# opensensor/thingino-accel

Hardware: AMD Instinct MI355X
Metric: images/sec yolov5s_int8 640x640 batch256 (higher is better)
Workload: dtype int8

## Files before the change

### thingino-accel_amd/csrc/hip/conv_i8.hip

```cpp
#include "conv_i8_common.hpp"

#ifndef I8M_ABL
#define I8M_ABL 0
#endif
template <int BPX, int BN, int STAGES, int KS = 1, int NW = 4>
__global__ __launch_bounds__(NW * 64) void conv_i8_mfma(const mhip_conv_i8_t p, const long total_pix, const int k64,
                                                         const int8_t *__restrict__ zeros, const unsigned noc,
                                                         const unsigned nblk, const int lg_inc, const unsigned kw_magic,
                                                         const fastdiv_t dhw, const fastdiv_t dow, const int bufmode,
                                                         const unsigned in_bytes) {
    ANAT_BEGIN();
    const bool POW2 = lg_inc >= 0;
    const bool masked = p.kh * p.kw <= 32;
    constexpr int SLICE = (BPX + BN) * BK;
    constexpr int STAGE = KS * SLICE;
    constexpr int NWN = BN == 128 ? 2 : 1;
    constexpr int NWM = NW / NWN;
    constexpr int WPX = BPX / NWM / 16;
    constexpr int WOC = BN / NWN / 16;
    constexpr int XROWS = BPX / NW;
    constexpr int XI = XROWS / 16;
    constexpr int LW = (BN / 16 + NW - 1) / NW;
    constexpr int L = XI + LW;
    static_assert(XI >= 1 && XROWS % 16 == 0, "every wave fetches whole 16-row pieces of the pixel tile");
// ... 158 lines not shown
        nstage = nstage + 1 == STAGES ? 0 : nstage + 1;
    }
    ANAT_NOW(2);
    __syncthreads();
    if (I8M_ABL & 1) {
        int fold = 0;
#pragma unroll
        for (int s = 0; s < WOC; s++)
#pragma unroll
            for (int t = 0; t < WPX; t++) fold ^= acc[s][t][0] ^ acc[s][t][1] ^ acc[s][t][2] ^ acc[s][t][3];
        if (fold == 0x12345678) p.out[0] = 1;
        return;
    }
    epilogue<BPX, BN, WPX, WOC, true>(p, acc, lds, slut, rowoff, oc0, pxw, ocw, hw);
    ANAT_END(p);
}

__device__ __forceinline__ int lds_off128(int row, int chunk8) { return row * 128 + ((chunk8 ^ ((row >> 1) & 7)) << 4); }
template <int BPX, int BN, int NW>
__global__ __launch_bounds__(NW * 64) void conv_i8_r128(const mhip_conv_i8_t p, const long total_pix, const int k128,
                                                         const unsigned noc, const unsigned nblk, const int lg_inc,
                                                         const unsigned kw_magic, const fastdiv_t dhw, const fastdiv_t dow,
                                                         const unsigned in_bytes) {
    constexpr int STAGE = (BPX + BN) * 128;
    constexpr int NWN = BN == 128 ? 2 : 1;
    constexpr int NWM = NW / NWN;
    constexpr int WPX = BPX / NWM / 16;
    constexpr int WOC = BN / NWN / 16;
    constexpr int XI = BPX / 8 / NW;
    constexpr int WI = BN / 8 / NW;
    static_assert(XI >= 1 && WI >= 1 && BPX % (8 * NW) == 0 && BN % (8 * NW) == 0, "whole 8-row pieces per wave");
    extern __shared__ __attribute__((aligned(16))) int8_t dynlds[];
    uint8_t *slut = (uint8_t *)dynlds;
    lds_base_must_be_zero(dynlds);
    long *rowoff = (long *)(dynlds + LUTB);
    int8_t *lds = dynlds + BPX * 8 + LUTB;

    const int tid = threadIdx.x, lane = tid & 63;
    const int wv = __builtin_amdgcn_readfirstlane(tid >> 6);
    const unsigned id = xcd_remap(blockIdx.x, nblk);
    const long pix0 = (long)(id / noc) * BPX;
    const int oc0 = (int)(id % noc) * BN;
    const int hw = p.out_h * p.out_w;
    const int wm = wv % NWM, wn = wv / NWM;
    const int pxw = wm * (WPX * 16), ocw = wn * (WOC * 16);
    v4i acc[WOC][WPX];
    init_acc<WPX, WOC>(p, acc, oc0 + ocw);
    if (p.lut2) { if (tid < 128) ((uint32_t *)slut)[tid] = ((const uint32_t *)p.lut2)[tid]; }
    else if (p.lut && tid < 64) ((uint32_t *)slut)[tid] = ((const uint32_t *)p.lut)[tid];
    fill_rowoff<BPX>(p, rowoff, [=](int row) { long q = pix0 + row; return q < total_pix ? q : -1L; }, (unsigned)hw, dhw);

    const int lrow = lane >> 3, lslot = lane & 7;
    int xvoff[XI];
    unsigned tapmask[XI];
#pragma unroll
    for (int j = 0; j < XI; j++) {
        const int trow = (wv * XI + j) * 8 + lrow;
        const long pix = pix0 + trow;
        const bool valid = pix < total_pix;
        const unsigned f = valid ? fdiv((unsigned)pix, dhw) : 0u;
        const unsigned rem = valid ? (unsigned)pix - f * (unsigned)hw : 0u;
        const int oy = (int)fdiv(rem, dow), ox = (int)(rem - (unsigned)oy * (unsigned)p.out_w);
        const int iy0 = oy * p.stride_h - p.pad_top, ix0 = ox * p.stride_w - p.pad_left;
        const int chunk = lslot ^ ((trow >> 1) & 7);
        xvoff[j] = (int)(f * (unsigned)p.in_stride) + (iy0 * p.in_w + ix0) * p.in_c + chunk * 16;
        const int kx_lo = ix0 < 0 ? -ix0 : 0, kx_hi = p.in_w - ix0 < p.kw ? p.in_w - ix0 : p.kw;
        const unsigned colbits = kx_hi > kx_lo ? ((kx_hi >= 32 ? ~0u : (1u << kx_hi) - 1u) & ~((1u << kx_lo) - 1u)) : 0u;
        unsigned m = 0;
        for (int r = 0; r < p.kh; r++) {
            const int iy = iy0 + r;
            if (iy >= 0 && iy < p.in_h) m |= colbits << (r * p.kw);
        }
        tapmask[j] = valid ? m : 0u;
    }
    int wvoff[WI];
#pragma unroll
    for (int j = 0; j < WI; j++) {
        const int trow = (wv * WI + j) * 8 + lrow;
        wvoff[j] = (oc0 + trow) * k128 + (lslot ^ ((trow >> 1) & 7)) * 16;
    }
    const __amdgpu_buffer_rsrc_t xrs = __builtin_amdgcn_make_buffer_rsrc((void *)p.in, 0, (int)in_bytes, 0x00020000);
    const __amdgpu_buffer_rsrc_t wrs = __builtin_amdgcn_make_buffer_rsrc((void *)p.w, 0, p.oc_pad * k128, 0x00020000);
    const int taps = p.kh * p.kw;
    const int nst = k128 / 128;
    auto issue = [&](int st, int buf) {
        int8_t *sb = lds + buf * STAGE;
        const int utap = (st * 128) >> lg_inc, urc = (st * 128) & ((1 << lg_inc) - 1);
        const int uky = (int)(((unsigned)utap * kw_magic) >> 16), ukx = utap - uky * p.kw;
        const int ukoff = (uky * p.in_w + ukx) * p.in_c + urc;
        const bool uvalid = utap < taps;
#pragma unroll
        for (int j = 0; j < XI; j++) {
            const bool ok = uvalid & (((tapmask[j] >> utap) & 1u) != 0u);
            blds16(xrs, ok ? xvoff[j] + ukoff : -1, 0, sb + (wv * XI + j) * 1024);
        }
#pragma unroll
        for (int j = 0; j < WI; j++) blds16(wrs, wvoff[j], st * 128, sb + BPX * 128 + (wv * WI + j) * 1024);
    };

    issue(0, 0);
    const int frow = lane & 15, fchunk = lane >> 4;
    for (int st = 0; st < nst; st++) {
        wait_vmcnt<0>();
        __builtin_amdgcn_s_barrier();
        asm volatile("" ::: "memory");
        const int8_t *xs = lds + (st & 1) * STAGE, *ws = xs + BPX * 128;
        v4i xb[2][WPX], wa[2][WOC];
#pragma unroll
        for (int h = 0; h < 2; h++) {
#pragma unroll
            for (int t = 0; t < WPX; t++) xb[h][t] = *(const v4i *)(xs + lds_off128(pxw + t * 16 + frow, h * 4 + fchunk));
#pragma unroll
            for (int q = 0; q < WOC; q++) wa[h][q] = *(const v4i *)(ws + lds_off128(ocw + q * 16 + frow, h * 4 + fchunk));
        }
        if (st + 1 < nst) issue(st + 1, (st + 1) & 1);
#pragma unroll
        for (int h = 0; h < 2; h++)
#pragma unroll
            for (int q = 0; q < WOC; q++)
#pragma unroll
                for (int t = 0; t < WPX; t++) acc[q][t] = __builtin_amdgcn_mfma_i32_16x16x64_i8(wa[h][q], xb[h][t], acc[q][t], 0, 0, 0);
    }
    __syncthreads();
    epilogue<BPX, BN, WPX, WOC, true>(p, acc, lds, slut, rowoff, oc0, pxw, ocw, hw);
}

template <int A, int B>
__device__ __forceinline__ void wait_vmcnt_at_most(int n) {
    constexpr int HI = A > B ? A : B, LO = A > B ? B : A;
    if (n >= A + B) wait_vmcnt<A + B>();
    else if (n >= HI) wait_vmcnt<HI>();
    else if (n >= LO) wait_vmcnt<LO>();
    else wait_vmcnt<0>();
}

struct conv_out_side_t {
    int8_t *out;
    size_t out_stride;
    const int8_t *w;
    const int32_t *bias;
    const uint8_t *lut, *lut2;
    int out_c, relu, out_pix_stride, out_ch_off;
    float cs;
    unsigned out_bytes;
};
template <int BPX, int BN, int STAGES, bool HAS_LUT, bool SEG = false, bool PAIR = false>
__global__ __launch_bounds__(NTHREADS) void conv_i8_persist(const mhip_conv_i8_t pin, const unsigned total_pix, const int k64,
                                                            const int8_t *__restrict__ zeros, const unsigned noc,
                                                            const unsigned npt, const unsigned ngrp, const int lg_inc,
                                                            const unsigned kw_magic, const fastdiv_t dhw, const fastdiv_t dow,
                                                            const unsigned out_bytes_first, const conv_out_side_t alt,
                                                            const unsigned noc0, const int bufmode, const unsigned in_bytes,
                                                            const int wres) {
    ANAT_BEGIN();
    const int STAGE = wres ? BPX * BK : (BPX + BN) * BK;
    constexpr int NWN = BN == 128 ? 2 : 1;
    constexpr int NWM = 4 / NWN;
    constexpr int WPX = BPX / NWM / 16;
    constexpr int WOC = BN / NWN / 16;
    constexpr int XI = BPX / 64;
    constexpr int LW = BN >= 128 ? 2 : 1;
    constexpr int L = XI + LW;
    constexpr int NST = WPX;
    extern __shared__ __attribute__((aligned(16))) int8_t dynlds[];
    uint8_t *slut = (uint8_t *)dynlds;
    int8_t *lds = dynlds + LUTB;
    lds_base_must_be_zero(dynlds);

    const int tid = threadIdx.x, lane = tid & 63;
    const int wv = __builtin_amdgcn_readfirstlane(tid >> 6);
    const unsigned id = xcd_remap(blockIdx.x, noc * ngrp);
    const unsigned grp = id / noc;
    unsigned ot = id - grp * noc;
    mhip_conv_i8_t p = pin;
    unsigned out_bytes = out_bytes_first;
    if (PAIR && ot >= noc0) {
        ot -= noc0;
        p.lut2 = alt.lut2;
        p.out = alt.out; p.out_stride = alt.out_stride; p.w = alt.w; p.bias = alt.bias; p.lut = alt.lut;
        p.out_c = alt.out_c; p.relu = alt.relu; p.out_pix_stride = alt.out_pix_stride; p.out_ch_off = alt.out_ch_off;
        p.cs = alt.cs;
        out_bytes = alt.out_bytes;
    }
    const int oc0 = (int)ot * BN;
    const unsigned t0 = (unsigned)(((unsigned long long)grp * npt) / ngrp);
    const unsigned t1 = (unsigned)(((unsigned long long)(grp + 1) * npt) / ngrp);
    if (t0 >= t1) return;
    const unsigned hw = (unsigned)(p.out_h * p.out_w);
    const int wm = wv % NWM, wn = wv / NWM;
    const int pxw = wm * (WPX * 16), ocw = wn * (WOC * 16);

    auto packed_row16 = [](int c) { return ((c >> 2) & 1) * 16 + (c >> 3) * 4 + (c & 3); };
    v4i bias[WOC];
#pragma unroll
    for (int s = 0; s < WOC; s++)
        bias[s] = p.bias ? *(const v4i *)(p.bias + (BN == 16 ? packed_row16((lane >> 4) * 4) : oc0 + ocw + s * 16 + (lane >> 4) * 4)) : (v4i){0, 0, 0, 0};
    if (HAS_LUT) {
        if (p.lut2) { if (tid < 128) ((uint32_t *)slut)[tid] = ((const uint32_t *)p.lut2)[tid]; }
        else if (tid < 64) ((uint32_t *)slut)[tid] = ((const uint32_t *)p.lut)[tid];
        __syncthreads();
    }
    const __amdgpu_buffer_rsrc_t orsrc = __builtin_amdgcn_make_buffer_rsrc(p.out, 0, (int)out_bytes, 0x00020000);

    const int schunk = (lane & 3) ^ (((lane >> 4) & 1) << 1);
    const int8_t *xwin[XI];
    unsigned tapmask[XI];
    unsigned rowf[SEG ? XI : 1], rowrem[SEG ? XI : 1];
    unsigned rowrem_up[SEG ? XI : 1];
    int xvoff[XI];
    auto setup_rows = [&](unsigned tile) {
#pragma unroll
        for (int j = 0; j < XI; j++) {
            const unsigned pix = tile * BPX + wv * (BPX / 4) + j * 16 + (lane >> 2);
            const bool valid = pix < total_pix;
            const unsigned f = valid ? fdiv(pix, dhw) : 0u;
            const unsigned rem = valid ? pix - f * hw : 0u;
            if (SEG) {
                rowf[j] = f;
                rowrem[j] = rem;
                const unsigned oy = fdiv(rem, dow), ox = rem - oy * (unsigned)p.out_w;
                rowrem_up[j] = (oy >> 1) * ((unsigned)p.out_w >> 1) + (ox >> 1);
                tapmask[j] = valid ? 1u : 0u;
                continue;
            }
            const int oy = (int)fdiv(rem, dow), ox = (int)(rem - (unsigned)oy * (unsigned)p.out_w);
            const int iy0 = oy * p.stride_h - p.pad_top, ix0 = ox * p.stride_w - p.pad_left;
            xwin[j] = p.in + (size_t)f * p.in_stride + ((long)iy0 * p.in_w + ix0) * p.in_c;
            xvoff[j] = (int)(f * (unsigned)p.in_stride) + (iy0 * p.in_w + ix0) * p.in_c + schunk * 16;
            const int kx_lo = ix0 < 0 ? -ix0 : 0, kx_hi = p.in_w - ix0 < p.kw ? p.in_w - ix0 : p.kw;
            const unsigned colbits = kx_hi > kx_lo ? ((kx_hi >= 32 ? ~0u : (1u << kx_hi) - 1u) & ~((1u << kx_lo) - 1u)) : 0u;
            unsigned m = 0;
            for (int r = 0; r < p.kh; r++) {
                const int iy = iy0 + r;
                if (iy >= 0 && iy < p.in_h) m |= colbits << (r * p.kw);
            }
            tapmask[j] = valid ? m : 0u;
        }
    };
    const int8_t *wsrc[LW];
    int wq[LW], wvoff[LW];
#pragma unroll
    for (int j = 0; j < LW; j++) {
        wq[j] = BN >= 64 ? wv * LW + j : (BN == 16 ? 0 : (wv & 1));
        const int wrow = BN == 16 ? packed_row16(lane >> 2) : oc0 + wq[j] * 16 + (lane >> 2);
        wsrc[j] = p.w + (size_t)wrow * k64 + schunk * 16;
        wvoff[j] = wrow * k64 + schunk * 16;
    }
    const __amdgpu_buffer_rsrc_t xrs = __builtin_amdgcn_make_buffer_rsrc((void *)p.in, 0, (int)in_bytes, 0x00020000);
    const __amdgpu_buffer_rsrc_t wrs = __builtin_amdgcn_make_buffer_rsrc((void *)p.w, 0, p.oc_pad * k64, 0x00020000);
    const int taps = p.kh * p.kw;
    const int nks = k64 / BK;

    auto issue = [&](int ks, int stage) {
        int8_t *sb = lds + stage * STAGE;
        const unsigned pos = (unsigned)(ks * BK + schunk * 16);
        if (SEG) {
            auto owner = [&](int c) { return (c >= p.seg_c0[1]) + (c >= p.seg_c0[2]) + (c >= p.seg_c0[3]); };
            const int sa = owner(ks * BK), sb2 = owner(ks * BK + 32);
            const bool hi = schunk >= 2;
            const int8_t *base = hi ? p.seg_in[sb2] : p.seg_in[sa];
            const unsigned fstride = (unsigned)(hi ? p.seg_stride[sb2] : p.seg_stride[sa]);
            const unsigned segc = (unsigned)(hi ? p.seg_c[sb2] : p.seg_c[sa]);
            const unsigned coff = pos - (unsigned)(hi ? p.seg_c0[sb2] : p.seg_c0[sa]);
            const bool up = ((p.seg_up >> (hi ? sb2 : sa)) & 1) != 0;
            const bool kvalid = (int)pos < p.in_c;
#pragma unroll
            for (int j = 0; j < XI; j++) {
                const bool ok = kvalid & (tapmask[j] != 0u);
                const int8_t *src = base + (size_t)rowf[j] * fstride + (size_t)(up ? rowrem_up[j] : rowrem[j]) * segc + coff;
                glds16(ok ? src : zeros, sb + (wv * (BPX / 4) + j * 16) * BK);
            }
        } else if (bufmode) {
            const int utap = (ks * BK) >> lg_inc, urc = (ks * BK) & ((1 << lg_inc) - 1);
            const int uky = (int)(((unsigned)utap * kw_magic) >> 16), ukx = utap - uky * p.kw;
            const int ukoff = (uky * p.in_w + ukx) * p.in_c + urc;
            const bool uvalid = utap < taps;
#pragma unroll
            for (int j = 0; j < XI; j++) {
                const bool ok = uvalid & (((tapmask[j] >> utap) & 1u) != 0u);
                blds16(xrs, ok ? xvoff[j] + ukoff : -1, 0, sb + (wv * (BPX / 4) + j * 16) * BK);
            }
            if (!wres)
#pragma unroll
                for (int j = 0; j < LW; j++) blds16(wrs, wvoff[j], ks * BK, sb + BPX * BK + wq[j] * 16 * BK);
            return;
        } else {
            const unsigned tap = pos >> lg_inc;
            const int rc = (int)(pos & ((1u << lg_inc) - 1u));
            const int ky = (int)((tap * kw_magic) >> 16);
            const int kx = (int)tap - ky * p.kw;
            const bool kvalid = (int)tap < taps;
            const long koff = ((long)ky * p.in_w + kx) * p.in_c + rc;
#pragma unroll
            for (int j = 0; j < XI; j++) {
                const bool ok = kvalid & ((tapmask[j] >> tap) & 1u);
                glds16(ok ? xwin[j] + koff : zeros, sb + (wv * (BPX / 4) + j * 16) * BK);
            }
        }
        if (!wres)
#pragma unroll
            for (int j = 0; j < LW; j++) glds16(wsrc[j] + ks * BK, sb + BPX * BK + wq[j] * 16 * BK);
    };

    int8_t *const wres_base = lds + STAGES * STAGE;
    if (wres)
        for (int ks = 0; ks < nks; ks++)
#pragma unroll
            for (int j = 0; j < LW; j++) glds16(wsrc[j] + ks * BK, wres_base + (ks * BN + wq[j] * 16) * BK);
    unsigned itile = t0;
    int iks = 0;
    int younger[STAGES - 1];
    setup_rows(t0);
    int nstage = 0;
#pragma unroll
    for (int s = 0; s < STAGES - 1; s++) {
        int n = 0;
        if (itile < t1) {
            issue(iks, nstage);
            n = wres ? XI : L;
            if (++iks == nks) {
                iks = 0;
                if (++itile < t1) setup_rows(itile);
            }
        }
#pragma unroll
        for (int i = 0; i < s; i++) younger[i] += n;
        younger[s] = 0;
        nstage++;
    }
    nstage = STAGES - 1;

    const int frow = lane & 15, fchunk = lane >> 4;
    const int chan = ocw + (lane >> 4) * (4 * WOC);
    const int pstride = p.out_pix_stride ? p.out_pix_stride : p.out_c;
    const int lo = p.relu ? 0 : -128;
    const uint8_t *lut128 = slut + 128;
    const bool ragged = (p.out_c % (WOC * 4)) != 0;
    int stage = 0;
    ANAT_NOW(1);
    for (unsigned tile = t0; tile < t1; tile++) {
        v4i acc[WOC][WPX];
        for (int ks = 0; ks < nks; ks++) {
            wait_vmcnt_at_most<(STAGES - 2) * L, NST>(younger[0]);
            __builtin_amdgcn_s_barrier();
            asm volatile("" ::: "memory");
            const int8_t *xs = lds + stage * STAGE, *ws = wres ? wres_base + ks * (BN * BK) : xs + BPX * BK;
            v4i xb[WPX], wa[WOC];
#pragma unroll
            for (int t = 0; t < WPX; t++) xb[t] = *(const v4i *)(xs + lds_off(pxw + t * 16 + frow, fchunk));
#pragma unroll
            for (int s = 0; s < WOC; s++) wa[s] = *(const v4i *)(ws + lds_off(ocw + s * 16 + frow, fchunk));
            int n = 0;
            if (itile < t1) {
                issue(iks, nstage);
                n = wres ? XI : L;
                if (++iks == nks) {
                    iks = 0;
                    if (++itile < t1) setup_rows(itile);
                }
            }
#pragma unroll
            for (int i = 0; i + 1 < STAGES - 1; i++) younger[i] = younger[i + 1] + n;
            younger[STAGES - 2] = 0;
            if (ks == 0) {
#pragma unroll
                for (int s = 0; s < WOC; s++)
#pragma unroll
                    for (int t = 0; t < WPX; t++) acc[s][t] = __builtin_amdgcn_mfma_i32_16x16x64_i8(wa[s], xb[t], bias[s], 0, 0, 0);
            } else {
#pragma unroll
                for (int s = 0; s < WOC; s++)
#pragma unroll
                    for (int t = 0; t < WPX; t++) acc[s][t] = __builtin_amdgcn_mfma_i32_16x16x64_i8(wa[s], xb[t], acc[s][t], 0, 0, 0);
            }
            stage = stage + 1 == STAGES ? 0 : stage + 1;
            nstage = nstage + 1 == STAGES ? 0 : nstage + 1;
        }
#ifdef ANATOMY
        if (tile + 1 == t1) ANAT_NOW(2);
#endif
#pragma unroll
        for (int t = 0; t < WPX; t++) {
            const unsigned pix = tile * BPX + pxw + t * 16 + (lane & 15);
            const unsigned f = fdiv(pix, dhw), rem = pix - f * hw;
            const unsigned off = f * (unsigned)p.out_stride + rem * (unsigned)pstride + (unsigned)(p.out_ch_off + oc0 + chan);
            const int nvalid = p.out_c - (oc0 + chan);
            const bool ok = pix < total_pix && nvalid >= WOC * 4;
            uint32_t pk[WOC];
            int a[WOC * 4];
#pragma unroll
            for (int s = 0; s < WOC; s++)
#pragma unroll
                for (int r = 0; r < 4; r++) a[s * 4 + r] = acc[s][t][r];
            if (HAS_LUT && p.lut2) requant_pack<WOC * 4, HAS_LUT, true, true, false, true>(a, p.cs, lo, lut128, pk);
            else requant_pack<WOC * 4, HAS_LUT, true, true>(a, p.cs, lo, lut128, pk);
            const int voff = ok ? (int)off : -1;
            if (WOC == 4)
                __builtin_amdgcn_raw_buffer_store_b128((v4i){(int)pk[0], (int)pk[1], (int)pk[2], (int)pk[3]}, orsrc, voff, 0, 0);
            else if (WOC == 2)
                __builtin_amdgcn_raw_buffer_store_b64((v2i){(int)pk[0], (int)pk[WOC > 1 ? 1 : 0]}, orsrc, voff, 0, 0);
            else
                __builtin_amdgcn_raw_buffer_store_b32((int)pk[0], orsrc, voff, 0, 0);
            if (ragged) {
                const bool part = pix < total_pix && nvalid > 0 && nvalid < WOC * 4;
                const int nv = part ? nvalid : 0;
                const int o4 = nv & 8, o2 = nv & 12, o1 = nv & 14;
                const uint32_t w4 = o4 ? pk[(WOC * 4 > 8) ? 2 : 0] : pk[0];
                const int i2 = o2 >> 2, i1 = o1 >> 2;
                uint32_t w2 = pk[0], w1 = pk[0];
#pragma unroll
                for (int q = 1; q < WOC; q++) {
                    w2 = i2 == q ? pk[q] : w2;
                    w1 = i1 == q ? pk[q] : w1;
                }
                w1 >>= (o1 & 2) * 8;
                if (WOC == 4)
                    __builtin_amdgcn_raw_buffer_store_b64((v2i){(int)pk[0], (int)pk[1]}, orsrc, (nv & 8) ? (int)off : -1, 0, 0);
                __builtin_amdgcn_raw_buffer_store_b32((int)w4, orsrc, (nv & 4) ? (int)off + o4 : -1, 0, 0);
                __builtin_amdgcn_raw_buffer_store_b16((short)w2, orsrc, (nv & 2) ? (int)off + o2 : -1, 0, 0);
                __builtin_amdgcn_raw_buffer_store_b8((char)w1, orsrc, (nv & 1) ? (int)off + o1 : -1, 0, 0);
            }
        }
#pragma unroll
        for (int i = 0; i < STAGES - 1; i++) younger[i] += ragged ? NST * (WOC == 4 ? 5 : 4) : NST;
    }
    ANAT_END(p);
}
ANAT_SETTER(mhip_anatomy_set_i8)
__device__ __forceinline__ bool mhip_small_c_dev(int in_c, int kw, int out_c) { return in_c <= 4 && kw <= 8 && out_c <= 64; }
template <int BN>
__global__ __launch_bounds__(NTHREADS) void conv_i8_generic(const mhip_conv_i8_t p, const long total_pix, const int k64,
                                                            const fastdiv_t dhw) {
    constexpr int STAGE = (BP + BN) * BK;
    constexpr int WPX = 2, WOC = BN / 16;
    constexpr int TILE_BYTES = BP * (BN + OPAD);
    constexpr int LDS_BYTES = (2 * STAGE > TILE_BYTES ? 2 * STAGE : TILE_BYTES) + 256;
    __shared__ __attribute__((aligned(16))) int8_t lds[LDS_BYTES];
    __shared__ long rowoff[BP];
    uint8_t *slut = (uint8_t *)lds + LDS_BYTES - 256;

    const int tid = threadIdx.x, lane = tid & 63, wv = tid >> 6;
    const long pix0 = (long)blockIdx.x * BP;
    const int oc0 = blockIdx.y * BN;
    const int hw = p.out_h * p.out_w;
    if (p.lut && tid < 64) ((uint32_t *)slut)[tid] = ((const uint32_t *)p.lut)[tid];
    fill_rowoff<BP>(p, rowoff, [=](int row) { long q = pix0 + row; return q < total_pix ? q : -1L; }, (unsigned)hw, dhw);

    const int cc = tid & 3;
    const int8_t *xbase[2];
    int iy0[2], ix0[2];
    bool rvalid[2];
#pragma unroll
    for (int j = 0; j < 2; j++) {
        long pix = pix0 + (tid >> 2) + j * 64;
        rvalid[j] = pix < total_pix;
        long f = rvalid[j] ? pix / hw : 0;
        int rem = rvalid[j] ? (int)(pix - f * hw) : 0;
        int oy = rem / p.out_w, ox = rem - oy * p.out_w;
        iy0[j] = oy * p.stride_h - p.pad_top;
        ix0[j] = ox * p.stride_w - p.pad_left;
        xbase[j] = p.in + (size_t)f * p.in_stride;
    }
    int ky = 0, rc = cc * 16;
    while (rc >= p.row_pad) { rc -= p.row_pad; ky++; }
    const int ceff = mhip_small_c_dev(p.in_c, p.kw, p.out_c) ? 4 : p.in_c;
    const int nks = k64 / BK;
    constexpr int WLOADS = (BN * 4 + NTHREADS - 1) / NTHREADS;
    v4i xreg[2], wreg[WLOADS];

    auto load_global = [&](int ks) {
#pragma unroll
        for (int j = 0; j < 2; j++) {
            v4i v = {0, 0, 0, 0};
            const int iy = iy0[j] + ky;
            if (rvalid[j] && ky < p.kh && iy >= 0 && iy < p.in_h) {
                const int8_t *rowp = xbase[j] + ((long)iy * p.in_w + ix0[j]) * p.in_c;
                int8_t b[16];
#pragma unroll
                for (int e = 0; e < 16; e++) {
                    const int rr = rc + e;
                    int8_t val = 0;
                    const int tap = rr / ceff, ch = rr - tap * ceff;
                    if (tap < p.kw && ch < p.in_c) {
                        const int ix = ix0[j] + tap;
                        if (ix >= 0 && ix < p.in_w) val = rowp[tap * p.in_c + ch];
                    }
                    b[e] = val;
                }
                v = *(v4i *)b;
            }
            xreg[j] = v;
        }
#pragma unroll
        for (int j = 0; j < WLOADS; j++) {
            const int idx = tid + j * NTHREADS;
            if (idx < BN * 4) wreg[j] = *(const v4i *)(p.w + (size_t)(oc0 + (idx >> 2)) * k64 + ks * BK + (idx & 3) * 16);
        }
        rc += BK;
        while (rc >= p.row_pad) { rc -= p.row_pad; ky++; }
    };
    auto store_lds = [&](int buf) {
#pragma unroll
        for (int j = 0; j < 2; j++) *(v4i *)(lds + buf * STAGE + lds_off((tid >> 2) + j * 64, cc)) = xreg[j];
#pragma unroll
        for (int j = 0; j < WLOADS; j++) {
            const int idx = tid + j * NTHREADS;
            if (idx < BN * 4) *(v4i *)(lds + buf * STAGE + BP * BK + lds_off(idx >> 2, idx & 3)) = wreg[j];
        }
    };

    v4i acc[WOC][WPX];
    init_acc<WPX, WOC>(p, acc, oc0);

    load_global(0);
    store_lds(0);
    __syncthreads();
    const int frow = lane & 15, fchunk = lane >> 4;
    const int pxw = wv * 32;
    for (int ks = 0; ks < nks; ks++) {
        const int buf = ks & 1;
        if (ks + 1 < nks) load_global(ks + 1);
        v4i xb[WPX];
#pragma unroll
        for (int t = 0; t < WPX; t++) xb[t] = *(const v4i *)(lds + buf * STAGE + lds_off(pxw + t * 16 + frow, fchunk));
#pragma unroll
        for (int s = 0; s < WOC; s++) {
            v4i wa = *(const v4i *)(lds + buf * STAGE + BP * BK + lds_off(s * 16 + frow, fchunk));
#pragma unroll
            for (int t = 0; t < WPX; t++) acc[s][t] = __builtin_amdgcn_mfma_i32_16x16x64_i8(wa, xb[t], acc[s][t], 0, 0, 0);
        }
        if (ks + 1 < nks) store_lds(buf ^ 1);
        __syncthreads();
    }
    epilogue<BP, BN, WPX, WOC>(p, acc, lds, slut, rowoff, oc0, pxw, 0, hw);
}

extern "C" int mhip_conv_i8_oc_row(int oc, int oc_pad) {
    const int G = (oc_pad % 64 == 0) ? 64 : 32, NS = G / 16;
    const int g = oc / G, local = oc - g * G;
    const int q = local / (4 * NS), rem = local - q * 4 * NS, s = rem >> 2, r = rem & 3;
    return g * G + s * 16 + q * 4 + r;
}

extern "C" int mhip_conv_i8_is_safe(float cs) {
    return cs == cs && cs < 0.99f && cs > -0.99f;
}

extern "C" int mhip_conv_i8_lut2_ok(float cs) {
    if (!mhip_conv_i8_is_safe(cs)) return 0;
    const float a = cs < 0 ? -cs : cs;
    if (!(a >= 1e-6f)) return 0;
    const float quirk = 0.49999997f;
    const double a0 = (double)quirk / (double)a;
    for (int d = -3; d <= 3; d++) {
        const double c = (double)(long long)(a0 + 0.5) + d;
        if (c < 1.0 || c > 2147483647.0) continue;
        volatile float prod = (float)(int)c * a;
        if (prod == quirk) return 0;
    }
    return 1;
}

extern "C" int mhip_conv_i8_small_c(int in_c, int kw, int out_c) { return in_c <= 4 && kw <= 8 && out_c <= 64; }

extern "C" void mhip_conv_i8_pack_geom(int in_c, int kw, int out_c, int *row_pad, int *oc_pad, int *c_eff) {
    const int small = mhip_conv_i8_small_c(in_c, kw, out_c);
    if (row_pad) *row_pad = small ? 32 : (kw * in_c + 15) & ~15;
    if (oc_pad) *oc_pad = (out_c + 31) & ~31;
    if (c_eff) *c_eff = small ? 4 : in_c;
}

static tune_t g_tune;
static int env_int(const char *name, int dflt) {
    const char *e = getenv(name);
    return e ? atoi(e) : dflt;
}
const tune_t &conv_i8_tune_state() {
    if (!g_tune.init) {
        g_tune.persist = env_int("MARS_HIP_PERSIST", 1);
// ... 208 lines not shown
    *bpx = px;
    return true;
}

static variant_t default_variant(const mhip_conv_i8_t *p, int nks) {
    variant_t v;
    v.patch = 0;
    v.ks2 = 0;
    v.w8 = 0;
    v.wres = 0;
    v.r128 = 0;
    v.rows = 0;
    int ring = 0;
    const long wg_large = ((long)p->frames * p->out_h * p->out_w + 255) / 256 * ((p->oc_pad + 127) / 128);
    const bool few = wg_large < tune().few_wgs && tune().persist && !tune().bpx && !tune().stages && tune().small_batch;
    if (few) {
        if (conv_i8_patch_ok(p, 4, &ring)) {
            v.persist = 0; v.bpx = 0; v.stages = 0; v.patch = 4;
            return v;
        }
        if (nks >= 8 && r128_ok(p)) {
            v.persist = 0; v.bpx = 0; v.stages = 0; v.r128 = 1;
            return v;
        }
        v.bpx = 128;
        v.persist = nks <= tune().persist_maxk && persist_eligible(p);
        if (((p->out_c | p->out_pix_stride | p->out_ch_off) & 15) != 0 && p->nseg <= 1) v.persist = 0;
        v.stages = v.persist ? 2 : 3;
        return v;
    }
    if (tune().persist && !tune().bpx && !tune().stages && tune().rows && p->out_w <= 20 && p->in_c >= 256 && conv_i8_rows_ok(p)) {
        v.persist = 0; v.bpx = 0; v.stages = 0; v.rows = 1;
        return v;
    }
    if (tune().persist && !tune().bpx && !tune().stages) {
        if (conv_i8_patch_ok(p, 16, &ring)) {
            v.persist = 0; v.bpx = 0; v.stages = 0; v.patch = 16;
            return v;
        }
        if (conv_i8_patch_ok(p, 8, &ring) && ring >= 2) {
            v.persist = 0; v.bpx = 0; v.stages = 0; v.patch = 8;
            return v;
        }
    }
    v.bpx = tune().bpx ? tune().bpx : ((p->oc_pad % 128 != 0 && nks <= 2) ? 256 : 128);
    v.persist = tune().persist && nks <= tune().persist_maxk && persist_eligible(p);
    if (((p->out_c | p->out_pix_stride | p->out_ch_off) & 15) != 0 && p->nseg <= 1) v.persist = 0;
    v.stages = v.persist ? 2 : (tune().stages ? tune().stages : (nks <= 4 ? 2 : 3));
    if (v.stages != 3) v.stages = 2;
    if (v.persist && v.stages == 2 && !tune().bpx && wres_default(p, nks, &v.bpx)) v.wres = 1;
    if ((!v.persist || (!v.wres && nks >= 8 && p->nseg <= 1)) && !tune().bpx && !tune().stages && p->oc_pad % 128 == 0 &&
        nks >= (tune().persist_maxk < 8 ? tune().persist_maxk + 1 : 8)) {
        v.persist = 0; v.w8 = 1; v.bpx = 256; v.stages = 3;
    }
    if (p->nseg > 1 && !v.wres && !tune().bpx && nks >= 8) v.bpx = 256;
    return v;
}

template <int BPX, int BN>
static int launch_variant_t(const mhip_conv_i8_t *p, long total_pix, int k64, const variant_t &v) {
    if (v.persist) {
        if (!persist_eligible(p)) return -1;
        int lg = 0;
        while ((1 << lg) < p->in_c) lg++;
        const unsigned magic = ((65536u + (unsigned)p->kw - 1u) / (unsigned)p->kw);
        if (v.wres && wres_lds<BPX, BN>(k64) > 80 * 1024) return -1;
        if (p->nseg > 1)
            return p->lut ? launch_persist_t<BPX, BN, 2, true, true>(p, total_pix, k64, lg, magic, nullptr, v.wres)
                          : launch_persist_t<BPX, BN, 2, false, true>(p, total_pix, k64, lg, magic, nullptr, v.wres);
        if (v.wres)
            return p->lut ? launch_persist_t<BPX, BN, 2, true>(p, total_pix, k64, lg, magic, nullptr, 1)
                          : launch_persist_t<BPX, BN, 2, false>(p, total_pix, k64, lg, magic, nullptr, 1);
        if (v.stages == 2)
            return p->lut ? launch_persist_t<BPX, BN, 2, true>(p, total_pix, k64, lg, magic)
                          : launch_persist_t<BPX, BN, 2, false>(p, total_pix, k64, lg, magic);
        return -1;
    }
    if constexpr (BN == 16) {
        return -1;
    } else {
        if (v.w8) return BN == 128 ? launch_mfma<256, 128, 3, 1, 8>(p, total_pix, k64) : -1;
        if (v.ks2) return BPX == 128 && BN >= 64 ? launch_mfma<128, (BN >= 64 ? BN : 64), 2, 2>(p, total_pix, k64) : -1;
        return v.stages == 2 ? launch_mfma<BPX, BN, 2>(p, total_pix, k64) : launch_mfma<BPX, BN, 3>(p, total_pix, k64);
    }
}
static bool bn16_ok(const mhip_conv_i8_t *p) {
    static const bool off = getenv("MARS_HIP_NO_BN16") != nullptr;
    return !off && p->out_c <= 16 && p->oc_pad == 32 && p->nseg <= 1;
}

static int launch_variant(const mhip_conv_i8_t *p, long total_pix, int k64, const variant_t &v) {
    if (v.persist < 0) return -1;
    if (v.rows) return conv_i8_launch_rows(p);
    if (v.r128) return launch_r128(p, total_pix, v.r128);
    if (v.patch) return conv_i8_launch_patch(p, k64, v.patch);
    const int bn = p->oc_pad % 128 == 0 ? 128 : (p->oc_pad % 64 == 0 ? 64 : 32);
    const bool b16 = v.persist && v.stages == 2 && bn16_ok(p);
    if (v.bpx == 256) {
        if (bn == 128) return launch_variant_t<256, 128>(p, total_pix, k64, v);
        if (bn == 64) return launch_variant_t<256, 64>(p, total_pix, k64, v);
        if (b16) return launch_variant_t<256, 16>(p, total_pix, k64, v);
        return launch_variant_t<256, 32>(p, total_pix, k64, v);
    }
    if (bn == 128) return launch_variant_t<128, 128>(p, total_pix, k64, v);
    if (bn == 64) return launch_variant_t<128, 64>(p, total_pix, k64, v);
    if (b16) return launch_variant_t<128, 16>(p, total_pix, k64, v);
    return launch_variant_t<128, 32>(p, total_pix, k64, v);
}

template <int BPX, int BN>
static int launch_pair_t(const mhip_conv_i8_t *a, const mhip_conv_i8_t *b, long total_pix, int k64, int lg, unsigned magic,
                         int wres) {
    if (a->nseg > 1) return -2;
    return launch_persist_t<BPX, BN, 2, true, false, true>(a, total_pix, k64, lg, magic, b, wres);
}
extern "C" int mhip_conv_i8_pair(const mhip_conv_i8_t *a, const mhip_conv_i8_t *b) {
    if (!a || !b || !tune().persist || tune().variant) return -2;
    if (a->in != b->in || a->in_stride != b->in_stride || a->frames != b->frames || a->in_h != b->in_h || a->in_w != b->in_w ||
        a->in_c != b->in_c || a->out_h != b->out_h || a->out_w != b->out_w || a->kh != b->kh || a->kw != b->kw ||
        a->stride_h != b->stride_h || a->stride_w != b->stride_w || a->pad_top != b->pad_top || a->pad_left != b->pad_left ||
        a->row_pad != b->row_pad || a->nseg != b->nseg || a->seg_up != b->seg_up || !a->lut || !b->lut || a->add || b->add ||
        a->out_nchw || b->out_nchw)
        return -2;
    for (int i = 0; i < a->nseg; i++)
        if (a->seg_in[i] != b->seg_in[i] || a->seg_c[i] != b->seg_c[i] || a->seg_stride[i] != b->seg_stride[i]) return -2;
    if ((a->in_c % 16) != 0 || mhip_conv_i8_small_c(a->in_c, a->kw, a->out_c) || mhip_conv_i8_small_c(b->in_c, b->kw, b->out_c))
        return -2;
    if (a->nseg > 1 && (!seg_valid(a) || !seg_valid(b))) return -2;
    if (!persist_eligible(a) || !persist_eligible(b)) return -2;
    const int bn = a->oc_pad % 128 == 0 ? 128 : (a->oc_pad % 64 == 0 ? 64 : 32);
    const int bnb = b->oc_pad % 128 == 0 ? 128 : (b->oc_pad % 64 == 0 ? 64 : 32);
    if (bn != bnb || !mhip_zero_page()) return -2;
    const long total_pix = (long)a->frames * a->out_h * a->out_w;
    const int k64 = (a->kh * a->row_pad + BK - 1) / BK * BK, nks = k64 / BK;
    if (total_pix <= 0 || total_pix > 0x7fffffffL) return -2;
    int lg = 0;
    while ((1 << lg) < a->in_c) lg++;
    const unsigned magic = ((65536u + (unsigned)a->kw - 1u) / (unsigned)a->kw);
    const variant_t dv = default_variant(a, nks);
    const int bpx = dv.bpx ? dv.bpx : 128, wres = dv.persist && dv.wres && (tune().wres & 2);
    const bool b16 = bn16_ok(a) && bn16_ok(b);
    if (bpx == 256) {
        if (bn == 128) return launch_pair_t<256, 128>(a, b, total_pix, k64, lg, magic, wres);
        if (bn == 64) return launch_pair_t<256, 64>(a, b, total_pix, k64, lg, magic, wres);
        if (b16) return launch_pair_t<256, 16>(a, b, total_pix, k64, lg, magic, wres);
        return launch_pair_t<256, 32>(a, b, total_pix, k64, lg, magic, wres);
    }
    if (bn == 128) return launch_pair_t<128, 128>(a, b, total_pix, k64, lg, magic, wres);
    if (bn == 64) return launch_pair_t<128, 64>(a, b, total_pix, k64, lg, magic, wres);
    if (b16) return launch_pair_t<128, 16>(a, b, total_pix, k64, lg, magic, wres);
    return launch_pair_t<128, 32>(a, b, total_pix, k64, lg, magic, wres);
}

extern "C" int mhip_conv_i8_seg_ok(const mhip_conv_i8_t *p) {
    return p && (p->in_c % 16) == 0 && !mhip_conv_i8_small_c(p->in_c, p->kw, p->out_c) && seg_valid(p) && persist_eligible(p);
}

extern "C" int mhip_conv_i8_variants(const mhip_conv_i8_t *p, int *codes, int max) {
    if (!p || (p->in_c % 16) != 0 || mhip_conv_i8_small_c(p->in_c, p->kw, p->out_c)) return 0;
    const int k64 = (p->kh * p->row_pad + BK - 1) / BK * BK, nks = k64 / BK;
    int n = 0;
    if (p->pre_w) {
        const int first = conv_i8_pre_tile_rows(p);
        for (int th : {first, 16, 8, 4})
            if (th && n < max && conv_i8_patch_ok(p, th, nullptr)) {
                const int code = th == 16 ? 10 : (th == 8 ? 9 : 11);
                bool seen = false;
                for (int i = 0; i < n; i++) seen |= codes[i] == code;
                if (!seen) codes[n++] = code;
            }
        return n;
    }
    if (p->nseg > 1) {
        const int bn = p->oc_pad % 128 == 0 ? 128 : (p->oc_pad % 64 == 0 ? 64 : 32);
        const variant_t dv = default_variant(p, nks);
        const int dflt = dv.persist && dv.wres ? (dv.bpx == 256 ? 15 : 14) : (dv.bpx == 256 ? 4 : 2);
        if (n < max) codes[n++] = dflt;
        if (n < max && dflt != 2) codes[n++] = 2;
        if (n < max && dflt != 4) codes[n++] = 4;
        if (n < max && dflt != 14 && LUTB + 2 * (size_t)128 * BK + (size_t)nks * bn * BK <= 80 * 1024) codes[n++] = 14;
        if (n < max && dflt != 15 && LUTB + 2 * (size_t)256 * BK + (size_t)nks * bn * BK <= 80 * 1024) codes[n++] = 15;
        return n;
    }
    const int dflt = variant_code(default_variant(p, nks));
    if (n < max) codes[n++] = dflt;
    for (int code = 1; code <= NVARIANTS; code++) {
        const variant_t v = variant_of(code);
        if (code == dflt) continue;
        if (v.patch && !conv_i8_patch_ok(p, v.patch, nullptr)) continue;
        if (v.persist && !persist_eligible(p)) continue;
        if (v.ks2 && ((nks & 1) || nks < 4 || p->oc_pad % 64 != 0)) continue;
        if (v.w8 && (p->oc_pad % 128 != 0 || nks < 3)) continue;
        if (v.persist < 0) continue;
        if (v.r128 && !r128_ok(p)) continue;
        if (v.rows && !conv_i8_rows_ok(p)) continue;
        if (v.wres) {
            const int bn = p->oc_pad % 128 == 0 ? 128 : (p->oc_pad % 64 == 0 ? 64 : 32);
            if (LUTB + 2 * (size_t)v.bpx * BK + (size_t)nks * bn * BK > 80 * 1024) continue;
        }
        if (!v.persist && v.stages == 3 && nks <= 2) continue;
        if (n < max) codes[n++] = code;
    }
    return n;
}

template <int BN>
static int launch_generic(const mhip_conv_i8_t *p, long total_pix, int k64) {
    dim3 grid((unsigned)((total_pix + BP - 1) / BP), (unsigned)(p->oc_pad / BN));
    hipLaunchKernelGGL((conv_i8_generic<BN>), grid, dim3(NTHREADS), 0, mhip_stream_native(), *p, total_pix, k64,
                       make_fastdiv((unsigned)(p->out_h * p->out_w)));
    return mhip_check(hipGetLastError(), "conv_i8_generic launch");
}

extern "C" int mhip_conv_i8(const mhip_conv_i8_t *p) {
    if (!p || !p->in || !p->out || !p->w) return -1;
    if (p->out_pix_stride < 0 || p->out_ch_off < 0 || (p->out_nchw && (p->out_pix_stride || p->out_ch_off)) ||
        (p->out_pix_stride && p->out_pix_stride < p->out_ch_off + p->out_c))
        return -1;
    if (p->frames <= 0 || p->in_h <= 0 || p->in_w <= 0 || p->in_c <= 0 || p->out_h <= 0 || p->out_w <= 0 ||
        p->out_c <= 0 || p->kh <= 0 || p->kw <= 0 || p->stride_h < 0 || p->stride_w < 0)
        return -1;
    int row_pad, oc_pad;
    mhip_conv_i8_pack_geom(p->in_c, p->kw, p->out_c, &row_pad, &oc_pad, nullptr);
    if (row_pad != p->row_pad || oc_pad != p->oc_pad) return -1;
    if (p->add && (!p->safe || p->out_nchw || ((p->out_c | p->out_pix_stride | p->out_ch_off) & 15) || (p->in_c % 16) != 0 ||
                   mhip_conv_i8_small_c(p->in_c, p->kw, p->out_c) || p->nseg > 1))
        return -1;
    const long total_pix = (long)p->frames * p->out_h * p->out_w;
    const int k64 = (p->kh * p->row_pad + BK - 1) / BK * BK;
    if (total_pix <= 0 || total_pix > 0x7fffffffL || (total_pix + BP - 1) / BP * (oc_pad / 32) > 0x7fffffffL) return -1;
    if (p->in_planar) {
        if (p->in_planar > 4 || p->in_c != 4 || p->in_w < 4 || p->stride_h < 1 || p->stride_w < 1 || p->add || p->nseg > 1 ||
            !mhip_conv_i8_small_c(p->in_c, p->kw, p->out_c))
            return -2;
        return conv_i8_try_smallc(p, k64);
    }
    if (mhip_conv_i8_small_c(p->in_c, p->kw, p->out_c)) {
        if (p->stride_h >= 1 && p->stride_w >= 1) {
            int rc = conv_i8_try_rgb(p, k64);
            if (rc == -2) rc = conv_i8_try_smallc(p, k64);
            if (rc != -2) return rc;
        }
        if (p->add || p->nseg > 1) return -1;
        if (oc_pad % 64 == 0) return launch_generic<64>(p, total_pix, k64);
        return launch_generic<32>(p, total_pix, k64);
    }
    if (p->pre_w) {
        if (!mhip_zero_page() || !mhip_conv_i8_pre_ok(p)) return -1;
        int th = conv_i8_pre_tile_rows(p);
        const int code = p->variant ? p->variant : tune().variant;
        if (code >= 9 && code <= 11) {
            const int want = code == 10 ? 16 : (code == 9 ? 8 : 4);
            if (conv_i8_patch_ok(p, want, nullptr)) th = want;
        } else if (tune().small_batch && conv_i8_patch_ok(p, 4, nullptr) &&
                   ((long)p->frames * p->out_h * p->out_w + 255) / 256 * ((p->oc_pad + 127) / 128) < 256) {
            th = 4;
        }
        return conv_i8_launch_patch(p, k64, th);
    }
    if ((p->in_c % 16) == 0) {
        if (!mhip_zero_page()) return -1;
        const int nks = k64 / BK;
        if (p->variant < 0 || p->variant > NVARIANTS) return -1;
        int code = p->variant;
        if (p->nseg > 1) {
            if (!seg_valid(p) || !persist_eligible(p)) return -1;
            if (!code && tune().variant) {
                int codes[NVARIANTS];
                const int n = mhip_conv_i8_variants(p, codes, NVARIANTS);
                for (int i = 0; i < n; i++)
                    if (codes[i] == tune().variant) code = codes[i];
            }
            variant_t v = variant_of(code == 4 || code == 14 || code == 15 ? code : 2);
            if (!code) {
                const variant_t dv = default_variant(p, nks);
                v.bpx = dv.bpx ? dv.bpx : 128;
                v.wres = dv.persist && dv.wres;
            }
            return launch_variant(p, total_pix, k64, v);
        }
        if (!code && tune().variant) {
            int codes[NVARIANTS];
            const int n = mhip_conv_i8_variants(p, codes, NVARIANTS);
            for (int i = 0; i < n; i++)
                if (codes[i] == tune().variant) code = codes[i];
        }
        return launch_variant(p, total_pix, k64, code ? variant_of(code) : default_variant(p, nks));
    }
    if (oc_pad % 64 == 0) return launch_generic<64>(p, total_pix, k64);
    return launch_generic<32>(p, total_pix, k64);
}
```

### thingino-accel_amd/csrc/host/mars_internal.h

```cpp
#ifndef MARS_INTERNAL_H
#define MARS_INTERNAL_H

#include <stddef.h>
#include <stdint.h>

#include "../mhip.h"
#include "mars_hip.h"
#include "mars_runtime.h"

enum {
    OP_CONV_I8 = 0,
    OP_CONV_F32,
    OP_RELU_BYTES,
    OP_LUT_I8,
    OP_BINARY_I8,
    OP_SIGMOID_F32,
    OP_BINARY_F32,
    OP_RELU_F32,
    OP_BN,
    OP_MAXPOOL,
    OP_CONCAT_SLICE,
    OP_UPSAMPLE,
    OP_UPSAMPLE_Q, OP_MAXPOOL_Q,
    OP_CONCAT_Q,
    OP_CONV_F32_VHEAD,
    OP_FAIL,
};

#define NO_OFF ((size_t)-1)
#define MARS_MAX_IO 4
#define MARS_MAX_MODEL_TUNE 16

typedef struct {
    size_t bytes;
    size_t extent;
    size_t stride;
    uint8_t *dev;
    int is_weight;
    int needed;
    int io_in, io_out;
    uint8_t *host;
    uint8_t *dense_dev;
    int pix_c, pix_stride;
    int rec_c, rec_hw;
    int nhwc_c, nhwc_hw;
    size_t zero_from;
    int partial;
    int nhwc_pitch;
    int tail_read;
} mtensor_t;

typedef struct {
    int kind, layer, err;
    int t_in[4], n_in, t_out;
    int in_h, in_w, in_c, out_h, out_w, out_c, kh, kw, sh, sw, pt, pl;
    int nchw, relu, is_mul, is_f32, leaky, safe;
    size_t in_byte_off, out_byte_off;
    int k_limit;
    int vc_n, vc_t[3], vc_run, vc_shift;
    int rows_only;
    int out_nchw;
    int silu_f32;
    int f32_exact;
    int variant;
    int add_t; float add_s_conv, add_s_other, add_inv;
    int nseg, seg_t[4], seg_c[4], seg_up;
    int chain_n, chain_out[3];
    int pair_next;
    int row_pad, oc_pad, c_pad;
    int ch_off, scale_h, scale_w, bn_n;
    int out_pix_stride, out_ch_off;
    int store_c;
    float cs, f0, f1, f2;
    size_t n;
    size_t w_off, b_off, lut_off, s_off;
    int pre;
    size_t pre_w_off, pre_b_off, pre_lut2_off;
    float pre_cs;
    size_t w2_off;
    int w2_rows;
    int w2_planes;
    size_t w3_off;
    int w3_stem;
    int in_rec, out_rec;
    size_t lut2_off;
    size_t w_blob_off[2];
    double macs, bytes;
    int prof_kind;
    float last_ms;
    void *ev0, *ev1;
    int prof_rec;
    void *ev_start;
} mars_op_t;

typedef struct {
    int fusion;
    unsigned no_fuse_lut : 1, no_nhwc_internal : 1, no_vconcat_q : 1, no_pair_f32 : 1, no_rec : 1, no_zero_tail : 1, no_vconcat_f32 : 1,
        no_rowpad : 1;
    size_t rec_limit;
    size_t vconcat_limit;
    size_t bottleneck_limit;
} plan_switches_t;

typedef struct mars_model_ext {
    mars_model_t pub;
    plan_switches_t sw;
    int batch, profiling, deferred;
    int plan_err;
    int no_vconcat;
    int no_download;
    int no_bottleneck;
    int rec_frames;
    int rec_skipped;
    size_t rec_max_frames;
    mtensor_t *mt;
    mars_op_t *ops;
    int n_ops, cap_ops;
    uint8_t *arena_host;
    size_t arena_size, arena_cap;
    uint8_t *arena_dev;
    size_t blob_mirror_bytes;
    uint8_t *act_dev;
    size_t act_bytes;
    uint8_t *scratch_dev;
    size_t scratch_per_frame;
    int scratch_t, scratch_cpad, scratch_f0, scratch_n;
    void *det_dev;
    int *det_counts_dev;
    float *det_lut_dev;
    int det_cap;
    float det_lut_scale[4];
    int det_lut_n;
    int det_lut_mono[4];
    float *heads_lut_dev;
    float heads_lut_scale[4];
    int heads_lut_n;
    float *dfl_lut_dev;
    float dfl_lut_scale[4][2];
    int dfl_lut_n;
    void *ev_graph_done, *ev_tail_done;
    int tail_pending;
    int frame0, run_frames;
    void *ev_fork, *ev_join[3];
    void *ev_chunk[2][8];
    void *graph_exec;
    unsigned graph_gen;
    int ran_plain;
    void *pipe;
    struct { char key[28]; int value, saved; } tune[MARS_MAX_MODEL_TUNE];
    int n_tune, tune_depth;
    int plan_f32_mode;
    unsigned char *layer_noop;
    void *roi_dev;
    int roi_cap_slots, roi_cap_frames;
    int roi_slots;
    struct mars_model_ext *roi_from;
    void *cls_dev;
    size_t cls_bytes, cls_sums_off, cls_top_off;
    int cls_frames, cls_c, cls_top_k;
    void *ev_label_done;
    int label_pending;
    void *label_dev;
    int label_cap, label_frames;
    void *match_dev;
    size_t match_bytes, match_top_off, match_row_off;
    int match_frames, match_top_k;
    void *ident_dev;
    int ident_cap, ident_frames;
    struct mars_model_ext *live_next;
} mars_model_ext_t;


#define MARS_INTERNAL __attribute__((visibility("hidden")))
#define ALIGN_UP(x, a) (((x) + (size_t)(a) - 1) & ~((size_t)(a) - 1))
#define NO_TENSOR 0xFFFFFFFFu
#define MAX_DIM_PRODUCT ((size_t)1 << 40)
#define ARENA_MAX ((size_t)1 << 40)
#define MAX_CHANNELS 65536
MARS_INTERNAL int mars_verbose(void);
#define VLOG(...) do { if (mars_verbose()) fprintf(stderr, "Mars: " __VA_ARGS__); } while (0)
MARS_INTERNAL void drop_graph(mars_model_ext_t *m);
MARS_INTERNAL mars_model_ext_t *mars_live_models(void);
MARS_INTERNAL void plan_switches_read(plan_switches_t *sw, int at_load);
MARS_INTERNAL mars_error_t build_plan(mars_model_ext_t *m);
MARS_INTERNAL mars_error_t upload_params(mars_model_ext_t *m);
MARS_INTERNAL mars_error_t alloc_batch(mars_model_ext_t *m, int n);
MARS_INTERNAL size_t elem_size(uint32_t dtype);
MARS_INTERNAL size_t shape_numel(const mars_tensor_t *d);
MARS_INTERNAL size_t reference_buffer_size(const mars_model_ext_t *m);
MARS_INTERNAL size_t arena_reserve(mars_model_ext_t *m, size_t bytes);
MARS_INTERNAL void blob_read(const mars_model_ext_t *m, size_t off, size_t n, void *dst);
MARS_INTERNAL int op_reads(const mars_op_t *o, int t);
MARS_INTERNAL int op_writes(const mars_op_t *o, int t);
MARS_INTERNAL size_t planned_stride(const mtensor_t *t);
MARS_INTERNAL void conv_i8_geometry(const mars_op_t *op, int frames, mhip_conv_i8_t *p);
MARS_INTERNAL int conv_i8_pre_fits(const mars_op_t *op, int frames, size_t in_stride, size_t out_stride);
MARS_INTERNAL void plan_layer(mars_model_ext_t *m, int li);
MARS_INTERNAL void fold_silu(mars_model_ext_t *m, int f32);
MARS_INTERNAL void fuse_lut(mars_model_ext_t *m);
MARS_INTERNAL void nhwc_internal(mars_model_ext_t *m);
MARS_INTERNAL void fold_add(mars_model_ext_t *m, int f32);
MARS_INTERNAL void virtual_concat(mars_model_ext_t *m);
MARS_INTERNAL void elide_concat(mars_model_ext_t *m);
MARS_INTERNAL void trim_concat(mars_model_ext_t *m);
MARS_INTERNAL void fuse_pool_chains(mars_model_ext_t *m);
MARS_INTERNAL void pair_convs(mars_model_ext_t *m);
MARS_INTERNAL void fuse_bottleneck(mars_model_ext_t *m);
MARS_INTERNAL void pad_output_rows(mars_model_ext_t *m);
MARS_INTERNAL void virtual_concat_q(mars_model_ext_t *m);
MARS_INTERNAL void f32_policy(mars_model_ext_t *m);
MARS_INTERNAL void zero_tail_f32(mars_model_ext_t *m);
MARS_INTERNAL void pair_convs_f32(mars_model_ext_t *m);
MARS_INTERNAL void rec_pairs(mars_model_ext_t *m);
MARS_INTERNAL void virtual_concat_f32(mars_model_ext_t *m);
MARS_INTERNAL void plan_check(mars_model_ext_t *m);
MARS_INTERNAL void conv_i8_params(const mars_model_ext_t *m, const mars_op_t *op, mhip_conv_i8_t *p);
MARS_INTERNAL int mars_preproc_prepare(int w, int h, int tw, int th);
MARS_INTERNAL int mars_preproc_prepare_nv12(int w, int h, int tw, int th, int frames);

MARS_INTERNAL void mars_roi_release(mars_model_ext_t *m);

MARS_INTERNAL void mars_cls_release(mars_model_ext_t *m);

MARS_INTERNAL void mars_match_release(mars_model_ext_t *m);

MARS_INTERNAL int mars_tensor_chw(const mars_tensor_t *d, int *c, int *h, int *w);
MARS_INTERNAL int mars_locate_i8(const mars_model_ext_t *m, int T, int ch, int hh, int ww, int any_writer, int *buf, int *off, int *pix_step, int *ch_step);
MARS_INTERNAL mars_error_t mars_tail_on_aux(mars_model_ext_t *m, int (*launch)(struct mars_model_ext *, const void *, void *, int *), const void *cfg);

mars_error_t mars_detect_prepare(mars_model_ext_t *m, const int *output_indices, int n_outputs);
int mars_detect_launch(mars_model_ext_t *m, const int *output_indices, int n_outputs, float nms_thresh, void *dets_dev,
                       int *counts_dev);

typedef struct {
    int n, ti[4], stride[4], nc[4], h[4], w[4], pix_step[4], ch_step[4];
    float anchors[4][3][2];
    float conf, nms;
    int map, px, py;
    float rx, ry;
    int internal;
} mars_heads_cfg_t;
MARS_INTERNAL int mars_find_heads(const mars_model_ext_t *m, int *tensor_ids, int *strides, int *num_classes, int cap);
MARS_INTERNAL mars_error_t mars_heads_resolve(mars_model_ext_t *m, const mars_yolo_heads_t *h, mars_heads_cfg_t *c);
MARS_INTERNAL mars_error_t mars_heads_prepare(mars_model_ext_t *m, const mars_heads_cfg_t *c);
MARS_INTERNAL int mars_heads_launch(mars_model_ext_t *m, const mars_heads_cfg_t *c, void *dets_dev, int *counts_dev);

typedef struct {
    int n, reg_max, stride[4], nc[4], h[4], w[4];
    int box_t[4], cls_t[4], box_buf[4], cls_buf[4], box_off[4], cls_off[4];
    int box_pix_step[4], box_ch_step[4], cls_pix_step[4], cls_ch_step[4];
    float box_scale[4], cls_scale[4];
    float conf, nms;
    int map, px, py;
    float rx, ry;
    int internal;
} mars_dfl_cfg_t;
MARS_INTERNAL int mars_find_dfl_heads(const mars_model_ext_t *m, int *box_ids, int *cls_ids, int *strides, int *num_classes, int *reg_max, int cap);
MARS_INTERNAL mars_error_t mars_dfl_resolve(mars_model_ext_t *m, const mars_yolo_dfl_heads_t *h, mars_dfl_cfg_t *c);
MARS_INTERNAL mars_error_t mars_dfl_prepare(mars_model_ext_t *m, const mars_dfl_cfg_t *c);
MARS_INTERNAL int mars_dfl_launch(mars_model_ext_t *m, const mars_dfl_cfg_t *c, void *dets_dev, int *counts_dev);

int32_t mars_trunc_x86(float x);
void mars_pack_conv_i8(const int8_t *w, size_t avail, int nchw, int out_c, int in_c, int kh, int kw,
                       int c_pad, int row_pad, int oc_pad, int8_t *dst);

#endif
```

### thingino-accel_amd/csrc/host/mars_model.c

```c
#include <math.h>
#include <stdio.h>
#include <stdlib.h>
#include <string.h>
#include <sys/types.h>
#include <time.h>

#include "mars_internal.h"
#include "nna.h"


int mars_verbose(void) {
    static int v = -1;
    if (v < 0) v = getenv("MARS_VERBOSE") ? 1 : 0;
    return v;
}

void plan_switches_read(plan_switches_t *sw, int at_load) {
    const char *e;
    if (at_load) sw->fusion = (e = getenv("MARS_HIP_FUSION")) ? atoi(e) : 1;
    sw->no_fuse_lut = getenv("MARS_HIP_NO_FUSE_LUT") != NULL;
    sw->no_nhwc_internal = getenv("MARS_HIP_NO_NHWC_INTERNAL") != NULL;
    sw->no_vconcat_q = getenv("MARS_HIP_NO_VCONCAT_Q") != NULL;
    sw->no_pair_f32 = getenv("MARS_HIP_NO_PAIR_F32") != NULL;
    sw->no_rec = getenv("MARS_HIP_NO_REC") != NULL;
    sw->no_zero_tail = getenv("MARS_HIP_NO_ZERO_TAIL") != NULL;
    sw->no_vconcat_f32 = getenv("MARS_HIP_NO_VCONCAT_F32") != NULL;
    sw->no_rowpad = getenv("MARS_HIP_NO_ROWPAD") != NULL;
    sw->rec_limit = (e = getenv("MARS_HIP_REC_LIMIT")) ? (size_t)strtoull(e, NULL, 0) : (size_t)0xfffffff0u;
    sw->vconcat_limit = (e = getenv("MARS_HIP_VCONCAT_LIMIT")) ? (size_t)strtoull(e, NULL, 0) : (size_t)0x7fffffffu;
    sw->bottleneck_limit = (e = getenv("MARS_HIP_BOTTLENECK_LIMIT")) ? (size_t)strtoull(e, NULL, 0) : 0;
}

void drop_graph(mars_model_ext_t *m) {
    if (m->graph_exec) {
        mhip_sync();
        mhip_graph_destroy(m->graph_exec);
    }
    m->graph_exec = NULL;
    m->ran_plain = 0;
}

static const char *const k_err[] = {
    "OK", "Invalid magic number", "Version mismatch", "Memory allocation failed",
    "Invalid file format", "NNA initialization failed", "Layer execution failed",
    "Invalid tensor", "Invalid layer",
};

const char *mars_get_error_string(mars_error_t err) {
    int i = -(int)err;
    if (i >= 0 && i < (int)(sizeof(k_err) / sizeof(k_err[0]))) return k_err[i];
    return "Unknown error";
}

static void free_device_state(mars_model_ext_t *m) {
    drop_graph(m);
    if (m->act_dev) mhip_free(m->act_dev);
    if (m->scratch_dev) mhip_free(m->scratch_dev);
    m->act_dev = m->scratch_dev = NULL;
    for (uint32_t i = 0; m->mt && i < m->pub.header.num_tensors; i++) {
        if (m->mt[i].host) mhip_host_free(m->mt[i].host);
        m->mt[i].host = NULL;
        if (m->mt[i].dense_dev) mhip_free(m->mt[i].dense_dev);
        m->mt[i].dense_dev = NULL;
        if (!m->mt[i].is_weight) m->mt[i].dev = NULL;
    }
    if (m->det_dev) mhip_free(m->det_dev);
    if (m->det_counts_dev) mhip_free(m->det_counts_dev);
    m->det_dev = NULL;
    m->det_counts_dev = NULL;
    m->det_cap = 0;
    m->tail_pending = 0;
    mars_roi_release(m);
    mars_cls_release(m);
}

static void free_ops(mars_model_ext_t *m) {
    drop_graph(m);
    for (int i = 0; i < m->n_ops; i++) {
        if (m->ops[i].ev0) mhip_event_destroy(m->ops[i].ev0);
        if (m->ops[i].ev1) mhip_event_destroy(m->ops[i].ev1);
    }
    free(m->ops);
    m->ops = NULL;
    m->n_ops = m->cap_ops = 0;
}

static mars_model_ext_t *g_live_models = NULL;
mars_model_ext_t *mars_live_models(void) { return g_live_models; }

void mars_free(mars_model_t *model) {
    if (!model) return;
    mars_model_ext_t *m = (mars_model_ext_t *)model;
    for (mars_model_ext_t **pp = &g_live_models; *pp; pp = &(*pp)->live_next)
        if (*pp == m) { *pp = m->live_next; break; }
    for (mars_model_ext_t *x = g_live_models; x; x = x->live_next)
        if (x->roi_from == m) x->roi_from = NULL;
    if (m->pipe) mars_hip_pipe_close(model);
    if (mhip_ready()) mhip_sync();
    free_device_state(m);
    free_ops(m);
    if (m->arena_dev) mhip_free(m->arena_dev);
    if (m->det_lut_dev) mhip_free(m->det_lut_dev);
    if (m->heads_lut_dev) mhip_free(m->heads_lut_dev);
    if (m->dfl_lut_dev) mhip_free(m->dfl_lut_dev);
    if (m->ev_graph_done) mhip_event_destroy(m->ev_graph_done);
    if (m->ev_tail_done) mhip_event_destroy(m->ev_tail_done);
    if (m->ev_label_done) mhip_event_destroy(m->ev_label_done);
    if (m->ev_fork) mhip_event_destroy(m->ev_fork);
    for (int k = 0; k < 3; k++)
        if (m->ev_join[k]) mhip_event_destroy(m->ev_join[k]);
    for (int k = 0; k < 2; k++)
        for (int c = 0; c < 8; c++)
            if (m->ev_chunk[k][c]) mhip_event_destroy(m->ev_chunk[k][c]);
    free(m->arena_host);
    free(m->layer_noop);
    free(m->mt);
    free(m->pub.weights);
    free(m->pub.layers);
    free(m->pub.tensors);
    free(m);
}

mars_error_t build_plan(mars_model_ext_t *m) {
    const uint32_t nt = m->pub.header.num_tensors, nl = m->pub.header.num_layers;
    plan_switches_read(&m->sw, 0);
    free_ops(m);
    m->arena_size = 0;
    if (m->arena_host) memset(m->arena_host, 0, m->arena_cap);
    m->scratch_per_frame = 0;
    m->plan_err = MARS_OK;
    m->plan_f32_mode = mhip_conv_f32_mode(-1);
    m->blob_mirror_bytes = m->pub.weights_size;
    for (uint32_t i = 0; i < nt; i++) {
        m->mt[i].extent = m->mt[i].bytes;
        m->mt[i].pix_c = m->mt[i].pix_stride = 0;
        m->mt[i].needed = (m->mt[i].io_in || m->mt[i].io_out) ? 1 : 0;
    }
    for (uint32_t i = 0; i < nl && m->plan_err == MARS_OK; i++) {
        const int n0 = m->n_ops;
        plan_layer(m, (int)i);
        m->layer_noop[i] = m->n_ops == n0;
    }
    if (m->plan_err != MARS_OK) return (mars_error_t)m->plan_err;
    if (m->sw.fusion >= 1) {
        fold_silu(m, 0);
        fuse_lut(m);
        fold_silu(m, 1);
        nhwc_internal(m);
        fold_add(m, 0);
        fold_add(m, 1);
        if (!m->no_vconcat) virtual_concat(m);
        elide_concat(m);
        trim_concat(m);
        fuse_pool_chains(m);
        pair_convs(m);
        if (m->sw.fusion >= 2 && !m->no_bottleneck) fuse_bottleneck(m);
        pad_output_rows(m);
        virtual_concat_q(m);
    } else {
        nhwc_internal(m);
    }
    f32_policy(m);
    zero_tail_f32(m);
    if (m->sw.fusion >= 1) pair_convs_f32(m);
    rec_pairs(m);
    virtual_concat_f32(m);
    if (m->plan_err == MARS_OK) plan_check(m);
    return (mars_error_t)m->plan_err;
}

mars_error_t upload_params(mars_model_ext_t *m) {
    size_t mirror_off = arena_reserve(m, m->blob_mirror_bytes + 64);
    if (mirror_off == NO_OFF) return MARS_ERR_ALLOC_FAILED;
    if (!m->deferred) blob_read(m, 0, m->blob_mirror_bytes, m->arena_host + mirror_off);
    if (m->arena_dev) mhip_free(m->arena_dev);
    m->arena_dev = (uint8_t *)mhip_malloc(m->arena_size);
    if (!m->arena_dev) return MARS_ERR_ALLOC_FAILED;
    if (mhip_h2d_async(m->arena_dev, m->arena_host, m->arena_size) || mhip_sync()) return MARS_ERR_NNA_INIT_FAILED;
    for (uint32_t i = 0; i < m->pub.header.num_tensors; i++) {
        if (!m->mt[i].is_weight) continue;
        m->mt[i].dev = m->arena_dev + mirror_off + (size_t)m->pub.tensors[i].desc.data_offset;
        m->mt[i].stride = 0;
        m->pub.tensors[i].paddr = m->mt[i].dev;
    }
    m->pub.ddr_paddr = m->arena_dev;
    m->pub.ddr_size = m->arena_size;
    return MARS_OK;
}

mars_error_t alloc_batch(mars_model_ext_t *m, int n) {
    const uint32_t nt = m->pub.header.num_tensors;
    if (m->pipe) mars_hip_pipe_close(&m->pub);
    if (mhip_sync()) return MARS_ERR_LAYER_FAILED;
    plan_switches_read(&m->sw, 0);
    const size_t vlim = m->sw.vconcat_limit, blim = m->sw.bottleneck_limit;
    const int rec_replan = (size_t)n > m->rec_max_frames || (m->rec_skipped && n < m->rec_frames);
    m->rec_frames = n;
    if (m->no_vconcat || m->no_bottleneck || rec_replan) {
        m->no_vconcat = m->no_bottleneck = 0;
        mars_error_t e = build_plan(m);
        if (e == MARS_OK) e = upload_params(m);
        if (e != MARS_OK) return e;
    }
    if (!m->no_vconcat)
        for (int i = 0; i < m->n_ops; i++) {
            const mars_op_t *op = &m->ops[i];
            if (op->kind != OP_CONV_I8 || op->nseg < 2 || op->t_out < 0) continue;
            if (planned_stride(&m->mt[op->t_out]) * (size_t)n > vlim) {
                m->no_vconcat = 1;
                mars_error_t e = build_plan(m);
                if (e == MARS_OK) e = upload_params(m);
                if (e != MARS_OK) return e;
                break;
            }
        }
    if (m->sw.fusion >= 2 && !m->no_bottleneck)
        for (int i = 0; i < m->n_ops; i++) {
            const mars_op_t *op = &m->ops[i];
            if (op->kind != OP_CONV_I8 || !op->pre || op->t_out < 0) continue;
            const size_t in_stride = op->t_in[0] >= 0 ? planned_stride(&m->mt[op->t_in[0]]) : 0;
            if (!conv_i8_pre_fits(op, n, in_stride, planned_stride(&m->mt[op->t_out])) || (blim && (size_t)n > blim)) {
                m->no_bottleneck = 1;
                mars_error_t e = build_plan(m);
                if (e == MARS_OK) e = upload_params(m);
                if (e != MARS_OK) return e;
                break;
            }
        }
    free_device_state(m);
    size_t per_frame = 0;
    for (uint32_t i = 0; i < nt; i++) {
        mtensor_t *t = &m->mt[i];
        if (t->is_weight || !t->needed) continue;
        t->stride = planned_stride(t);
        per_frame += t->stride;
    }
    m->act_bytes = per_frame * (size_t)n;
    m->act_dev = (uint8_t *)mhip_malloc(m->act_bytes + 512);
    if (!m->act_dev) return MARS_ERR_ALLOC_FAILED;
    if (mhip_memset_async(m->act_dev, 0, m->act_bytes + 256)) return MARS_ERR_ALLOC_FAILED;
    size_t off = 256;
    for (uint32_t i = 0; i < nt; i++) {
        mtensor_t *t = &m->mt[i];
        mars_runtime_tensor_t *rt = &m->pub.tensors[i];
        if (t->is_weight) continue;
        rt->vaddr = NULL; rt->paddr = NULL; rt->alloc_size = 0;
        if (!t->needed) continue;
        t->dev = m->act_dev + off;
        off += t->stride * (size_t)n;
        rt->paddr = t->dev;
        rt->alloc_size = t->stride * (size_t)n;
        if (t->io_in || t->io_out) {
            const size_t hb = t->bytes * (size_t)n, ref = reference_buffer_size(m);
            size_t cap = hb > ref ? hb : ref;
            if (ref > ((size_t)8 << 20)) cap = hb;
            t->host = (uint8_t *)mhip_host_alloc(cap ? cap : 64);
            if (!t->host) return MARS_ERR_ALLOC_FAILED;
            memset(t->host, 0, cap);
            rt->vaddr = t->host;
            rt->alloc_size = n == 1 && cap >= ref ? ref : hb;
        }
        if (t->pix_stride) {
            t->dense_dev = (uint8_t *)mhip_malloc(t->bytes * (size_t)n);
            if (!t->dense_dev) return MARS_ERR_ALLOC_FAILED;
        }
    }
    if (m->scratch_per_frame) {
        m->scratch_dev = (uint8_t *)mhip_malloc(ALIGN_UP(m->scratch_per_frame, 256) * (size_t)n + 256);
        if (!m->scratch_dev) return MARS_ERR_ALLOC_FAILED;
    }
    m->batch = n;
    m->frame0 = 0;
    m->run_frames = n;
    return mhip_sync() ? MARS_ERR_ALLOC_FAILED : MARS_OK;
}

static mars_error_t load_host(const void *data, size_t size, unsigned flags, mars_model_ext_t **out_m) {
    if (!data || !out_m || size < sizeof(mars_header_t)) return MARS_ERR_INVALID_FILE;
    const uint8_t *p = (const uint8_t *)data;
    mars_header_t h;
    memcpy(&h, p, sizeof(h));
    if (h.magic != MARS_MAGIC) {
        VLOG("Invalid magic 0x%08x (expected 0x%08x)\n", h.magic, MARS_MAGIC);
        return MARS_ERR_INVALID_MAGIC;
    }
    if (h.version_major != MARS_VERSION_MAJOR) return MARS_ERR_VERSION_MISMATCH;
    if (h.num_tensors > 65536 || h.num_layers > 65536 || h.num_inputs > 4 || h.num_outputs > 4) return MARS_ERR_INVALID_FILE;
    const size_t tables = sizeof(h) + (size_t)h.num_tensors * sizeof(mars_tensor_t) + (size_t)h.num_layers * sizeof(mars_layer_t);
    if (tables > size) return MARS_ERR_INVALID_FILE;
    const int deferred = (flags & MARS_HIP_LOAD_DEFER_WEIGHTS) != 0;
    if (!deferred && h.weights_size > 0 && (h.weights_offset > size || h.weights_size > size - h.weights_offset))
        return MARS_ERR_INVALID_FILE;
    if (h.weights_size > ((uint64_t)1 << 36)) return MARS_ERR_INVALID_FILE;

    mars_model_ext_t *m = (mars_model_ext_t *)calloc(1, sizeof(*m));
    if (!m) return MARS_ERR_ALLOC_FAILED;
    m->pub.header = h;
    plan_switches_read(&m->sw, 1);
    m->deferred = deferred;
    m->pub.tensors = (mars_runtime_tensor_t *)calloc(h.num_tensors ? h.num_tensors : 1, sizeof(mars_runtime_tensor_t));
    m->pub.layers = (mars_runtime_layer_t *)calloc(h.num_layers ? h.num_layers : 1, sizeof(mars_runtime_layer_t));
    m->mt = (mtensor_t *)calloc(h.num_tensors ? h.num_tensors : 1, sizeof(mtensor_t));
    m->layer_noop = (unsigned char *)calloc(h.num_layers ? h.num_layers : 1, 1);
    if (!m->pub.tensors || !m->pub.layers || !m->mt || !m->layer_noop) { mars_free(&m->pub); return MARS_ERR_ALLOC_FAILED; }
    const uint8_t *q = p + sizeof(h);
    for (uint32_t i = 0; i < h.num_tensors; i++, q += sizeof(mars_tensor_t)) memcpy(&m->pub.tensors[i].desc, q, sizeof(mars_tensor_t));
    for (uint32_t i = 0; i < h.num_layers; i++, q += sizeof(mars_layer_t)) memcpy(&m->pub.layers[i].desc, q, sizeof(mars_layer_t));

    m->pub.weights_size = (size_t)h.weights_size;
    if (h.weights_size) {
        m->pub.weights = calloc(1, (size_t)h.weights_size);
        if (!m->pub.weights) { mars_free(&m->pub); return MARS_ERR_ALLOC_FAILED; }
        if (!deferred) memcpy(m->pub.weights, p + h.weights_offset, (size_t)h.weights_size);
    }
    m->pub.ddr_base = m->pub.weights;
    for (uint32_t i = 0; i < h.num_tensors; i++) {
        mars_runtime_tensor_t *rt = &m->pub.tensors[i];
        if (rt->desc.ndims > MARS_MAX_DIMS) { mars_free(&m->pub); return MARS_ERR_INVALID_FILE; }
        m->mt[i].bytes = shape_numel(&rt->desc) * elem_size(rt->desc.dtype);
        if (rt->desc.data_size > 0) {
            if (rt->desc.data_offset > h.weights_size) { mars_free(&m->pub); return MARS_ERR_INVALID_FILE; }
            m->mt[i].is_weight = 1;
            rt->vaddr = (uint8_t *)m->pub.weights + rt->desc.data_offset;
            rt->alloc_size = (size_t)rt->desc.data_size;
        }
    }
    for (uint32_t i = 0; i < h.num_inputs; i++) {
        uint32_t id = h.input_tensor_ids[i];
        if (id < h.num_tensors && !m->mt[id].is_weight) m->mt[id].io_in = (int)i + 1;
    }
    for (uint32_t i = 0; i < h.num_outputs; i++) {
        uint32_t id = h.output_tensor_ids[i];
        if (id < h.num_tensors && !m->mt[id].is_weight) m->mt[id].io_out = (int)i + 1;
    }

    mars_error_t err = build_plan(m);
    if (err != MARS_OK) { mars_free(&m->pub); return err; }
    VLOG("%u layers -> %d launches, parameter arena %zu bytes\n", h.num_layers, m->n_ops, m->arena_size);
    *out_m = m;
    return MARS_OK;
}

mars_error_t mars_hip_load_memory_ex(const void *data, size_t size, unsigned flags, mars_model_t **out_model) {
    if (!out_model) return MARS_ERR_INVALID_FILE;
    mars_model_ext_t *m = NULL;
    mars_error_t err = load_host(data, size, flags, &m);
    if (err != MARS_OK) return err;
    if (!nna_is_ready() || !mhip_ready()) {
        fprintf(stderr, "Mars: no initialised MI355X device (call nna_init first); refusing to load\n");
        mars_free(&m->pub);
        return MARS_ERR_NNA_INIT_FAILED;
    }
    err = upload_params(m);
    if (err == MARS_OK) err = alloc_batch(m, 1);
    if (err != MARS_OK) { mars_free(&m->pub); return err; }
    m->live_next = g_live_models;
    g_live_models = m;
    *out_model = &m->pub;
    return MARS_OK;
}

static int describe_op_full(const mars_op_t *o, char *line, size_t cap, int k) {
#define ADD(...) k += snprintf(line + k, cap - (size_t)k, __VA_ARGS__)
    ADD(" | err %d in %dx%dx%d out %dx%dx%d k %dx%d s %dx%d p %d,%d", o->err, o->in_h, o->in_w, o->in_c, o->out_h, o->out_w, o->out_c, o->kh, o->kw, o->sh, o->sw, o->pt, o->pl);
    ADD(" nchw %d out_nchw %d relu %d is_mul %d is_f32 %d leaky %d safe %d silu %d f32_exact %d variant %d", o->nchw, o->out_nchw, o->relu, o->is_mul, o->is_f32, o->leaky,
        o->safe, o->silu_f32, o->f32_exact, o->variant);
    ADD(" row_pad %d oc_pad %d c_pad %d store_c %d ch_off %d out_ch_off %d out_pix_stride %d in_byte_off %zu out_byte_off %zu scale %dx%d bn_n %d n %zu", o->row_pad,
        o->oc_pad, o->c_pad, o->store_c, o->ch_off, o->out_ch_off, o->out_pix_stride, o->in_byte_off, o->out_byte_off, o->scale_h, o->scale_w, o->bn_n, o->n);
    ADD(" k_limit %d rows_only %d pair_next %d in_rec %d out_rec %d vc %d,%d,%d:", o->k_limit, o->rows_only, o->pair_next, o->in_rec, o->out_rec, o->vc_n, o->vc_run, o->vc_shift);
    for (int q = 0; q < o->vc_n && q < 3; q++) ADD(" %d", o->vc_t[q]);
    ADD(" add %d %a %a %a seg %d up %d:", o->add_t, (double)o->add_s_conv, (double)o->add_s_other, (double)o->add_inv, o->nseg, o->seg_up);
    for (int q = 0; q < o->nseg && q < 4; q++) ADD(" %d/%d", o->seg_t[q], o->seg_c[q]);
    ADD(" chain %d:", o->chain_n);
    for (int q = 0; q < o->chain_n && q < 3; q++) ADD(" %d", o->chain_out[q]);
    ADD(" cs %a f %a %a %a", (double)o->cs, (double)o->f0, (double)o->f1, (double)o->f2);
    ADD(" w_off %zd b_off %zd lut_off %zd lut2_off %zd s_off %zd w2_off %zd rows %d planes %d w3_off %zd stem %d blob %zd %zd", (ssize_t)o->w_off, (ssize_t)o->b_off,
        (ssize_t)o->lut_off, (ssize_t)o->lut2_off, (ssize_t)o->s_off, (ssize_t)o->w2_off, o->w2_rows, o->w2_planes, (ssize_t)o->w3_off, o->w3_stem, (ssize_t)o->w_blob_off[0],
        (ssize_t)o->w_blob_off[1]);
    ADD(" pre %d", o->pre);
    if (o->pre) ADD(" %zd %zd %zd %a", (ssize_t)o->pre_w_off, (ssize_t)o->pre_b_off, (ssize_t)o->pre_lut2_off, (double)o->pre_cs);
    ADD(" macs %a bytes %a prof_kind %d", o->macs, o->bytes, o->prof_kind);
#undef ADD
    return k;
}

size_t mars_hip_describe_plan(const void *data, size_t size, unsigned flags, char *out, size_t cap) {
    static const char *const kinds[] = {"conv_i8", "conv_f32", "relu_bytes", "lut_i8", "binary_i8", "sigmoid_f32", "binary_f32", "relu_f32", "bn",
                                        "maxpool", "concat_slice", "upsample", "upsample_q", "maxpool_q", "concat_q", "conv_f32_vhead", "fail"};
    mars_model_ext_t *m = NULL;
    const int full = (flags & MARS_HIP_DESCRIBE_FULL) != 0;
    if (load_host(data, size, flags & ~MARS_HIP_DESCRIBE_FULL, &m) != MARS_OK) return 0;
    size_t n = 0;
    char line[4096];
#define EMIT() do { const size_t l = strlen(line); if (out && n < cap) memcpy(out + n, line, n + l <= cap ? l : cap - n); n += l; } while (0)
    for (int i = 0; i < m->n_ops; i++) {
        const mars_op_t *o = &m->ops[i];
        int k = snprintf(line, sizeof line, "op %d layer %d %s in", i, o->layer, o->kind >= 0 && o->kind <= OP_FAIL ? kinds[o->kind] : "?");
        for (int q = 0; q < o->n_in && q < 4; q++) k += snprintf(line + k, sizeof line - (size_t)k, " %d", o->t_in[q]);
        k += snprintf(line + k, sizeof line - (size_t)k, " out %d", o->t_out);
#define FLAG(cond, ...) if (cond) k += snprintf(line + k, sizeof line - (size_t)k, __VA_ARGS__)
        FLAG(o->kind == OP_CONV_I8 || o->kind == OP_CONV_F32 || o->kind == OP_CONV_F32_VHEAD, " k%dx%d s%d c%d->%d", o->kh, o->kw, o->sw, o->in_c, o->out_c);
        FLAG(o->nchw, " relayout"); FLAG(o->out_nchw, " planar_store"); FLAG(o->lut_off != NO_OFF, " lut"); FLAG(o->add_t, " add=%d", o->add_t - 1);
        FLAG(o->nseg, " seg=%d", o->nseg); FLAG(o->pair_next, " pair_next"); FLAG(o->pre, " pre"); FLAG(o->silu_f32, " silu");
        FLAG(o->k_limit, " k_limit=%d", o->k_limit); FLAG(o->in_rec, " in_rec=%d", o->in_rec); FLAG(o->out_rec, " out_rec");
        FLAG(o->vc_shift, " view=-%d", o->vc_shift); FLAG(o->vc_n, " vcat=%dx%d", o->vc_n, o->vc_run);
        FLAG(o->rows_only, " rows_only=%d", o->rows_only); FLAG(o->out_byte_off, " out_off=%zu", o->out_byte_off); FLAG(o->chain_n, " chain=%d", o->chain_n);
        FLAG(o->out_pix_stride, " pix_stride=%d", o->out_pix_stride); FLAG(o->kind == OP_FAIL, " err=%d", o->err);
#undef FLAG
        if (full) k = describe_op_full(o, line, sizeof line, k);
        snprintf(line + k, sizeof line - (size_t)k, "\n");
        EMIT();
    }
    for (uint32_t t = 0; t < m->pub.header.num_tensors; t++) {
        const mtensor_t *mt = &m->mt[t];
        const int listed = mt->nhwc_c || mt->partial || mt->zero_from || mt->rec_c || mt->pix_stride;
        if (!listed && !(full && mt->needed)) continue;
        int k = listed ? snprintf(line, sizeof line, "tensor %u nhwc_c %d pitch %d partial %d zero_from %zu rec_c %d pix_stride %d", t, mt->nhwc_c, mt->nhwc_pitch,
                                  mt->partial, mt->zero_from, mt->rec_c, mt->pix_stride)
                       : snprintf(line, sizeof line, "+tensor %u", t);
        if (full)
            k += snprintf(line + k, sizeof line - (size_t)k, " | bytes %zu extent %zu needed %d tail_read %d weight %d io %d,%d pix_c %d rec_hw %d nhwc_hw %d", mt->bytes,
                          mt->extent, mt->needed, mt->tail_read, mt->is_weight, mt->io_in, mt->io_out, mt->pix_c, mt->rec_hw, mt->nhwc_hw);
        snprintf(line + k, sizeof line - (size_t)k, "\n");
        EMIT();
    }
    if (full) {
        const plan_switches_t *w = &m->sw;
        snprintf(line, sizeof line, "+plan n_ops %d arena_size %zu scratch_per_frame %zu blob_mirror_bytes %zu rec_max_frames %zu rec_skipped %d f32_mode %d | fusion %d"
                 " no_fuse_lut %d no_nhwc_internal %d no_vconcat_q %d no_pair_f32 %d no_rec %d no_zero_tail %d no_vconcat_f32 %d no_rowpad %d rec_limit %zu"
                 " vconcat_limit %zu bottleneck_limit %zu\n", m->n_ops, m->arena_size, m->scratch_per_frame, m->blob_mirror_bytes, m->rec_max_frames, m->rec_skipped,
                 m->plan_f32_mode, w->fusion, w->no_fuse_lut, w->no_nhwc_internal, w->no_vconcat_q, w->no_pair_f32, w->no_rec, w->no_zero_tail, w->no_vconcat_f32,
                 w->no_rowpad, w->rec_limit, w->vconcat_limit, w->bottleneck_limit);
        EMIT();
    }
#undef EMIT
    if (out && cap) out[n < cap ? n : cap - 1] = 0;
    mars_free(&m->pub);
    return n;
}

int mars_yolo_find_heads(const void *data, size_t size, int *tensor_ids, int *strides, int *num_classes, int cap) {
    mars_model_ext_t *m = NULL;
    if (load_host(data, size, 0, &m) != MARS_OK) return -1;
    const int n = mars_find_heads(m, tensor_ids, strides, num_classes, cap);
    mars_free(&m->pub);
    return n;
}

int mars_yolo_find_dfl_heads(const void *data, size_t size, int *box_ids, int *cls_ids, int *strides, int *num_classes, int *reg_max, int cap) {
    mars_model_ext_t *m = NULL;
    if (load_host(data, size, 0, &m) != MARS_OK) return -1;
    const int n = mars_find_dfl_heads(m, box_ids, cls_ids, strides, num_classes, reg_max, cap);
    mars_free(&m->pub);
    return n;
}

mars_error_t mars_load_memory(const void *data, size_t size, mars_model_t **model) {
    return mars_hip_load_memory_ex(data, size, 0, model);
}

mars_error_t mars_load_file(const char *path, mars_model_t **model) {
    if (!path || !model) return MARS_ERR_INVALID_FILE;
    FILE *fp = fopen(path, "rb");
    if (!fp) {
        fprintf(stderr, "Mars: Cannot open %s\n", path);
        return MARS_ERR_INVALID_FILE;
    }
    fseek(fp, 0, SEEK_END);
    long size = ftell(fp);
    fseek(fp, 0, SEEK_SET);
    if (size <= 0) { fclose(fp); return MARS_ERR_INVALID_FILE; }
    void *buf = malloc((size_t)size);
    if (!buf) { fclose(fp); return MARS_ERR_ALLOC_FAILED; }
    if (fread(buf, 1, (size_t)size, fp) != (size_t)size) { free(buf); fclose(fp); return MARS_ERR_INVALID_FILE; }
    fclose(fp);
    mars_error_t err = mars_load_memory(buf, (size_t)size, model);
    free(buf);
    return err;
}

mars_runtime_tensor_t *mars_get_input(mars_model_t *model, int index) {
    if (!model || index < 0 || (uint32_t)index >= model->header.num_inputs) return NULL;
    uint32_t tid = model->header.input_tensor_ids[index];
    if (tid >= model->header.num_tensors) return NULL;
    return &model->tensors[tid];
}

mars_runtime_tensor_t *mars_get_output(mars_model_t *model, int index) {
    if (!model || index < 0 || (uint32_t)index >= model->header.num_outputs) return NULL;
    uint32_t tid = model->header.output_tensor_ids[index];
    if (tid >= model->header.num_tensors) return NULL;
    return &model->tensors[tid];
}

int mars_get_num_inputs(mars_model_t *model) { return model ? (int)model->header.num_inputs : 0; }
int mars_get_num_outputs(mars_model_t *model) { return model ? (int)model->header.num_outputs : 0; }

void mars_print_summary(mars_model_t *model) {
    if (!model) return;
    mars_model_ext_t *m = (mars_model_ext_t *)model;
    printf("\nMars model summary (MI355X)\n");
    printf("Layers: %u\n", model->header.num_layers);
    printf("Tensors: %u\n", model->header.num_tensors);
    printf("Inputs: %u\n", model->header.num_inputs);
    printf("Outputs: %u\n", model->header.num_outputs);
    printf("Weights: %zu bytes\n", model->weights_size);
    printf("Launches per run: %d, batch %d, activations %zu bytes, parameters %zu bytes\n\n", m->n_ops, m->batch,
           m->act_bytes, m->arena_size);
}
```

### thingino-accel_amd/csrc/host/mars_plan.c

```c
#include <math.h>
#include <stdio.h>
#include <stdlib.h>
#include <string.h>
#include <time.h>

#include "mars_internal.h"
#include "nna.h"

int32_t mars_trunc_x86(float x) {
    if (x >= -2147483648.0f && x < 2147483648.0f) return (int32_t)x;
    return INT32_MIN;
}
static int sat8(int32_t v) { return v > 127 ? 127 : (v < -128 ? -128 : v); }
static int q_half_up(float v) { return sat8(mars_trunc_x86(v + 0.5f)); }

size_t elem_size(uint32_t dtype) {
    switch (dtype) {
        case MARS_DTYPE_FLOAT32: case MARS_DTYPE_INT32: return 4;
        case MARS_DTYPE_INT16: return 2;
        default: return 1;
    }
}

size_t shape_numel(const mars_tensor_t *d) {
// ... 1023 lines not shown
    drop_dead_ops(m);
    free(readers);
}

void pad_output_rows(mars_model_ext_t *m) {
    for (uint32_t i = 0; i < m->pub.header.num_tensors; i++) m->mt[i].pix_c = m->mt[i].pix_stride = 0;
    if (m->sw.no_rowpad) return;
    for (int i = 0; i < m->n_ops; i++) {
        mars_op_t *o = &m->ops[i];
        if (o->kind != OP_CONV_I8 || o->out_nchw || o->out_pix_stride || o->out_ch_off || o->add_t || o->t_out < 0 ||
            (o->out_c & 15) == 0 || (o->in_c & 15) != 0)
            continue;
        mtensor_t *t = &m->mt[o->t_out];
        const int P = (o->out_c + 15) & ~15;
        const size_t px = (size_t)o->out_h * o->out_w;
        if (!t->io_out || t->io_in || P > o->oc_pad || t->bytes != px * (size_t)o->out_c || (px * P) % 256 != 0) continue;
        if (touched_by_other(m, o->t_out, i, i)) continue;
        o->out_pix_stride = P;
        o->store_c = P;
        t->pix_c = o->out_c;
        t->pix_stride = P;
        if (px * P > t->extent) t->extent = px * P;
    }
}

void virtual_concat(mars_model_ext_t *m) {
    const int nt = (int)m->pub.header.num_tensors;
    for (int T = 0; T < nt; T++) {
        const mtensor_t *mt = &m->mt[T];
        if (mt->is_weight || mt->io_in || mt->io_out) continue;
        int sl[4], ns = 0, bad = 0, first_reader = -1, last_reader = -1, last_slice = -1;
        for (int i = 0; i < m->n_ops && !bad; i++) {
            const mars_op_t *o = &m->ops[i];
            if (o->t_out == T) {
                if (o->kind != OP_CONCAT_SLICE || ns >= 4) bad = 1;
                else { sl[ns++] = i; last_slice = i; }
            }
            for (int k = 0; k < o->n_in; k++)
                if (o->t_in[k] == T) {
                    if (o->kind != OP_CONV_I8 || k != 0 || o->n_in != 1 || o->nchw || o->kh != 1 || o->kw != 1 || o->sh != 1 ||
                        o->sw != 1 || o->pt || o->pl || !o->safe || o->nseg || (o->out_c & 15) || o->in_h != o->out_h ||
                        o->in_w != o->out_w || (o->in_c & (o->in_c - 1)) != 0 || o->add_t)
                        bad = 1;
                    if (first_reader < 0) first_reader = i;
                    last_reader = i;
                }
        }
        if (bad || ns < 2 || first_reader < 0 || last_slice > first_reader) continue;
        for (int a = 0; a < ns; a++)
            for (int b = a + 1; b < ns; b++)
                if (m->ops[sl[b]].ch_off < m->ops[sl[a]].ch_off) { int t = sl[a]; sl[a] = sl[b]; sl[b] = t; }
        int c = 0;
        const mars_op_t *s0 = &m->ops[sl[0]];
        for (int a = 0; a < ns && !bad; a++) {
            const mars_op_t *o = &m->ops[sl[a]];
            if (o->ch_off != c || (o->in_c & 31) || o->out_h != s0->out_h || o->out_w != s0->out_w || o->out_c != s0->out_c ||
                o->t_in[0] == T || o->t_in[0] < 0)
                bad = 1;
            c += o->in_c;
            if (!bad && touched_between(m, sl[a] + 1, last_reader + 1, o->t_in[0], USE_WRITE)) bad = 1;
        }
        if (bad || c != s0->out_c) continue;
        for (int i = 0; i < m->n_ops && !bad; i++) {
            const mars_op_t *o = &m->ops[i];
            if (o->kind == OP_CONV_I8 && o->n_in == 1 && o->t_in[0] == T &&
                (o->in_c != c || (size_t)o->in_h * o->in_w != (size_t)s0->out_h * s0->out_w))
                bad = 1;
        }
        if (bad) continue;
        for (int i = 0; i < m->n_ops; i++) {
            mars_op_t *o = &m->ops[i];
            if (o->kind != OP_CONV_I8 || o->n_in != 1 || o->t_in[0] != T) continue;
            o->nseg = ns;
            o->n_in = ns;
            for (int a = 0; a < ns; a++) {
                o->seg_t[a] = o->t_in[a] = m->ops[sl[a]].t_in[0];
                o->seg_c[a] = m->ops[sl[a]].in_c;
            }
        }
        for (int a = 0; a < ns; a++) m->ops[sl[a]].kind = -1;
        m->mt[T].needed = 0;
        for (int a = 0; a < ns; a++) {
            const int S = m->ops[sl[a]].t_in[0];
            int up = -1, nread = 0, nwrite = 0, ok = 1;
            for (int i = 0; i < m->n_ops; i++) {
                const mars_op_t *o = &m->ops[i];
                if (o->kind == -1) continue;
                if (o->t_out == S) { nwrite++; up = i; }
                for (int k = 0; k < o->n_in; k++)
                    if (o->t_in[k] == S && !(o->kind == OP_CONV_I8 && o->nseg == ns && o->seg_t[a] == S)) nread++;
            }
            if (nwrite != 1 || nread != 0 || up < 0 || m->mt[S].io_out || m->mt[S].io_in || m->mt[S].is_weight) continue;
            const mars_op_t *u = &m->ops[up];
            if (u->kind != OP_UPSAMPLE || u->out_pix_stride || u->scale_h != 2 || u->scale_w != 2 || u->out_h != 2 * u->in_h ||
                u->out_w != 2 * u->in_w || u->in_c != m->ops[sl[a]].in_c || u->out_h != s0->out_h || u->out_w != s0->out_w)
                continue;
            const int U = u->t_in[0];
            if (U < 0 || U == S) continue;
            int last = -1;
            for (int i = 0; i < m->n_ops; i++)
                if (m->ops[i].kind == OP_CONV_I8 && m->ops[i].nseg == ns && m->ops[i].seg_t[a] == S) last = i;
            for (int i = up; i <= last && ok; i++)
                if (m->ops[i].kind != -1 && m->ops[i].t_out == U) ok = 0;
            if (!ok) continue;
            for (int i = 0; i < m->n_ops; i++) {
                mars_op_t *o = &m->ops[i];
                if (o->kind == OP_CONV_I8 && o->nseg == ns && o->seg_t[a] == S) {
                    o->seg_t[a] = o->t_in[a] = U;
                    o->seg_up |= 1 << a;
                }
            }
            m->ops[up].kind = -1;
            m->mt[S].needed = 0;
        }
    }
    drop_dead_ops(m);
}

static int same_conv_input(const mars_op_t *a, const mars_op_t *b) {
    if (a->n_in != b->n_in || a->nseg != b->nseg || a->seg_up != b->seg_up) return 0;
    for (int k = 0; k < a->n_in; k++)
        if (a->t_in[k] != b->t_in[k]) return 0;
    for (int k = 0; k < a->nseg; k++)
        if (a->seg_t[k] != b->seg_t[k] || a->seg_c[k] != b->seg_c[k]) return 0;
    return a->in_h == b->in_h && a->in_w == b->in_w && a->in_c == b->in_c && a->out_h == b->out_h && a->out_w == b->out_w &&
           a->kh == b->kh && a->kw == b->kw && a->sh == b->sh && a->sw == b->sw && a->pt == b->pt && a->pl == b->pl &&
           a->row_pad == b->row_pad && a->oc_pad == b->oc_pad;
}
static int pairable(const mars_op_t *o) {
    return o->kind == OP_CONV_I8 && !o->nchw && !o->out_nchw && !o->add_t && !o->nseg && o->safe && o->lut_off != NO_OFF && !o->pair_next &&
           (o->in_c & 15) == 0 && o->in_c > 4 && (o->out_c & 15) == 0 && !o->out_pix_stride;
}
static int pair_up(mars_model_ext_t *m, int i, int j) {
    const mars_op_t *b = &m->ops[j];
    if (touched_between(m, i + 1, j, b->t_out, USE_READ | USE_WRITE)) return 0;
    for (int k = 0; k < b->n_in; k++)
        if (touched_between(m, i + 1, j, b->t_in[k], USE_WRITE)) return 0;
    const mars_op_t moved = *b;
    memmove(&m->ops[i + 2], &m->ops[i + 1], sizeof(mars_op_t) * (size_t)(j - i - 1));
    m->ops[i + 1] = moved;
    m->ops[i].pair_next = 1;
    return 1;
}
void pair_convs(mars_model_ext_t *m) {
    for (int i = 0; i + 1 < m->n_ops; i++) {
        mars_op_t *a = &m->ops[i];
        if (!pairable(a) || (i > 0 && m->ops[i - 1].pair_next)) continue;
        for (int j = i + 1; j < m->n_ops && j <= i + 48; j++) {
            mars_op_t *b = &m->ops[j];
            if (!pairable(b) || !same_conv_input(a, b) || b->t_out == a->t_out) continue;
            if (op_reads(b, b->t_out) || op_reads(b, a->t_out)) continue;
            if (pair_up(m, i, j)) break;
        }
    }
}

static int pairable_f32(const mars_op_t *o) {
    return o->kind == OP_CONV_F32 && !o->add_t && o->n_in == 1 && o->w2_off != NO_OFF && o->w3_off == NO_OFF && !o->pair_next && !o->in_rec && !o->out_rec &&
           o->kh == 1 && o->kw == 1;
}
void pair_convs_f32(mars_model_ext_t *m) {
    if (m->sw.no_pair_f32) return;
    for (int i = 0; i + 1 < m->n_ops; i++) {
        mars_op_t *a = &m->ops[i];
        if (!pairable_f32(a) || (i > 0 && m->ops[i - 1].pair_next)) continue;
        for (int j = i + 1; j < m->n_ops && j <= i + 48; j++) {
            mars_op_t *b = &m->ops[j];
            if (!pairable_f32(b) || b->t_in[0] != a->t_in[0] || b->t_out == a->t_out || b->t_out < 0 || a->t_out < 0) continue;
            if (a->in_h != b->in_h || a->in_w != b->in_w || a->in_c != b->in_c || a->out_h != b->out_h || a->out_w != b->out_w || a->out_c != b->out_c ||
                a->sh != b->sh || a->sw != b->sw || a->pt != b->pt || a->pl != b->pl || a->silu_f32 != b->silu_f32 || a->f32_exact != b->f32_exact)
                continue;
            if (planned_stride(&m->mt[a->t_out]) != planned_stride(&m->mt[b->t_out])) continue;
            if (a->w2_planes != b->w2_planes) continue;
            int ok = b->t_in[0] != b->t_out && b->t_in[0] != a->t_out;
            for (int q = i + 1; q < j && ok; q++)
                if (m->ops[q].pair_next) ok = 0;
            if (ok && pair_up(m, i, j)) break;
        }
    }
}

void fuse_pool_chains(mars_model_ext_t *m) {
    for (int i = 0; i + 1 < m->n_ops; i++) {
        mars_op_t *a = &m->ops[i];
        if (a->kind != OP_MAXPOOL || a->chain_n || a->sh != 1 || a->sw != 1 || a->out_pix_stride || (a->in_c & 15) ||
            a->out_h != a->in_h || a->out_w != a->in_w || a->kh <= 0 || a->kw <= 0 || (size_t)a->in_h * a->in_w * 64 > 60 * 1024 ||
            a->t_out < 0 || m->mt[a->t_out].io_out)
            continue;
        int n = 1;
        a->chain_out[0] = a->t_out;
        while (n < 3 && i + n < m->n_ops) {
            const mars_op_t *b = &m->ops[i + n];
            if (b->kind != OP_MAXPOOL || b->t_in[0] != a->chain_out[n - 1] || b->sh != 1 || b->sw != 1 || b->out_pix_stride ||
                b->in_c != a->in_c || b->in_h != a->in_h || b->in_w != a->in_w || b->out_h != a->in_h || b->out_w != a->in_w ||
                b->kh != a->kh || b->kw != a->kw || b->t_out < 0 || m->mt[b->t_out].io_out || b->t_out == a->t_in[0])
                break;
            a->chain_out[n] = b->t_out;
            n++;
        }
        if (n < 2) continue;
        a->chain_n = n;
        for (int k = 1; k < n; k++) {
            a->bytes += m->ops[i + k].bytes - (double)a->in_h * a->in_w * a->in_c;
            m->ops[i + k].kind = -1;
        }
        a->t_out = a->chain_out[n - 1];
    }
    drop_dead_ops(m);
}

void rec_pairs(mars_model_ext_t *m) {
    const int nt = (int)m->pub.header.num_tensors;
    for (int i = 0; i < nt; i++) m->mt[i].rec_c = m->mt[i].rec_hw = 0;
    m->rec_skipped = 0;
    m->rec_max_frames = (size_t)-1;
    if (m->sw.fusion < 1 || m->sw.no_rec || m->plan_f32_mode != 3) return;
    const size_t frames = m->rec_frames > 0 ? (size_t)m->rec_frames : 1, lim = m->sw.rec_limit;
    int *readers, *writers;
    if (!use_counts(m, &readers, &writers)) return;
    for (int j = 0; j < m->n_ops; j++) {
        mars_op_t *x = &m->ops[j];
        if (x->kind != OP_CONV_F32 || x->w3_off == NO_OFF || x->w3_stem || x->n_in != (x->add_t ? 2 : 1) || x->in_rec) continue;
        const int T = x->t_in[0];
        if (T < 0 || readers[T] != 1 || writers[T] != 1 || m->mt[T].io_in || m->mt[T].io_out || m->mt[T].is_weight) continue;
        if (x->add_t && x->add_t - 1 == T) continue;
        const int i = writer_before(m, T, j);
        if (i < 0) continue;
        mars_op_t *pr = &m->ops[i];
        if (pr->kind != OP_CONV_F32 || pr->add_t || pr->out_rec || (pr->out_c & 7) || pr->kh > 32 || pr->kw > 32) continue;
        if (pr->pair_next || (i > 0 && m->ops[i - 1].pair_next)) continue;
        if (pr->out_c != x->in_c || pr->out_h != x->in_h || pr->out_w != x->in_w) continue;
        if (!(pr->w2_off != NO_OFF || (pr->w3_off != NO_OFF && pr->w3_stem))) continue;
        if (pr->w2_off != NO_OFF && mhip_conv_f32_split_takes(pr->out_c, pr->in_c, pr->kh, pr->kw, pr->sh, pr->sw, pr->pl, pr->in_w, pr->out_w) < 0) continue;
        if (x->add_t && planned_stride(&m->mt[x->add_t - 1]) != planned_stride(&m->mt[x->t_out])) continue;
        if (m->mt[T].bytes != (size_t)x->in_c * x->in_h * x->in_w * 4) continue;
        const int form = mhip_conv_f32_patch_rec_form(x->out_c, x->in_c, x->kh, x->kw, x->sw, x->pl, x->in_h, x->in_w, x->out_h, x->out_w);
        if (!form) continue;
        if (form == 1) {
            const size_t n0 = mhip_conv_f32_patch_pack2(x->out_c, x->in_c, x->kh, x->kw, x->sw, x->pl, x->in_h, x->in_w, x->out_h, x->out_w, 0, NULL, NULL);
            const size_t n1 = mhip_conv_f32_patch_pack2(x->out_c, x->in_c, x->kh, x->kw, x->sw, x->pl, x->in_h, x->in_w, x->out_h, x->out_w, 1, NULL, NULL);
            if (!n1 || n1 != n0) continue;
        }
        {
            const int tt[3] = {pr->t_in[0], T, x->t_out};
            size_t worst = 0;
            for (int q = 0; q < 3; q++)
                if (tt[q] >= 0 && planned_stride(&m->mt[tt[q]]) > worst) worst = planned_stride(&m->mt[tt[q]]);
            if (worst && worst * frames > lim) {
                m->rec_skipped = 1;
                continue;
            }
            if (worst && lim / worst < m->rec_max_frames) m->rec_max_frames = lim / worst;
        }
        if (form == 1 && !m->deferred)
            mhip_conv_f32_patch_pack2(x->out_c, x->in_c, x->kh, x->kw, x->sw, x->pl, x->in_h, x->in_w, x->out_h, x->out_w, 1,
                                      (const float *)(m->arena_host + x->w_off), m->arena_host + x->w3_off);
        x->in_rec = form;
        pr->out_rec = 1;
        m->mt[T].rec_c = x->in_c;
        m->mt[T].rec_hw = x->in_h * x->in_w;
    }
    free(readers);
}

void zero_tail_f32(mars_model_ext_t *m) {
    const int nt = (int)m->pub.header.num_tensors;
    for (int i = 0; i < nt; i++) m->mt[i].zero_from = 0;
    for (int i = 0; i < m->n_ops; i++) m->ops[i].k_limit = 0;
    if (m->sw.fusion < 1 || m->sw.no_zero_tail) return;
    for (int j = 0; j < m->n_ops; j++) {
        mars_op_t *x = &m->ops[j];
        if (x->kind != OP_CONV_F32 || x->kh != 1 || x->kw != 1 || x->sh != 1 || x->sw != 1 || x->pt || x->pl || x->in_rec || x->w2_off == NO_OFF) continue;
        const int T = x->t_in[0];
        if (T < 0 || m->mt[T].is_weight || m->mt[T].io_in || m->pub.tensors[T].desc.dtype != MARS_DTYPE_FLOAT32) continue;
        if (m->mt[T].bytes != (size_t)x->in_c * x->in_h * x->in_w * 4) continue;
        size_t written = 0;
        int ok = 1, nw = 0;
        for (int q = 0; q < m->n_ops && ok; q++) {
            const mars_op_t *o = &m->ops[q];
            if (!op_writes(o, T)) continue;
            if (o->kind != OP_CONCAT_SLICE || o->out_pix_stride) { ok = 0; break; }
            nw++;
            const size_t npix = (size_t)o->out_h * o->out_w;
            if (npix && o->in_c > 0) {
                const size_t end = (npix - 1) * (size_t)o->out_c + (size_t)o->ch_off + (size_t)o->in_c;
                if (end > written) written = end;
            }
        }
        if (!ok || !nw || !written) continue;
        const size_t plane = (size_t)x->in_h * x->in_w * 4;
        const size_t kl = (written + plane - 1) / plane;
        if (kl >= (size_t)x->in_c) continue;
        if (!m->deferred) {
            const float *w = (const float *)(m->arena_host + x->w_off);
            int finite = 1;
            for (int oc = 0; oc < x->out_c && finite; oc++)
                for (int ic = (int)kl; ic < x->in_c; ic++) {
                    const float v = w[(size_t)oc * x->in_c + ic];
                    if (!(v - v == 0.0f)) { finite = 0; break; }
                }
            if (!finite) continue;
        }
        x->k_limit = (int)kl;
        if (!m->mt[T].zero_from || written > m->mt[T].zero_from) m->mt[T].zero_from = written;
        x->macs = (double)x->out_h * x->out_w * x->out_c * (double)kl;
        x->bytes = ((double)x->in_h * x->in_w * (double)kl + (double)x->out_h * x->out_w * x->out_c) * 4.0;
// ... 13 lines not shown
        if (N < 2 || N > 4 || T < 0 || m->mt[T].io_in || m->mt[T].io_out || m->mt[T].is_weight || m->pub.tensors[T].desc.dtype != MARS_DTYPE_FLOAT32) continue;
        const mars_op_t *last = &m->ops[e];
        const int Wb = last->in_c;
        if (Wb <= 0 || (Wb & 3) || last->out_c != Wb || last->ch_off != (N - 1) * Wb || last->out_pix_stride || last->out_h <= 0 || last->out_w <= 0) continue;
        const int TL = last->t_in[0];
        const size_t Lb = (size_t)last->out_h * last->out_w * (size_t)Wb, sB = (size_t)(N - 1) * (size_t)Wb;
        if (TL < 0 || TL == T || m->mt[TL].is_weight || m->mt[TL].io_in || m->mt[TL].io_out  || m->mt[TL].rec_c || m->mt[TL].nhwc_c || m->mt[TL].pix_stride || m->mt[TL].bytes < Lb ||
            m->pub.tensors[TL].desc.dtype != MARS_DTYPE_FLOAT32 || sB > 256)
            continue;
        int ok = 1, firsts[3] = {-1, -1, -1};
        for (int k = 0; k < N - 1 && ok; k++) {
            const mars_op_t *sl = &m->ops[first_op + k];
            const int ti = sl->t_in[0];
            if (sl->in_c != Wb || sl->out_c != Wb || sl->ch_off != k * Wb || sl->out_h != 1 || sl->out_w != 1 || sl->out_pix_stride || ti < 0 || ti == T ||
                m->mt[ti].is_weight || m->mt[ti].rec_c || m->mt[ti].nhwc_c || m->mt[ti].bytes < (size_t)Wb)
                ok = 0;
            firsts[k] = ti;
        }
        if (!ok) continue;
        int r1 = -1, nr = 0;
        for (int j = 0; j < m->n_ops && ok; j++) {
            const mars_op_t *o = &m->ops[j];
            if (j >= first_op && j <= e) continue;
            if (op_writes(o, T)) ok = 0;
            for (int k = 0; k < o->n_in; k++)
                if (o->t_in[k] == T) {
                    if (k != 0 || j <= e) ok = 0;
                    if (r1 < 0) r1 = j;
                    nr++;
                }
        }
        if (!ok || r1 < 0 || nr > 2) continue;
        const int paired = m->ops[r1].pair_next ? 1 : 0;
        if (nr != 1 + paired || (r1 > 0 && m->ops[r1 - 1].pair_next) || (paired && (r1 + 1 >= m->n_ops || m->ops[r1 + 1].t_in[0] != T))) continue;
        const int rl = r1 + paired;
        size_t km = 0, worst = 0;
        for (int j = r1; j <= rl && ok; j++) {
            const mars_op_t *x = &m->ops[j];
            if (x->kind != OP_CONV_F32 || x->k_limit <= 0 || x->n_in != 1 || x->add_t || x->in_rec || x->vc_shift || x->kh != 1 || x->kw != 1 || x->sh != 1 || x->sw != 1 ||
                x->pt || x->pl || x->w2_off == NO_OFF || x->in_h != x->out_h || x->in_w != x->out_w || x->t_out == TL || x->t_out == T || x->t_out < 0) { ok = 0; break; }
            const size_t hw = (size_t)x->in_h * x->in_w, Pb = hw * 4;
            if (m->mt[T].bytes != (size_t)x->in_c * Pb || Lb % Pb || sB / 4 >= hw) { ok = 0; break; }
            km = Lb / Pb;
            if (km < 1 || (size_t)x->k_limit != km + 1 || km + 1 > (size_t)x->in_c) { ok = 0; break; }
            if (x->out_rec && (x->out_c & 7)) { ok = 0; break; }
            for (int k = 0; k < N - 1; k++)
                if (x->t_out == firsts[k]) ok = 0;
            const size_t st = planned_stride(&m->mt[x->t_out]);
            if (st > worst) worst = st;
        }
        if (!ok) continue;
        ok = !touched_between(m, e + 1, rl + 1, TL, USE_WRITE);
        for (int k = 0; k < N - 1 && ok; k++) ok = !touched_between(m, e + 1, rl + 1, firsts[k], USE_WRITE);
        if (!ok) continue;
        if (planned_stride(&m->mt[TL]) > worst) worst = planned_stride(&m->mt[TL]);
        if (worst * (frames + 3) > lim) {
            m->rec_skipped = 1;
            continue;
        }
        if (lim / worst - 3 < m->rec_max_frames) m->rec_max_frames = lim / worst - 3;
        if (!m->deferred) {
            for (int j = r1; j <= rl && ok; j++) {
                const mars_op_t *x = &m->ops[j];
                const float *w = (const float *)(m->arena_host + x->w_off);
                for (int oc = 0; oc < x->out_c; oc++) {
                    const float v = w[(size_t)oc * x->in_c + km];
                    if (!(v - v == 0.0f)) { ok = 0; break; }
                }
            }
            if (!ok) continue;
        }
        const int heads = 1 + paired;
        size_t wt_off[2] = {NO_OFF, NO_OFF};
        for (int q = 0; q < heads; q++) {
            const mars_op_t *x = &m->ops[r1 + q];
            wt_off[q] = arena_reserve(m, mhip_conv_f32_vcat_pack(x->out_c, x->in_c, (int)km + 1, NULL, NULL));
            if (wt_off[q] == NO_OFF) return;
            if (!m->deferred)
                mhip_conv_f32_vcat_pack(x->out_c, x->in_c, (int)km + 1, (const float *)(m->arena_host + x->w_off), (float *)(m->arena_host + wt_off[q]));
        }
        while (m->n_ops + heads > m->cap_ops) {
            const int cap = m->cap_ops * 2;
            mars_op_t *np = (mars_op_t *)realloc(m->ops, (size_t)cap * sizeof(mars_op_t));
            if (!np) { m->plan_err = MARS_ERR_ALLOC_FAILED; return; }
            m->ops = np; m->cap_ops = cap;
        }
        memmove(&m->ops[rl + 1 + heads], &m->ops[rl + 1], sizeof(mars_op_t) * (size_t)(m->n_ops - rl - 1));
        m->n_ops += heads;
        for (int q = 0; q < heads; q++) {
            mars_op_t *x = &m->ops[r1 + q], *h = &m->ops[rl + 1 + q];
            const double hw = (double)x->in_h * x->in_w;
            x->t_in[0] = TL;
            x->vc_shift = (int)sB;
            x->k_limit = (int)km;
            x->macs = hw * x->out_c * (double)km;
            x->bytes = (hw * (double)km + hw * x->out_c) * 4.0;
            *h = *x;
            h->kind = OP_CONV_F32_VHEAD;
            h->pair_next = 0; h->vc_shift = 0;
            h->k_limit = (int)km + 1;
            h->vc_n = N - 1; h->vc_run = Wb / 4;
            h->n_in = N;
            for (int k = 0; k < N - 1; k++) { h->vc_t[k] = firsts[k]; h->t_in[1 + k] = firsts[k]; }
            h->macs = (double)(sB / 4) * x->out_c * (double)(km + 1);
            h->bytes = ((double)(sB / 4) * (double)(km + 1) + (double)(sB / 4) * x->out_c) * 4.0;
            h->variant = 0;
            h->w3_off = wt_off[q]; h->w3_stem = 0;
            h->w2_off = NO_OFF; h->w2_planes = 0;
        }
        memmove(&m->ops[first_op], &m->ops[e + 1], sizeof(mars_op_t) * (size_t)(m->n_ops - e - 1));
        m->n_ops -= N;
        m->mt[T].needed = 0;
        m->mt[T].partial = 1;
        m->mt[T].zero_from = 0;
        i = first_op - 1;
    }
}

void f32_policy(mars_model_ext_t *m) {
    const int nt = (int)m->pub.header.num_tensors;
    unsigned char *hot = (unsigned char *)calloc((size_t)nt + 1, 1);
    if (!hot) {
        for (int i = 0; i < m->n_ops; i++) m->ops[i].f32_exact = 1;
        return;
    }
    for (int i = m->n_ops - 1; i >= 0; i--) {
        mars_op_t *o = &m->ops[i];
        int reach = 0;
        if (o->kind == OP_MAXPOOL && o->t_in[0] >= 0 && m->pub.tensors[o->t_in[0]].desc.dtype == MARS_DTYPE_FLOAT32) reach = 1;
        if (o->kind == OP_RELU_BYTES && o->t_out >= 0) {
            hot[o->t_out] = 1;
            continue;
        }
        if (o->t_out >= 0 && hot[o->t_out]) reach = 1;
        for (int k = 0; k < o->chain_n; k++)
            if (o->chain_out[k] >= 0 && hot[o->chain_out[k]]) reach = 1;
        if (!reach) continue;
        for (int k = 0; k < o->n_in; k++)
            if (o->t_in[k] >= 0) hot[o->t_in[k]] = 1;
        if (o->kind == OP_CONV_F32) o->f32_exact = 1;
    }
    free(hot);
}

void plan_check(mars_model_ext_t *m) {
    for (int i = 0; i < m->n_ops; i++) {
        const mars_op_t *o = &m->ops[i];
        const char *why = NULL;
        if (o->kind == -1) why = "a dead op is left";
        else if (o->n_in < 0 || o->n_in > 4 || o->nseg < 0 || o->nseg > 4 || o->chain_n < 0 || o->chain_n > 3 || o->vc_n < 0 || o->vc_n > 3) why = "an operand count is out of range";
        else if (o->add_t && !op_reads(o, o->add_t - 1)) why = "add_t is not among t_in";
        else if (o->chain_n && o->t_out != o->chain_out[o->chain_n - 1]) why = "t_out is not the chain's last stage";
        else if (o->pair_next && (i + 1 >= m->n_ops || m->ops[i + 1].kind != o->kind)) why = "pair_next without a mate of its kind";
        for (int k = 0; !why && k < o->nseg; k++)
            if (!op_reads(o, o->seg_t[k])) why = "a seg_t is not among t_in";
        for (int k = 0; !why && k < o->vc_n; k++)
            if (!op_reads(o, o->vc_t[k])) why = "a vc_t is not among t_in";
        if (!why) continue;
        VLOG("plan_check: op %d (layer %d, kind %d): %s\n", i, o->layer, o->kind, why);
        m->plan_err = MARS_ERR_LAYER_FAILED;
        return;
    }
}
```

### thingino-accel_amd/csrc/host/mars_run.c

```c
#include <math.h>
#include <stdio.h>
#include <stdlib.h>
#include <string.h>
#include <time.h>

#include "mars_internal.h"
#include "nna.h"

static int g_graph_max_batch = 8;
static unsigned g_tune_gen = 1;
static int g_dual_min_batch = 64;
static int g_dual_ways = 2;
static uint8_t *tdev(const mars_model_ext_t *m, int ti) {
    if (ti < 0 || !m->mt[ti].dev) return NULL;
    return m->mt[ti].dev + (m->mt[ti].is_weight ? 0 : (size_t)m->frame0 * m->mt[ti].stride);
}
static size_t tstride(const mars_model_ext_t *m, int ti) { return ti >= 0 ? m->mt[ti].stride : 0; }

void conv_i8_params(const mars_model_ext_t *m, const mars_op_t *op, mhip_conv_i8_t *p) {
    uint8_t *A = m->arena_dev;
    conv_i8_geometry(op, m->run_frames, p);
    p->in = (const int8_t *)tdev(m, op->t_in[0]); p->in_stride = tstride(m, op->t_in[0]);
    p->out = (int8_t *)tdev(m, op->t_out); p->out_stride = tstride(m, op->t_out);
    if (p->in) p->in += op->in_byte_off;
// ... 127 lines not shown
            return mhip_binary_i8(op->is_mul, (const int8_t *)tdev(m, op->t_in[0]), tstride(m, op->t_in[0]),
                                  (const int8_t *)tdev(m, op->t_in[1]), tstride(m, op->t_in[1]),
                                  (int8_t *)tdev(m, op->t_out), tstride(m, op->t_out), B, op->n, op->f0, op->f1, op->f2,
                                  op->out_pix_stride ? op->in_c : 0, op->out_pix_stride, op->out_ch_off);
        case OP_SIGMOID_F32:
            return mhip_sigmoid_f32((const float *)tdev(m, op->t_in[0]), tstride(m, op->t_in[0]),
                                    (float *)tdev(m, op->t_out), tstride(m, op->t_out), B, op->n);
        case OP_RELU_F32:
            return mhip_relu_f32((const float *)tdev(m, op->t_in[0]), tstride(m, op->t_in[0]), (float *)tdev(m, op->t_out),
                                 tstride(m, op->t_out), B, op->n, op->f0);
        case OP_BINARY_F32:
            return mhip_binary_f32(op->is_mul ? 1 : 0, (const float *)tdev(m, op->t_in[0]), tstride(m, op->t_in[0]),
                                   (const float *)tdev(m, op->t_in[1]), tstride(m, op->t_in[1]),
                                   (float *)tdev(m, op->t_out), tstride(m, op->t_out), B, op->n);
        case OP_BN: {
            const float *s = op->s_off != NO_OFF ? (const float *)(A + op->s_off) : NULL;
            const float *b = op->b_off != NO_OFF ? (const float *)(A + op->b_off) : NULL;
            if (op->is_f32)
                return mhip_batchnorm_f32((const float *)tdev(m, op->t_in[0]), tstride(m, op->t_in[0]),
                                          (float *)tdev(m, op->t_out), tstride(m, op->t_out), B, op->bn_n, op->in_c,
                                          op->in_h * op->in_w, s, b);
            return mhip_batchnorm_i8((const int8_t *)tdev(m, op->t_in[0]), tstride(m, op->t_in[0]),
                                     (int8_t *)tdev(m, op->t_out), tstride(m, op->t_out), B, op->bn_n, op->in_c,
                                     op->in_h * op->in_w, s, b, op->f0, op->f1);
        }
        case OP_MAXPOOL:
            if (op->chain_n) {
                int8_t *outs[3] = {NULL, NULL, NULL};
                size_t strides[3] = {0, 0, 0};
                for (int k = 0; k < op->chain_n; k++) {
                    outs[k] = (int8_t *)tdev(m, op->chain_out[k]);
                    strides[k] = tstride(m, op->chain_out[k]);
                }
                return mhip_pool_chain_i8((const int8_t *)tdev(m, op->t_in[0]), tstride(m, op->t_in[0]), outs, strides,
                                          op->chain_n, B, op->in_h, op->in_w, op->in_c, op->kh, op->kw);
            }
            return mhip_maxpool_i8((const int8_t *)tdev(m, op->t_in[0]), tstride(m, op->t_in[0]), (int8_t *)tdev(m, op->t_out),
                                   tstride(m, op->t_out), B, op->in_h, op->in_w, op->in_c, op->out_h, op->out_w, op->kh,
                                   op->kw, op->sh, op->sw, op->out_pix_stride, op->out_ch_off);
        case OP_CONCAT_SLICE:
            return mhip_concat_slice((const int8_t *)tdev(m, op->t_in[0]), tstride(m, op->t_in[0]),
                                     (int8_t *)tdev(m, op->t_out), tstride(m, op->t_out), B, op->out_h, op->out_w,
                                     op->in_c, op->out_c, op->ch_off);
        case OP_UPSAMPLE_Q: {
            const mars_tensor_t *id = &m->pub.tensors[op->t_in[0]].desc, *od = &m->pub.tensors[op->t_out].desc;
            return mhip_upsample_nchwq((const int8_t *)tdev(m, op->t_in[0]), tstride(m, op->t_in[0]), id->shape[1], id->shape[2], id->shape[3],
                                       (int8_t *)tdev(m, op->t_out), tstride(m, op->t_out), od->shape[1], od->shape[2], od->shape[3], B, op->in_h, op->in_w,
                                       op->in_c, op->out_h, op->out_w, op->scale_h, op->scale_w);
        }
        case OP_MAXPOOL_Q: {
            const mars_tensor_t *id = &m->pub.tensors[op->t_in[0]].desc;
            return mhip_maxpool_nchwq((const int8_t *)tdev(m, op->t_in[0]), tstride(m, op->t_in[0]), (int8_t *)tdev(m, op->t_out), tstride(m, op->t_out), B,
                                      id->shape[1], id->shape[2], id->shape[3], op->kh, op->kw);
        }
        case OP_CONCAT_Q: {
            const int8_t *ins[4];
            size_t strides[4];
            int cs[4];
            for (int k = 0; k < op->n_in && k < 4; k++) {
                ins[k] = (const int8_t *)tdev(m, op->t_in[k]);
                strides[k] = tstride(m, op->t_in[k]);
                cs[k] = m->mt[op->t_in[k]].nhwc_c;
            }
            return mhip_concat_nchwq(ins, strides, cs, op->n_in, (int8_t *)tdev(m, op->t_out), tstride(m, op->t_out), B, op->out_c, op->in_h, op->in_w,
                                     op->rows_only);
        }
        case OP_UPSAMPLE:
            return mhip_upsample_i8((const int8_t *)tdev(m, op->t_in[0]), tstride(m, op->t_in[0]),
                                    (int8_t *)tdev(m, op->t_out), tstride(m, op->t_out), B, op->in_h, op->in_w, op->in_c,
                                    op->out_h, op->out_w, op->scale_h, op->scale_w, op->out_pix_stride, op->out_ch_off);
        default: return -1;
    }
}

static mars_error_t enqueue_plan(mars_model_t *model);
static double now_us(void);
static int tune_raw(const char *key, int value, int *get);

static void tune_push(mars_model_ext_t *m) {
    if (m->tune_depth++ || !m->n_tune) return;
    for (int i = 0; i < m->n_tune; i++) {
        tune_raw(m->tune[i].key, 0, &m->tune[i].saved);
        tune_raw(m->tune[i].key, m->tune[i].value, NULL);
    }
}
static void tune_pop(mars_model_ext_t *m) {
    if (--m->tune_depth || !m->n_tune) return;
    for (int i = m->n_tune - 1; i >= 0; i--) tune_raw(m->tune[i].key, m->tune[i].saved, NULL);
}
static mars_error_t run_device_async(mars_model_t *model);
mars_error_t mars_hip_run_device_async(mars_model_t *model) {
    if (!model) return MARS_ERR_INVALID_FILE;
    tune_push((mars_model_ext_t *)model);
    mars_error_t e = run_device_async(model);
    tune_pop((mars_model_ext_t *)model);
    return e;
}

static mars_error_t run_device_async(mars_model_t *model) {
    mars_model_ext_t *m = (mars_model_ext_t *)model;
    if (!m->act_dev || !m->arena_dev) return MARS_ERR_NNA_INIT_FAILED;
    int graphable = g_graph_max_batch > 0 && m->batch <= g_graph_max_batch && !m->profiling && !m->pipe;
    for (int i = 0; i < m->n_ops && graphable; i++)
        if (m->ops[i].kind == OP_FAIL) graphable = 0;
    if (!graphable) return enqueue_plan(model);
    if (m->graph_exec && m->graph_gen != g_tune_gen) {
        drop_graph(m);
        m->ran_plain = 0;
    }
    if (!m->graph_exec) {
        if (!m->ran_plain) {
            mars_error_t e = enqueue_plan(model);
            if (e == MARS_OK) m->ran_plain = 1;
            return e;
        }
        if (m->tail_pending) {
            mhip_select_stream(0);
            if (mhip_stream_wait(0, m->ev_tail_done)) return MARS_ERR_LAYER_FAILED;
            m->tail_pending = 0;
        }
        if (mhip_graph_begin() == 0) {
            mars_error_t e = enqueue_plan(model);
            m->graph_exec = mhip_graph_end(e == MARS_OK);
            m->graph_gen = g_tune_gen;
            if (e != MARS_OK) { m->graph_exec = NULL; return e; }
        }
        VLOG("plan of %d launches at batch %d %s\n", m->n_ops, m->batch, m->graph_exec ? "captured into a HIP graph" : "could not be captured");
        if (!m->graph_exec) {
            g_graph_max_batch = 0;
            return enqueue_plan(model);
        }
    }
    if (m->tail_pending) {
        mhip_select_stream(0);
        if (mhip_stream_wait(0, m->ev_tail_done)) return MARS_ERR_LAYER_FAILED;
        m->tail_pending = 0;
    }
    if (mhip_graph_launch(m->graph_exec)) return MARS_ERR_LAYER_FAILED;
    for (uint32_t i = 0; i < model->header.num_layers; i++) model->layers[i].is_executed = true;
    return MARS_OK;
}

static mars_error_t enqueue_range(mars_model_ext_t *m, int sid, int wait_tail) {
    void *prof_last = NULL;
    mhip_select_stream(sid);
    m->scratch_t = -1;
    for (int i = 0; i < m->n_ops; i++) {
        mars_op_t *op = &m->ops[i];
        if (op->kind == OP_FAIL) {
            fprintf(stderr, "Mars: Layer %d execution failed\n", op->layer);
            return (mars_error_t)op->err;
        }
        mars_op_t *mate = op->pair_next && i + 1 < m->n_ops ? &m->ops[i + 1] : NULL;
        if (wait_tail && ((op->t_out >= 0 && (m->mt[op->t_out].io_out || m->mt[op->t_out].tail_read)) ||
                          (mate && mate->t_out >= 0 && (m->mt[mate->t_out].io_out || m->mt[mate->t_out].tail_read)))) {
            mhip_stream_wait(sid, m->ev_tail_done);
            wait_tail = 0;
        }
        if (m->profiling) {
            if (!op->ev1) op->ev1 = mhip_event_create();
            if (!prof_last) {
                if (!op->ev0) op->ev0 = mhip_event_create();
                mhip_event_record(op->ev0);
                prof_last = op->ev0;
            }
            op->ev_start = prof_last;
        }
        int rc;
        if (mate && op->kind == OP_CONV_F32) {
            mhip_conv_f32_t pa, pb;
            conv_f32_params(m, op, &pa);
            conv_f32_params(m, mate, &pb);
            rc = mhip_conv_f32_pair(&pa, &pb);
            if (rc == -2) {
                rc = launch_op(m, op);
                if (!rc) rc = launch_op(m, mate);
            }
            i++;
        } else if (mate) {
            mhip_conv_i8_t pa, pb;
            conv_i8_params(m, op, &pa);
            conv_i8_params(m, mate, &pb);
            rc = mhip_conv_i8_pair(&pa, &pb);
            if (rc == -2) {
                rc = launch_op(m, op);
                if (!rc) rc = launch_op(m, mate);
            }
            i++;
        } else {
            rc = launch_op(m, op);
        }
        {
            const mars_op_t *w2[2] = {op, mate};
            for (int q = 0; q < 2; q++)
                if (w2[q] && op_writes(w2[q], m->scratch_t)) m->scratch_t = -1;
        }
        if (m->profiling) {
            const int nx = i + 1;
            const int end = m->profiling != 2 || nx >= m->n_ops || m->ops[nx].prof_kind != op->prof_kind;
            op->prof_rec = end;
            if (end) {
                mhip_event_record(op->ev1);
                prof_last = op->ev1;
            }
        }
        if (rc != 0) {
            fprintf(stderr, "Mars: Layer %d launch failed: %s\n", op->layer, mhip_last_error());
            return MARS_ERR_LAYER_FAILED;
        }
    }
    return MARS_OK;
}

static mars_error_t enqueue_plan(mars_model_t *model) {
    mars_model_ext_t *m = (mars_model_ext_t *)model;
    for (uint32_t i = 0; i < model->header.num_layers; i++) model->layers[i].is_executed = false;
    const int B = m->batch;
    int dual = g_dual_min_batch > 0 && B >= g_dual_min_batch && B >= 2 && !m->profiling &&
               !(g_graph_max_batch > 0 && B <= g_graph_max_batch);
    if (dual) {
        if (!m->ev_fork) m->ev_fork = mhip_event_create_sync();
        for (int k = 0; k < 3; k++) {
            if (!m->ev_join[k]) m->ev_join[k] = mhip_event_create_sync();
            if (!m->ev_join[k]) dual = 0;
        }
        if (!m->ev_fork) dual = 0;
    }
    mars_error_t e;
    if (!dual) {
        m->frame0 = 0; m->run_frames = B;
        e = enqueue_range(m, 0, m->tail_pending);
    } else {
        const int ways = g_dual_ways < B ? g_dual_ways : B;
        mhip_select_stream(0);
        int rc = mhip_event_record(m->ev_fork);
        for (int k = 1; k < ways && !rc; k++) rc = mhip_stream_wait(3 + k, m->ev_fork);
        if (rc) return MARS_ERR_LAYER_FAILED;
        e = MARS_OK;
        int f0 = 0;
        for (int k = 0; k < ways && e == MARS_OK; k++) {
            const int n = (B - f0 + (ways - k) - 1) / (ways - k);
            m->frame0 = f0; m->run_frames = n;
            e = enqueue_range(m, k ? 3 + k : 0, m->tail_pending);
            f0 += n;
        }
        for (int k = 1; k < ways; k++) {
            mhip_select_stream(3 + k);
            rc = mhip_event_record(m->ev_join[k - 1]);
            if (!rc) rc = mhip_stream_wait(0, m->ev_join[k - 1]);
            if (rc && e == MARS_OK) e = MARS_ERR_LAYER_FAILED;
        }
    }
    mhip_select_stream(0);
    m->frame0 = 0; m->run_frames = B;
    if (e != MARS_OK) return e;
    m->tail_pending = 0;
    for (uint32_t i = 0; i < model->header.num_layers; i++) model->layers[i].is_executed = true;
    return MARS_OK;
}

static double now_us(void) {
    struct timespec ts;
    clock_gettime(CLOCK_MONOTONIC, &ts);
    return ts.tv_sec * 1e6 + ts.tv_nsec * 1e-3;
}

mars_error_t mars_hip_run_device(mars_model_t *model) {
    double t0 = now_us();
    mars_error_t e = mars_hip_run_device_async(model);
    if (e != MARS_OK) { mhip_sync(); return e; }
    if (mhip_sync()) return MARS_ERR_LAYER_FAILED;
    mars_model_ext_t *m = (mars_model_ext_t *)model;
    if (m->profiling)
        for (int i = 0; i < m->n_ops; i++)
            m->ops[i].last_ms = (m->ops[i].prof_rec && m->ops[i].ev_start && m->ops[i].ev1) ? mhip_event_elapsed_ms(m->ops[i].ev_start, m->ops[i].ev1) : 0.f;
    model->total_inference_us += (uint64_t)(now_us() - t0);
    model->inference_count++;
    return MARS_OK;
}

static mars_error_t enqueue_upload_frames(mars_model_ext_t *m, int f0, int n) {
    for (uint32_t i = 0; i < m->pub.header.num_tensors; i++) {
        mtensor_t *t = &m->mt[i];
        if (!t->io_in || !t->host || !t->dev || t->bytes == 0) continue;
        if (mhip_h2d_2d_async(t->dev + (size_t)f0 * t->stride, t->stride, (const uint8_t *)t->host + (size_t)f0 * t->bytes, t->bytes,
                              t->bytes, (size_t)n))
            return MARS_ERR_LAYER_FAILED;
    }
    return MARS_OK;
}
static mars_error_t enqueue_upload(mars_model_ext_t *m) { return enqueue_upload_frames(m, 0, m->batch); }

static mars_error_t enqueue_download_frames(mars_model_ext_t *m, int f0, int n) {
    for (uint32_t i = 0; i < m->pub.header.num_tensors; i++) {
        mtensor_t *t = &m->mt[i];
        if (!t->io_out || !t->host || !t->dev || t->bytes == 0) continue;
        uint8_t *host = (uint8_t *)t->host + (size_t)f0 * t->bytes;
        if (t->pix_stride) {
            const size_t rows = (t->bytes / (size_t)t->pix_c) * (size_t)n;
            if (!t->dense_dev || t->stride != (t->bytes / (size_t)t->pix_c) * (size_t)t->pix_stride) return MARS_ERR_LAYER_FAILED;
            uint8_t *dense = (uint8_t *)t->dense_dev + (size_t)f0 * t->bytes;
            if (mhip_unpad_rows(t->dev + (size_t)f0 * t->stride, dense, rows, t->pix_c, t->pix_stride) ||
                mhip_d2h_async(host, dense, t->bytes * (size_t)n))
                return MARS_ERR_LAYER_FAILED;
            continue;
        }
        if (mhip_d2h_2d_async(host, t->bytes, t->dev + (size_t)f0 * t->stride, t->stride, t->bytes, (size_t)n)) return MARS_ERR_LAYER_FAILED;
    }
    return MARS_OK;
}
static mars_error_t enqueue_download(mars_model_ext_t *m) { return enqueue_download_frames(m, 0, m->batch); }

mars_error_t mars_hip_upload_inputs(mars_model_t *model) {
    if (!model) return MARS_ERR_INVALID_FILE;
    mars_error_t e = enqueue_upload((mars_model_ext_t *)model);
    if (mhip_sync() && e == MARS_OK) e = MARS_ERR_LAYER_FAILED;
    return e;
}

mars_error_t mars_hip_download_outputs(mars_model_t *model) {
    if (!model) return MARS_ERR_INVALID_FILE;
    mars_error_t e = enqueue_download((mars_model_ext_t *)model);
    if (mhip_sync() && e == MARS_OK) e = MARS_ERR_LAYER_FAILED;
    return e;
}

static int g_run_chunk = 128;
static mars_error_t run_chunked(mars_model_ext_t *m) {
    mars_model_t *model = &m->pub;
    const int B = m->batch;
    int nch = (B + g_run_chunk - 1) / g_run_chunk;
    if (nch > 8) nch = 8;
    for (int k = 0; k < 2; k++)
        for (int c = 0; c < nch; c++)
            if (!m->ev_chunk[k][c] && !(m->ev_chunk[k][c] = mhip_event_create_sync())) return MARS_ERR_ALLOC_FAILED;
    for (uint32_t i = 0; i < model->header.num_layers; i++) model->layers[i].is_executed = false;
    mars_error_t e = MARS_OK;
    mhip_select_stream(0);
    if (mhip_event_record(m->ev_chunk[1][nch - 1]) || mhip_stream_wait(2, m->ev_chunk[1][nch - 1])) e = MARS_ERR_LAYER_FAILED;
    int f0 = 0;
    mhip_select_stream(2);
    for (int c = 0; c < nch && e == MARS_OK; c++) {
        const int n = (B - f0 + (nch - c) - 1) / (nch - c);
        e = enqueue_upload_frames(m, f0, n);
        if (e == MARS_OK && mhip_event_record(m->ev_chunk[0][c])) e = MARS_ERR_LAYER_FAILED;
        f0 += n;
    }
    f0 = 0;
// ... 32 lines not shown
static mars_error_t run_whole(mars_model_t *model) {
    mars_model_ext_t *m = (mars_model_ext_t *)model;
    if (!m->act_dev || !m->arena_dev) return MARS_ERR_NNA_INIT_FAILED;
    const double t0 = now_us();
    mars_error_t e;
    int chunked = g_run_chunk > 0 && m->batch >= 2 * g_run_chunk && !m->profiling && !m->pipe;
    for (int i = 0; i < m->n_ops && chunked; i++)
        if (m->ops[i].kind == OP_FAIL) chunked = 0;
    if (chunked) {
        e = run_chunked(m);
    } else {
        e = enqueue_upload(m);
        if (e == MARS_OK) e = mars_hip_run_device_async(model);
        if (e == MARS_OK && !m->no_download) e = enqueue_download(m);
    }
    if (mhip_sync() && e == MARS_OK) e = MARS_ERR_LAYER_FAILED;
    if (e != MARS_OK) return e;
    if (m->profiling)
        for (int i = 0; i < m->n_ops; i++)
            m->ops[i].last_ms = (m->ops[i].prof_rec && m->ops[i].ev_start && m->ops[i].ev1) ? mhip_event_elapsed_ms(m->ops[i].ev_start, m->ops[i].ev1) : 0.f;
    model->total_inference_us += (uint64_t)(now_us() - t0);
    model->inference_count++;
    return MARS_OK;
}

mars_error_t mars_hip_sync(void) { return mhip_sync() ? MARS_ERR_LAYER_FAILED : MARS_OK; }


mars_error_t mars_hip_set_batch(mars_model_t *model, int n) {
    if (!model || n <= 0 || n > 65535) return MARS_ERR_INVALID_FILE;
    return alloc_batch((mars_model_ext_t *)model, n);
}

int mars_hip_get_batch(const mars_model_t *model) { return model ? ((const mars_model_ext_t *)model)->batch : 0; }

mars_error_t mars_hip_set_output_mode(mars_model_t *model, int mode) {
    if (!model || (mode != MARS_HIP_OUTPUT_HEADS && mode != MARS_HIP_OUTPUT_ON_DEVICE)) return MARS_ERR_INVALID_FILE;
    ((mars_model_ext_t *)model)->no_download = mode == MARS_HIP_OUTPUT_ON_DEVICE;
    return MARS_OK;
}

mars_error_t mars_hip_set_fusion(mars_model_t *model, int level) {
    if (!model) return MARS_ERR_INVALID_FILE;
    mars_model_ext_t *m = (mars_model_ext_t *)model;
    if (m->deferred) return MARS_ERR_INVALID_FILE;
    mhip_sync();
    m->sw.fusion = level;
    mars_error_t e = build_plan(m);
    if (e == MARS_OK) e = upload_params(m);
    if (e == MARS_OK) e = alloc_batch(m, m->batch > 0 ? m->batch : 1);
    return e;
}

static int tune_raw(const char *key, int value, int *get) {
    if (!key) return -1;
    struct { const char *k; int *v; int lo, hi; } tab[] = {
        {"graph_max_batch", &g_graph_max_batch, 0, 1 << 30},
        {"dual_stream_min_batch", &g_dual_min_batch, 0, 1 << 30},
        {"run_chunk", &g_run_chunk, 0, 1 << 30},
        {"dual_stream_ways", &g_dual_ways, 2, 4},
    };
    for (size_t i = 0; i < sizeof tab / sizeof tab[0]; i++)
        if (!strcmp(key, tab[i].k)) {
            if (get) { *get = *tab[i].v; return 0; }
            if (value < tab[i].lo || value > tab[i].hi) return -1;
            *tab[i].v = value;
            return 0;
        }
    if (!strcmp(key, "f32_mfma")) {
        if (get) { *get = mhip_conv_f32_mode(-1); return 0; }
        if (value < 0 || value > 4) return -1;
        mhip_conv_f32_mode(value);
        return 0;
    }
    return get ? mhip_conv_i8_tune_get(key, get) : mhip_conv_i8_tune(key, value);
}

static mars_error_t replan_for_f32_mode(mars_model_ext_t *m) {
    if (m->deferred || !m->arena_dev) return MARS_OK;
    int has_f32 = 0;
    for (int i = 0; i < m->n_ops && !has_f32; i++) has_f32 = m->ops[i].kind == OP_CONV_F32;
    if (!has_f32) return MARS_OK;
    tune_push(m);
    const int mode = mhip_conv_f32_mode(-1);
    mars_error_t e = MARS_OK;
    if (mode != m->plan_f32_mode && (mode >= 3 || m->plan_f32_mode >= 3)) {
        mhip_sync();
        e = build_plan(m);
        if (e == MARS_OK) e = upload_params(m);
        if (e == MARS_OK) e = alloc_batch(m, m->batch > 0 ? m->batch : 1);
    }
    tune_pop(m);
    return e;
}

int mars_hip_set_tuning(const char *key, int value) {
    g_tune_gen++;
    int rc = tune_raw(key, value, NULL);
    if (rc == 0 && key && !strcmp(key, "f32_mfma"))
        for (mars_model_ext_t *m = mars_live_models(); m; m = m->live_next)
            if (replan_for_f32_mode(m) != MARS_OK) rc = -1;
    return rc;
}

int mars_hip_get_tuning(const char *key, int *value) { return value ? tune_raw(key, 0, value) : -1; }

int mars_hip_model_set_tuning(mars_model_t *model, const char *key, int value) {
    mars_model_ext_t *m = (mars_model_ext_t *)model;
    int cur;
    if (!m || !key || strlen(key) >= sizeof m->tune[0].key || tune_raw(key, 0, &cur)) return -1;
    if (tune_raw(key, value, NULL)) return -1;
    tune_raw(key, cur, NULL);
    int i = 0;
    while (i < m->n_tune && strcmp(m->tune[i].key, key)) i++;
    if (i == m->n_tune) {
        if (m->n_tune == MARS_MAX_MODEL_TUNE) return -1;
        strcpy(m->tune[m->n_tune++].key, key);
    }
    m->tune[i].value = value;
    drop_graph(m);
    if (!strcmp(key, "f32_mfma") && replan_for_f32_mode(m) != MARS_OK) return -1;
    return 0;
}

int mars_hip_model_get_tuning(mars_model_t *model, const char *key, int *value) {
    mars_model_ext_t *m = (mars_model_ext_t *)model;
    if (!m || !key || !value) return -1;
    for (int i = 0; i < m->n_tune; i++)
        if (!strcmp(m->tune[i].key, key)) { *value = m->tune[i].value; return 0; }
    return tune_raw(key, 0, value);
}

static mars_error_t autotune_model(mars_model_t *model, int reps);
mars_error_t mars_hip_autotune(mars_model_t *model, int reps) {
    if (!model) return MARS_ERR_INVALID_FILE;
    tune_push((mars_model_ext_t *)model);
    mars_error_t e = autotune_model(model, reps);
    tune_pop((mars_model_ext_t *)model);
    return e;
}
static mars_error_t autotune_model(mars_model_t *model, int reps) {
    mars_model_ext_t *m = (mars_model_ext_t *)model;
    if (!m->act_dev || !m->arena_dev) return MARS_ERR_NNA_INIT_FAILED;
    drop_graph(m);
    if (reps <= 0) reps = 3;
    void *e0 = mhip_event_create(), *e1 = mhip_event_create();
    if (!e0 || !e1) return MARS_ERR_ALLOC_FAILED;
    mars_error_t err = MARS_OK;
    if (mhip_sync()) err = MARS_ERR_LAYER_FAILED;
    for (int i = 0; i < m->n_ops && err == MARS_OK; i++) {
        mars_op_t *op = &m->ops[i];
        if (op->kind != OP_CONV_I8 || op->nchw) continue;
        if (op->pair_next || (i > 0 && m->ops[i - 1].pair_next)) continue;
        mhip_conv_i8_t p;
        conv_i8_params(m, op, &p);
        int codes[32];
        const int n = mhip_conv_i8_variants(&p, codes, 32);
        if (getenv("MARS_VERBOSE") && atoi(getenv("MARS_VERBOSE")) > 1)
            fprintf(stderr, "Mars: autotune layer %d: %dx%dx%d -> %dx%dx%d k%dx%d s%d pixstride %d choff %d lut %d safe %d\n", op->layer,
                    p.in_h, p.in_w, p.in_c, p.out_h, p.out_w, p.out_c, p.kh, p.kw, p.stride_w, p.out_pix_stride, p.out_ch_off,
                    p.lut != NULL, p.safe);
        float best = 0.0f;
        int best_code = 0;
        for (int k = 0; k < n && err == MARS_OK; k++) {
            p.variant = codes[k];
            int rc = mhip_conv_i8(&p);
            if (!rc) rc = mhip_event_record(e0);
            for (int r = 0; r < reps && !rc; r++) rc = mhip_conv_i8(&p);
            if (!rc) rc = mhip_event_record(e1);
            if (rc || mhip_sync()) { err = MARS_ERR_LAYER_FAILED; break; }
            const float ms = mhip_event_elapsed_ms(e0, e1);
            if (getenv("MARS_VERBOSE") && atoi(getenv("MARS_VERBOSE")) > 1)
                fprintf(stderr, "Mars: autotune layer %d: candidate %d: %.1f us\n", op->layer, codes[k], ms * 1000.0f / reps);
            if (best_code == 0 || ms < best) { best = ms; best_code = codes[k]; }
        }
        if (err == MARS_OK && best_code) {
            if (getenv("MARS_VERBOSE"))
                fprintf(stderr, "Mars: autotune layer %d: variant %d (%.1f us) of %d candidates, default %d\n", op->layer,
                        best_code, best * 1000.0f / reps, n, n ? codes[0] : 0);
            op->variant = best_code;
        }
    }
    mhip_event_destroy(e0);
    mhip_event_destroy(e1);
    return err;
}

void *mars_hip_tensor_device(mars_model_t *model, int ti, size_t *frame_stride) {
    if (!model || ti < 0 || (uint32_t)ti >= model->header.num_tensors) return NULL;
    mars_model_ext_t *m = (mars_model_ext_t *)model;
    if (frame_stride) *frame_stride = m->mt[ti].stride;
    return m->mt[ti].dev;
}

size_t mars_hip_tensor_frame_bytes(const mars_model_t *model, int ti) {
    if (!model || ti < 0 || (uint32_t)ti >= model->header.num_tensors) return 0;
    return ((const mars_model_ext_t *)model)->mt[ti].bytes;
}

int mars_hip_tensor_row_pitch(mars_model_t *model, int ti, int *row_bytes) {
    if (!model || ti < 0 || (uint32_t)ti >= model->header.num_tensors) return 0;
    const mtensor_t *t = &((mars_model_ext_t *)model)->mt[ti];
    if (row_bytes) *row_bytes = t->pix_stride ? t->pix_c : 0;
    return t->pix_stride;
}

mars_error_t mars_hip_read_tensor(mars_model_t *model, int ti, int frame, void *dst, size_t bytes) {
    if (!model || !dst || ti < 0 || (uint32_t)ti >= model->header.num_tensors) return MARS_ERR_INVALID_TENSOR;
    mars_model_ext_t *m = (mars_model_ext_t *)model;
    mtensor_t *t = &m->mt[ti];
    if (!t->dev || frame < 0 || (!t->is_weight && frame >= m->batch)) return MARS_ERR_INVALID_TENSOR;
    if (!t->is_weight && bytes > t->stride) return MARS_ERR_INVALID_TENSOR;
    if (t->partial) return MARS_ERR_INVALID_TENSOR;
    if (t->is_weight) {
        const size_t off = (size_t)m->pub.tensors[ti].desc.data_offset;
        if (off > m->blob_mirror_bytes || bytes > m->blob_mirror_bytes - off) return MARS_ERR_INVALID_TENSOR;
        frame = 0;
    }
    if (mhip_sync()) return MARS_ERR_LAYER_FAILED;
    if (t->rec_c) {
        const size_t full = (size_t)t->rec_c * t->rec_hw * 4;
        uint8_t *raw = (uint8_t *)malloc(full);
        float *f = (float *)malloc(full);
        if (!raw || !f || bytes > full || mhip_d2h_async(raw, t->dev + (size_t)frame * t->stride, full) || mhip_sync()) {
            free(raw); free(f);
            return MARS_ERR_LAYER_FAILED;
        }
        for (int c = 0; c < t->rec_c; c++)
            for (int px = 0; px < t->rec_hw; px++) {
                const uint8_t *r = raw + ((size_t)(c >> 3) * t->rec_hw + px) * 32 + (size_t)(c & 7) * 2;
                uint16_t h, md;
                memcpy(&h, r, 2); memcpy(&md, r + 16, 2);
                const uint32_t hb = (uint32_t)h << 16, mb = (uint32_t)md << 16;
                float hf, mf;
                memcpy(&hf, &hb, 4); memcpy(&mf, &mb, 4);
                f[(size_t)c * t->rec_hw + px] = hf + mf;
            }
        memcpy(dst, f, bytes);
        free(raw); free(f);
        return MARS_OK;
    }
    if (t->nhwc_c) {
        const size_t full = (size_t)t->nhwc_c * t->nhwc_hw, pitch = t->nhwc_pitch ? (size_t)t->nhwc_pitch : (size_t)t->nhwc_c, dev_b = pitch * t->nhwc_hw;
        uint8_t *raw = (uint8_t *)malloc(dev_b), *pl = (uint8_t *)malloc(full);
        if (!raw || !pl || bytes > full || dev_b > t->stride || mhip_d2h_async(raw, t->dev + (size_t)frame * t->stride, dev_b) || mhip_sync()) {
            free(raw); free(pl);
            return MARS_ERR_LAYER_FAILED;
        }
        for (int px = 0; px < t->nhwc_hw; px++)
            for (int c = 0; c < t->nhwc_c; c++) pl[(size_t)c * t->nhwc_hw + px] = raw[(size_t)px * pitch + c];
        memcpy(dst, pl, bytes);
        free(raw); free(pl);
        return MARS_OK;
    }
    if (t->pix_stride) {
        uint8_t *dense = t->dense_dev + (size_t)frame * t->bytes;
        if (bytes > t->bytes || !t->dense_dev) return MARS_ERR_INVALID_TENSOR;
        if (mhip_unpad_rows(t->dev + (size_t)frame * t->stride, dense, t->bytes / (size_t)t->pix_c, t->pix_c, t->pix_stride) ||
            mhip_d2h_async(dst, dense, bytes) || mhip_sync())
            return MARS_ERR_LAYER_FAILED;
        return MARS_OK;
    }
    if (mhip_d2h_async(dst, t->dev + (size_t)frame * t->stride, bytes) || mhip_sync()) return MARS_ERR_LAYER_FAILED;
    return MARS_OK;
}

mars_error_t mars_hip_write_tensor(mars_model_t *model, int ti, int frame, const void *src, size_t bytes) {
    if (!model || !src || ti < 0 || (uint32_t)ti >= model->header.num_tensors) return MARS_ERR_INVALID_TENSOR;
    mars_model_ext_t *m = (mars_model_ext_t *)model;
    mtensor_t *t = &m->mt[ti];
    if (!t->dev || t->is_weight || frame < 0 || frame >= m->batch || bytes > t->stride) return MARS_ERR_INVALID_TENSOR;
    if (t->rec_c) {
        const size_t full = (size_t)t->rec_c * t->rec_hw * 4;
        if (bytes != full) return MARS_ERR_INVALID_TENSOR;
        uint8_t *raw = (uint8_t *)calloc(1, full);
        if (!raw) return MARS_ERR_ALLOC_FAILED;
        const float *f = (const float *)src;
        for (int c = 0; c < t->rec_c; c++)
            for (int px = 0; px < t->rec_hw; px++) {
                float x, hv, r;
                memcpy(&x, &f[(size_t)c * t->rec_hw + px], 4);
                uint32_t b;
                memcpy(&b, &x, 4);
                const uint16_t h = (b & 0x7fffffffu) > 0x7f800000u ? (uint16_t)((b >> 16) | 0x40u) : (uint16_t)((b + 0x7fffu + ((b >> 16) & 1u)) >> 16);
                const uint32_t hb = (uint32_t)h << 16;
                memcpy(&hv, &hb, 4);
                r = hv - hv == 0.0f ? x - hv : 0.0f;
                memcpy(&b, &r, 4);
                const uint16_t md = (b & 0x7fffffffu) > 0x7f800000u ? (uint16_t)((b >> 16) | 0x40u) : (uint16_t)((b + 0x7fffu + ((b >> 16) & 1u)) >> 16);
                uint8_t *q = raw + ((size_t)(c >> 3) * t->rec_hw + px) * 32 + (size_t)(c & 7) * 2;
                memcpy(q, &h, 2); memcpy(q + 16, &md, 2);
            }
        const int rc = mhip_h2d_async(t->dev + (size_t)frame * t->stride, raw, full) || mhip_sync();
        free(raw);
        return rc ? MARS_ERR_LAYER_FAILED : MARS_OK;
    }
    if (t->zero_from && bytes > t->zero_from) {
        const uint8_t *b = (const uint8_t *)src;
        for (size_t i = t->zero_from; i < bytes; i++)
            if (b[i]) return MARS_ERR_INVALID_TENSOR;
    }
    if (t->nhwc_c) {
        const size_t full = (size_t)t->nhwc_c * t->nhwc_hw, pitch = t->nhwc_pitch ? (size_t)t->nhwc_pitch : (size_t)t->nhwc_c, dev_b = pitch * t->nhwc_hw;
        if (bytes != full || dev_b > t->stride) return MARS_ERR_INVALID_TENSOR;
        uint8_t *raw = (uint8_t *)calloc(1, dev_b);
        if (!raw) return MARS_ERR_ALLOC_FAILED;
// ... 50 lines not shown
```

### thingino-accel_amd/csrc/mhip.h

```cpp
#ifndef MHIP_H
#define MHIP_H

#include <stddef.h>
#include <stdint.h>

#ifdef __cplusplus
extern "C" {
#endif

int mhip_init(int device_hint);
void mhip_shutdown(void);
int mhip_ready(void);
int mhip_device_info(int *cu_count, int *lds_bytes, int *gfx_version, size_t *hbm_bytes);
void *mhip_stream(void);
int mhip_sync(void);
void mhip_select_aux(int on);
void mhip_select_stream(int which);
int mhip_stream_wait(int which, void *ev);
int mhip_event_sync(void *ev);
void *mhip_malloc(size_t bytes);
void mhip_free(void *p);
void *mhip_host_alloc(size_t bytes);
void mhip_host_free(void *p);
int mhip_memset_async(void *dst, int value, size_t bytes);
int mhip_h2d_async(void *dst, const void *src, size_t bytes);
int mhip_d2h_async(void *dst, const void *src, size_t bytes);
int mhip_d2d_async(void *dst, const void *src, size_t bytes);
int mhip_h2d_2d_async(void *dst, size_t dpitch, const void *src, size_t spitch, size_t row_bytes, size_t rows);
int mhip_d2h_2d_async(void *dst, size_t dpitch, const void *src, size_t spitch, size_t row_bytes, size_t rows);
void *mhip_event_create(void);
void *mhip_event_create_sync(void);
void mhip_event_destroy(void *ev);
int mhip_event_record(void *ev);
float mhip_event_elapsed_ms(void *start, void *stop);
const char *mhip_last_error(void);
int mhip_graph_begin(void);
void *mhip_graph_end(int ok);
int mhip_graph_launch(void *exec);
void mhip_graph_destroy(void *exec);

typedef struct {
    const int8_t *in;  size_t in_stride;
    int8_t *out;       size_t out_stride;
    const int8_t *w;
    const int32_t *bias;
    const uint8_t *lut;
    const uint8_t *lut2;
    const int8_t *pre_w;
    const int32_t *pre_bias;
    const uint8_t *pre_lut2;
    float pre_cs;
    const int8_t *w_rgb;
    const int8_t *w_rows;
    int frames;
    int in_h, in_w, in_c;
    int out_h, out_w, out_c;
    int kh, kw, stride_h, stride_w, pad_top, pad_left;
    int row_pad;
    int oc_pad;
    float cs;
    int relu;
    int out_nchw;
    int in_planar;
    int safe;
    int out_pix_stride;
    int out_ch_off;
    int variant;
    const int8_t *add;
    float add_s_conv, add_s_other, add_inv;
    int nseg;
    const int8_t *seg_in[4];
    size_t seg_stride[4];
    int seg_c[4], seg_c0[4];
    int seg_up;
} mhip_conv_i8_t;
int mhip_conv_i8_oc_row(int oc, int oc_pad);
int mhip_conv_i8_pre_ok(const mhip_conv_i8_t *p);
size_t mhip_conv_i8_rgb_pack(int in_c, int kh, int kw, int stride_h, int stride_w, int pad_left, int oc_pad, int k64,
                             const int8_t *packed, int8_t *out);
size_t mhip_conv_i8_rows_pack(int in_c, int kh, int kw, int stride_h, int stride_w, int oc_pad, int k64, int out_w,
                              const int8_t *packed, int8_t *out);
unsigned long mhip_conv_i8_rows_launches(void);
int mhip_conv_i8_is_safe(float cs);
int mhip_conv_i8_lut2_ok(float cs);
int mhip_conv_i8_tune(const char *key, int value);
int mhip_conv_i8_tune_get(const char *key, int *value);
int mhip_conv_i8_variants(const mhip_conv_i8_t *p, int *codes, int max);
int mhip_conv_i8_seg_ok(const mhip_conv_i8_t *p);
int mhip_conv_i8_pair(const mhip_conv_i8_t *a, const mhip_conv_i8_t *b);
int mhip_conv_i8_small_c(int in_c, int kw, int out_c);
void mhip_conv_i8_pack_geom(int in_c, int kw, int out_c, int *row_pad, int *oc_pad, int *c_eff);
int mhip_conv_i8(const mhip_conv_i8_t *p);

typedef struct {
    const float *in;  size_t in_stride;
    float *out;       size_t out_stride;
    const float *w;   const float *bias;
    const void *w_split;
    const void *w_patch;
    int frames;
    int in_h, in_w, in_c, out_h, out_w, out_c;
    int kh, kw, stride_h, stride_w, pad_top, pad_left;
    int silu;
    const float *add; size_t add_stride;
    int use_mfma;
    int k_limit;
    int k_limit_required;
    int in_rec, out_rec;
} mhip_conv_f32_t;
int mhip_conv_f32(const mhip_conv_f32_t *p);
size_t mhip_conv_f32_vcat_pack(int out_c, int in_c, int planes, const float *w, float *out);
int mhip_conv_f32_vcat_head(const mhip_conv_f32_t *p, const float *w_t, const float *const *first, const size_t *first_strides, int n_first, int run_floats);
int mhip_conv_f32_pair(const mhip_conv_f32_t *a, const mhip_conv_f32_t *b);
unsigned long mhip_conv_f32_pair_launches(void);
size_t mhip_conv_f32_split_pack(int out_c, int in_c, int kh, int kw, int stride_w, int planes, const float *w, void *out);
unsigned long mhip_conv_f32_split_launches(void);
int mhip_conv_f32_split_takes(int out_c, int in_c, int kh, int kw, int stride_h, int stride_w, int pad_left, int in_w, int out_w);
size_t mhip_conv_f32_patch_pack(int out_c, int in_c, int kh, int kw, int stride, int pad, int in_h, int in_w, int out_h, int out_w,
                                const float *w, void *out);
size_t mhip_conv_f32_patch_pack2(int out_c, int in_c, int kh, int kw, int stride, int pad, int in_h, int in_w, int out_h, int out_w,
                                 int rec, const float *w, void *out);
int mhip_conv_f32_patch_geom2(int out_c, int in_c, int kh, int kw, int stride, int pad, int in_h, int in_w, int out_h, int out_w,
                              int rec, int *outv, int cap);
unsigned long mhip_conv_f32_prec_launches(void);
unsigned long mhip_conv_f32_recin_launches(void);
int mhip_conv_f32_patch_rec_form(int out_c, int in_c, int kh, int kw, int stride, int pad, int in_h, int in_w, int out_h, int out_w);
int mhip_conv_f32_patch_geom(int out_c, int in_c, int kh, int kw, int stride, int pad, int in_h, int in_w, int out_h, int out_w,
                             int *outv, int cap);
unsigned long mhip_conv_f32_patch_launches(void);
size_t mhip_conv_f32_stem_pack(int out_c, int in_c, int kh, int kw, int stride, int pad, int in_h, int in_w, int out_h, int out_w,
                               const float *w, void *out);
unsigned long mhip_conv_f32_stem_launches(void);
int mhip_conv_f32_mode(int set);

int mhip_lut_i8(const int8_t *in, size_t in_stride, int8_t *out, size_t out_stride, int frames,
                size_t n, const uint8_t *lut_dev);
int mhip_relu_bytes(int8_t *buf, size_t stride, int frames, size_t n);
int mhip_binary_i8(int is_mul, const int8_t *a, size_t a_stride, const int8_t *b, size_t b_stride,
                   int8_t *out, size_t out_stride, int frames, size_t n, float sa, float sb, float inv_so,
                   int out_run, int out_pix_stride, int out_ch_off);
int mhip_sigmoid_f32(const float *in, size_t in_stride, float *out, size_t out_stride, int frames, size_t n);
int mhip_binary_f32(int op , const float *a, size_t a_stride, const float *b,
                    size_t b_stride, float *out, size_t out_stride, int frames, size_t n);
int mhip_relu_f32(const float *in, size_t in_stride, float *out, size_t out_stride, int frames,
                  size_t n, float alpha);
int mhip_batchnorm_i8(const int8_t *in, size_t in_stride, int8_t *out, size_t out_stride, int frames,
                      int n, int c, int hw, const float *s, const float *b, float in_scale, float out_scale);
int mhip_batchnorm_f32(const float *in, size_t in_stride, float *out, size_t out_stride, int frames,
                       int n, int c, int hw, const float *s, const float *b);

int mhip_maxpool_i8(const int8_t *in, size_t in_stride, int8_t *out, size_t out_stride, int frames,
                    int in_h, int in_w, int ch, int out_h, int out_w, int kh, int kw, int sh, int sw,
                    int out_pix_stride, int out_ch_off);
int mhip_pool_chain_i8(const int8_t *in, size_t in_stride, int8_t *const *outs, const size_t *out_strides, int n,
                       int frames, int h, int w, int ch, int kh, int kw);
int mhip_unpad_rows(const void *src, void *dst, size_t rows, int width, int pitch);
int mhip_concat_slice(const int8_t *in, size_t in_stride, int8_t *out, size_t out_stride, int frames,
                      int out_h, int out_w, int in_c, int out_c, int ch_off);
int mhip_concat_nchwq(const int8_t *const *ins, const size_t *in_strides, const int *in_c, int n, int8_t *out, size_t out_stride,
                      int frames, int out_c, int H, int W, int rows_only );
int mhip_upsample_nchwq(const int8_t *in, size_t in_stride, int Ci, int Hi, int Wi, int8_t *out, size_t out_stride, int Co, int Ho, int Wo,
                        int frames, int qih, int qiw, int qch, int qoh, int qow, int sh, int sw);
int mhip_maxpool_nchwq(const int8_t *in, size_t in_stride, int8_t *out, size_t out_stride, int frames, int C, int H, int W, int kh, int kw);
int mhip_upsample_i8(const int8_t *in, size_t in_stride, int8_t *out, size_t out_stride, int frames,
                     int in_h, int in_w, int ch, int out_h, int out_w, int scale_h, int scale_w,
                     int out_pix_stride, int out_ch_off);
int mhip_nchw_to_nhwc_pad(const int8_t *in, size_t in_stride, int8_t *out, size_t out_stride,
                          int frames, int c, int hw, int c_pad);

typedef struct {
    const int8_t *pred[4]; size_t stride[4]; int npred[4];
    int pix_c[4], pix_stride[4];
    const float *lut[4];
    int mono[4];
    int nseg;
    int frames;
    float nms_thresh;
    void *dets;
    int *counts;
    int *raw_counts;
    int do_nms;
} mhip_detect_t;
int mhip_detect(const mhip_detect_t *p);
int mhip_nms_only(void *dets_dev, int *count_dev, int n, float thresh);
typedef struct {
    const int8_t *base[4]; size_t frame_stride[4];
    int h[4], w[4], nc[4];
    int pix_step[4], ch_step[4];
    int stride[4];
    float anchors[4][3][2];
    const float *sig;
    int nheads, frames;
    float conf, nms_thresh;
    void *dets;
    int *counts;
    int *raw_counts;
    int map, px, py;
    float rx, ry;
} mhip_heads_t;
int mhip_detect_heads(const mhip_heads_t *p);
typedef struct {
    const int8_t *box[4], *cls[4]; size_t box_frame_stride[4], cls_frame_stride[4];
    int h[4], w[4], nc[4];
    int box_pix_step[4], box_ch_step[4], cls_pix_step[4], cls_ch_step[4];
    int stride[4];
    int reg_max;
    const float *tab;
    int nheads, frames;
    float conf, nms_thresh;
    void *dets;
    int *counts;
    int *raw_counts;
    int map, px, py;
    float rx, ry;
} mhip_dfl_heads_t;
int mhip_detect_dfl(const mhip_dfl_heads_t *p);

typedef struct {
    const uint8_t *rgb; size_t rgb_stride;
    int8_t *out;        size_t out_stride;
    int frames, w, h, tw, th, nhwc;
    int nw, nh, px, py;
    const int *xstart, *xsrc; const float *xw;
    const int *ystart, *ysrc; const float *yw;
    int max_cols, max_rows;
    int n_xtaps;
    int max_ytaps;
    int form;
} mhip_letterbox_t;
int mhip_letterbox(const mhip_letterbox_t *p);
int mhip_nv12_to_rgb(const uint8_t *nv12, size_t nv12_stride, uint8_t *rgb, size_t rgb_stride, int frames, int w, int h, unsigned flags);
int mhip_letterbox_nv12_fused(const mhip_letterbox_t *p);
int mhip_letterbox_nv12(const mhip_letterbox_t *p, unsigned flags, uint8_t *scratch);

typedef struct {
    const uint8_t *frames; size_t frame_stride;
    int n_frames, w, h, fmt;
    unsigned nv12_flags;
    const void *dets; const int *counts; int det_cap;
    const void *boxes; const int *frame_of_box; int n_boxes;
    float expand, min_conf;
    int min_size, cls_first, cls_count, max_per_frame;
// ... 52 lines not shown
```

Measured before the change: 55610.

## Co-launch up to three independent 1x1 int8 convs in one persistent grid

Adds a grouped persistent conv kernel that takes up to three independent 1x1 int8 convolutions as one launch. Blocks are split among members in proportion to their work, and the shared kernel body moves into an included header. A planner pass finds groups of independent convs that share a tile size, and the runtime launches them together, falling back to separate launches if the group call declines. The aim is to fill the GPU better on small layers and cut launch count and tail idle time, at the cost of fixed STAGES=2, no per-layer autotuned variant, and a larger argument block.

```diff
diff --git a/thingino-accel_amd/csrc/hip/conv_i8.hip b/thingino-accel_amd/csrc/hip/conv_i8.hip
--- a/thingino-accel_amd/csrc/hip/conv_i8.hip
+++ b/thingino-accel_amd/csrc/hip/conv_i8.hip
@@ -334,279 +334,40 @@
                                                             const unsigned out_bytes_first, const conv_out_side_t alt,
                                                             const unsigned noc0, const int bufmode, const unsigned in_bytes,
                                                             const int wres) {
-    ANAT_BEGIN();
-    const int STAGE = wres ? BPX * BK : (BPX + BN) * BK;
-    constexpr int NWN = BN == 128 ? 2 : 1;
-    constexpr int NWM = 4 / NWN;
-    constexpr int WPX = BPX / NWM / 16;
-    constexpr int WOC = BN / NWN / 16;
-    constexpr int XI = BPX / 64;
-    constexpr int LW = BN >= 128 ? 2 : 1;
-    constexpr int L = XI + LW;
-    constexpr int NST = WPX;
-    extern __shared__ __attribute__((aligned(16))) int8_t dynlds[];
-    uint8_t *slut = (uint8_t *)dynlds;
-    int8_t *lds = dynlds + LUTB;
-    lds_base_must_be_zero(dynlds);
-
-    const int tid = threadIdx.x, lane = tid & 63;
-    const int wv = __builtin_amdgcn_readfirstlane(tid >> 6);
-    const unsigned id = xcd_remap(blockIdx.x, noc * ngrp);
-    const unsigned grp = id / noc;
-    unsigned ot = id - grp * noc;
-    mhip_conv_i8_t p = pin;
-    unsigned out_bytes = out_bytes_first;
-    if (PAIR && ot >= noc0) {
-        ot -= noc0;
-        p.lut2 = alt.lut2;
-        p.out = alt.out; p.out_stride = alt.out_stride; p.w = alt.w; p.bias = alt.bias; p.lut = alt.lut;
-        p.out_c = alt.out_c; p.relu = alt.relu; p.out_pix_stride = alt.out_pix_stride; p.out_ch_off = alt.out_ch_off;
-        p.cs = alt.cs;
-        out_bytes = alt.out_bytes;
-    }
-    const int oc0 = (int)ot * BN;
-    const unsigned t0 = (unsigned)(((unsigned long long)grp * npt) / ngrp);
-    const unsigned t1 = (unsigned)(((unsigned long long)(grp + 1) * npt) / ngrp);
-    if (t0 >= t1) return;
-    const unsigned hw = (unsigned)(p.out_h * p.out_w);
-    const int wm = wv % NWM, wn = wv / NWM;
-    const int pxw = wm * (WPX * 16), ocw = wn * (WOC * 16);
-
-    auto packed_row16 = [](int c) { return ((c >> 2) & 1) * 16 + (c >> 3) * 4 + (c & 3); };
-    v4i bias[WOC];
-#pragma unroll
-    for (int s = 0; s < WOC; s++)
-        bias[s] = p.bias ? *(const v4i *)(p.bias + (BN == 16 ? packed_row16((lane >> 4) * 4) : oc0 + ocw + s * 16 + (lane >> 4) * 4)) : (v4i){0, 0, 0, 0};
-    if (HAS_LUT) {
-        if (p.lut2) { if (tid < 128) ((uint32_t *)slut)[tid] = ((const uint32_t *)p.lut2)[tid]; }
-        else if (tid < 64) ((uint32_t *)slut)[tid] = ((const uint32_t *)p.lut)[tid];
-        __syncthreads();
-    }
-    const __amdgpu_buffer_rsrc_t orsrc = __builtin_amdgcn_make_buffer_rsrc(p.out, 0, (int)out_bytes, 0x00020000);
-
-    const int schunk = (lane & 3) ^ (((lane >> 4) & 1) << 1);
-    const int8_t *xwin[XI];
-    unsigned tapmask[XI];
-    unsigned rowf[SEG ? XI : 1], rowrem[SEG ? XI : 1];
-    unsigned rowrem_up[SEG ? XI : 1];
-    int xvoff[XI];
-    auto setup_rows = [&](unsigned tile) {
-#pragma unroll
-        for (int j = 0; j < XI; j++) {
-            const unsigned pix = tile * BPX + wv * (BPX / 4) + j * 16 + (lane >> 2);
-            const bool valid = pix < total_pix;
-            const unsigned f = valid ? fdiv(pix, dhw) : 0u;
-            const unsigned rem = valid ? pix - f * hw : 0u;
-            if (SEG) {
-                rowf[j] = f;
-                rowrem[j] = rem;
-                const unsigned oy = fdiv(rem, dow), ox = rem - oy * (unsigned)p.out_w;
-                rowrem_up[j] = (oy >> 1) * ((unsigned)p.out_w >> 1) + (ox >> 1);
-                tapmask[j] = valid ? 1u : 0u;
-                continue;
-            }
-            const int oy = (int)fdiv(rem, dow), ox = (int)(rem - (unsigned)oy * (unsigned)p.out_w);
-            const int iy0 = oy * p.stride_h - p.pad_top, ix0 = ox * p.stride_w - p.pad_left;
-            xwin[j] = p.in + (size_t)f * p.in_stride + ((long)iy0 * p.in_w + ix0) * p.in_c;
-            xvoff[j] = (int)(f * (unsigned)p.in_stride) + (iy0 * p.in_w + ix0) * p.in_c + schunk * 16;
-            const int kx_lo = ix0 < 0 ? -ix0 : 0, kx_hi = p.in_w - ix0 < p.kw ? p.in_w - ix0 : p.kw;
-            const unsigned colbits = kx_hi > kx_lo ? ((kx_hi >= 32 ? ~0u : (1u << kx_hi) - 1u) & ~((1u << kx_lo) - 1u)) : 0u;
-            unsigned m = 0;
-            for (int r = 0; r < p.kh; r++) {
-                const int iy = iy0 + r;
-                if (iy >= 0 && iy < p.in_h) m |= colbits << (r * p.kw);
-            }
-            tapmask[j] = valid ? m : 0u;
-        }
-    };
-    const int8_t *wsrc[LW];
-    int wq[LW], wvoff[LW];
-#pragma unroll
-    for (int j = 0; j < LW; j++) {
-        wq[j] = BN >= 64 ? wv * LW + j : (BN == 16 ? 0 : (wv & 1));
-        const int wrow = BN == 16 ? packed_row16(lane >> 2) : oc0 + wq[j] * 16 + (lane >> 2);
-        wsrc[j] = p.w + (size_t)wrow * k64 + schunk * 16;
-        wvoff[j] = wrow * k64 + schunk * 16;
-    }
-    const __amdgpu_buffer_rsrc_t xrs = __builtin_amdgcn_make_buffer_rsrc((void *)p.in, 0, (int)in_bytes, 0x00020000);
-    const __amdgpu_buffer_rsrc_t wrs = __builtin_amdgcn_make_buffer_rsrc((void *)p.w, 0, p.oc_pad * k64, 0x00020000);
-    const int taps = p.kh * p.kw;
-    const int nks = k64 / BK;
-
-    auto issue = [&](int ks, int stage) {
-        int8_t *sb = lds + stage * STAGE;
-        const unsigned pos = (unsigned)(ks * BK + schunk * 16);
-        if (SEG) {
-            auto owner = [&](int c) { return (c >= p.seg_c0[1]) + (c >= p.seg_c0[2]) + (c >= p.seg_c0[3]); };
-            const int sa = owner(ks * BK), sb2 = owner(ks * BK + 32);
-            const bool hi = schunk >= 2;
-            const int8_t *base = hi ? p.seg_in[sb2] : p.seg_in[sa];
-            const unsigned fstride = (unsigned)(hi ? p.seg_stride[sb2] : p.seg_stride[sa]);
-            const unsigned segc = (unsigned)(hi ? p.seg_c[sb2] : p.seg_c[sa]);
-            const unsigned coff = pos - (unsigned)(hi ? p.seg_c0[sb2] : p.seg_c0[sa]);
-            const bool up = ((p.seg_up >> (hi ? sb2 : sa)) & 1) != 0;
-            const bool kvalid = (int)pos < p.in_c;
-#pragma unroll
-            for (int j = 0; j < XI; j++) {
-                const bool ok = kvalid & (tapmask[j] != 0u);
-                const int8_t *src = base + (size_t)rowf[j] * fstride + (size_t)(up ? rowrem_up[j] : rowrem[j]) * segc + coff;
-                glds16(ok ? src : zeros, sb + (wv * (BPX / 4) + j * 16) * BK);
-            }
-        } else if (bufmode) {
-            const int utap = (ks * BK) >> lg_inc, urc = (ks * BK) & ((1 << lg_inc) - 1);
-            const int uky = (int)(((unsigned)utap * kw_magic) >> 16), ukx = utap - uky * p.kw;
-            const int ukoff = (uky * p.in_w + ukx) * p.in_c + urc;
-            const bool uvalid = utap < taps;
-#pragma unroll
-            for (int j = 0; j < XI; j++) {
-                const bool ok = uvalid & (((tapmask[j] >> utap) & 1u) != 0u);
-                blds16(xrs, ok ? xvoff[j] + ukoff : -1, 0, sb + (wv * (BPX / 4) + j * 16) * BK);
-            }
-            if (!wres)
-#pragma unroll
-                for (int j = 0; j < LW; j++) blds16(wrs, wvoff[j], ks * BK, sb + BPX * BK + wq[j] * 16 * BK);
-            return;
-        } else {
-            const unsigned tap = pos >> lg_inc;
-            const int rc = (int)(pos & ((1u << lg_inc) - 1u));
-            const int ky = (int)((tap * kw_magic) >> 16);
-            const int kx = (int)tap - ky * p.kw;
-            const bool kvalid = (int)tap < taps;
-            const long koff = ((long)ky * p.in_w + kx) * p.in_c + rc;
-#pragma unroll
-            for (int j = 0; j < XI; j++) {
-                const bool ok = kvalid & ((tapmask[j] >> tap) & 1u);
-                glds16(ok ? xwin[j] + koff : zeros, sb + (wv * (BPX / 4) + j * 16) * BK);
-            }
-        }
-        if (!wres)
-#pragma unroll
-            for (int j = 0; j < LW; j++) glds16(wsrc[j] + ks * BK, sb + BPX * BK + wq[j] * 16 * BK);
-    };
-
-    int8_t *const wres_base = lds + STAGES * STAGE;
-    if (wres)
-        for (int ks = 0; ks < nks; ks++)
-#pragma unroll
-            for (int j = 0; j < LW; j++) glds16(wsrc[j] + ks * BK, wres_base + (ks * BN + wq[j] * 16) * BK);
-    unsigned itile = t0;
-    int iks = 0;
-    int younger[STAGES - 1];
-    setup_rows(t0);
-    int nstage = 0;
-#pragma unroll
-    for (int s = 0; s < STAGES - 1; s++) {
-        int n = 0;
-        if (itile < t1) {
-            issue(iks, nstage);
-            n = wres ? XI : L;
-            if (++iks == nks) {
-                iks = 0;
-                if (++itile < t1) setup_rows(itile);
-            }
-        }
-#pragma unroll
-        for (int i = 0; i < s; i++) younger[i] += n;
-        younger[s] = 0;
-        nstage++;
-    }
-    nstage = STAGES - 1;
-
-    const int frow = lane & 15, fchunk = lane >> 4;
-    const int chan = ocw + (lane >> 4) * (4 * WOC);
-    const int pstride = p.out_pix_stride ? p.out_pix_stride : p.out_c;
-    const int lo = p.relu ? 0 : -128;
-    const uint8_t *lut128 = slut + 128;
-    const bool ragged = (p.out_c % (WOC * 4)) != 0;
-    int stage = 0;
-    ANAT_NOW(1);
-    for (unsigned tile = t0; tile < t1; tile++) {
-        v4i acc[WOC][WPX];
-        for (int ks = 0; ks < nks; ks++) {
-            wait_vmcnt_at_most<(STAGES - 2) * L, NST>(younger[0]);
-            __builtin_amdgcn_s_barrier();
-            asm volatile("" ::: "memory");
-            const int8_t *xs = lds + stage * STAGE, *ws = wres ? wres_base + ks * (BN * BK) : xs + BPX * BK;
-            v4i xb[WPX], wa[WOC];
-#pragma unroll
-            for (int t = 0; t < WPX; t++) xb[t] = *(const v4i *)(xs + lds_off(pxw + t * 16 + frow, fchunk));
-#pragma unroll
-            for (int s = 0; s < WOC; s++) wa[s] = *(const v4i *)(ws + lds_off(ocw + s * 16 + frow, fchunk));
-            int n = 0;
-            if (itile < t1) {
-                issue(iks, nstage);
-                n = wres ? XI : L;
-                if (++iks == nks) {
-                    iks = 0;
-                    if (++itile < t1) setup_rows(itile);
-                }
-            }
-#pragma unroll
-            for (int i = 0; i + 1 < STAGES - 1; i++) younger[i] = younger[i + 1] + n;
-            younger[STAGES - 2] = 0;
-            if (ks == 0) {
-#pragma unroll
-                for (int s = 0; s < WOC; s++)
-#pragma unroll
-                    for (int t = 0; t < WPX; t++) acc[s][t] = __builtin_amdgcn_mfma_i32_16x16x64_i8(wa[s], xb[t], bias[s], 0, 0, 0);
-            } else {
-#pragma unroll
-                for (int s = 0; s < WOC; s++)
-#pragma unroll
-                    for (int t = 0; t < WPX; t++) acc[s][t] = __builtin_amdgcn_mfma_i32_16x16x64_i8(wa[s], xb[t], acc[s][t], 0, 0, 0);
-            }
-            stage = stage + 1 == STAGES ? 0 : stage + 1;
-            nstage = nstage + 1 == STAGES ? 0 : nstage + 1;
-        }
-#ifdef ANATOMY
-        if (tile + 1 == t1) ANAT_NOW(2);
-#endif
-#pragma unroll
-        for (int t = 0; t < WPX; t++) {
-            const unsigned pix = tile * BPX + pxw + t * 16 + (lane & 15);
-            const unsigned f = fdiv(pix, dhw), rem = pix - f * hw;
-            const unsigned off = f * (unsigned)p.out_stride + rem * (unsigned)pstride + (unsigned)(p.out_ch_off + oc0 + chan);
-            const int nvalid = p.out_c - (oc0 + chan);
-            const bool ok = pix < total_pix && nvalid >= WOC * 4;
-            uint32_t pk[WOC];
-            int a[WOC * 4];
-#pragma unroll
-            for (int s = 0; s < WOC; s++)
-#pragma unroll
-                for (int r = 0; r < 4; r++) a[s * 4 + r] = acc[s][t][r];
-            if (HAS_LUT && p.lut2) requant_pack<WOC * 4, HAS_LUT, true, true, false, true>(a, p.cs, lo, lut128, pk);
-            else requant_pack<WOC * 4, HAS_LUT, true, true>(a, p.cs, lo, lut128, pk);
-            const int voff = ok ? (int)off : -1;
-            if (WOC == 4)
-                __builtin_amdgcn_raw_buffer_store_b128((v4i){(int)pk[0], (int)pk[1], (int)pk[2], (int)pk[3]}, orsrc, voff, 0, 0);
-            else if (WOC == 2)
-                __builtin_amdgcn_raw_buffer_store_b64((v2i){(int)pk[0], (int)pk[WOC > 1 ? 1 : 0]}, orsrc, voff, 0, 0);
-            else
-                __builtin_amdgcn_raw_buffer_store_b32((int)pk[0], orsrc, voff, 0, 0);
-            if (ragged) {
-                const bool part = pix < total_pix && nvalid > 0 && nvalid < WOC * 4;
-                const int nv = part ? nvalid : 0;
-                const int o4 = nv & 8, o2 = nv & 12, o1 = nv & 14;
-                const uint32_t w4 = o4 ? pk[(WOC * 4 > 8) ? 2 : 0] : pk[0];
-                const int i2 = o2 >> 2, i1 = o1 >> 2;
-                uint32_t w2 = pk[0], w1 = pk[0];
-#pragma unroll
-                for (int q = 1; q < WOC; q++) {
-                    w2 = i2 == q ? pk[q] : w2;
-                    w1 = i1 == q ? pk[q] : w1;
-                }
-                w1 >>= (o1 & 2) * 8;
-                if (WOC == 4)
-                    __builtin_amdgcn_raw_buffer_store_b64((v2i){(int)pk[0], (int)pk[1]}, orsrc, (nv & 8) ? (int)off : -1, 0, 0);
-                __builtin_amdgcn_raw_buffer_store_b32((int)w4, orsrc, (nv & 4) ? (int)off + o4 : -1, 0, 0);
-                __builtin_amdgcn_raw_buffer_store_b16((short)w2, orsrc, (nv & 2) ? (int)off + o2 : -1, 0, 0);
-                __builtin_amdgcn_raw_buffer_store_b8((char)w1, orsrc, (nv & 1) ? (int)off + o1 : -1, 0, 0);
-            }
-        }
-#pragma unroll
-        for (int i = 0; i < STAGES - 1; i++) younger[i] += ragged ? NST * (WOC == 4 ? 5 : 4) : NST;
-    }
-    ANAT_END(p);
+#define PERSIST_BLOCK blockIdx.x
+#include "conv_i8_persist_body.hpp"
+#undef PERSIST_BLOCK
+}
+
+struct conv_group_member_t {
+    mhip_conv_i8_t p;
+    fastdiv_t dhw, dow;
+    unsigned total_pix, noc, npt, ngrp, kw_magic, out_bytes, in_bytes;
+    int k64, lg_inc, bufmode, wres;
+    unsigned end;
+};
+struct conv_group_t {
+    conv_group_member_t m[3];
+};
+static_assert(sizeof(conv_group_t) <= 3072, "the group's parameters travel as kernel arguments");
+template <int BPX, int BN, bool HAS_LUT>
+__global__ __launch_bounds__(NTHREADS) void conv_i8_persist_group(const conv_group_t g, const int8_t *__restrict__ zeros) {
+    constexpr int STAGES = 2;
+    constexpr bool SEG = false, PAIR = false;
+    const unsigned bid = blockIdx.x;
+    const int mi = (bid >= g.m[0].end ? 1 : 0) + (bid >= g.m[1].end ? 1 : 0);
+    const unsigned local = bid - (mi == 0 ? 0u : g.m[mi - 1].end);
+    const conv_group_member_t &mb = g.m[mi];
+    if (local >= mb.noc * mb.ngrp) return;
+    const mhip_conv_i8_t &pin = mb.p;
+    const unsigned total_pix = mb.total_pix, noc = mb.noc, npt = mb.npt, ngrp = mb.ngrp, kw_magic = mb.kw_magic;
+    const unsigned out_bytes_first = mb.out_bytes, in_bytes = mb.in_bytes, noc0 = mb.noc;
+    const int k64 = mb.k64, lg_inc = mb.lg_inc, bufmode = mb.bufmode, wres = mb.wres;
+    const fastdiv_t dhw = mb.dhw, dow = mb.dow;
+    const conv_out_side_t alt = {};
+#define PERSIST_BLOCK local
+#include "conv_i8_persist_body.hpp"
+#undef PERSIST_BLOCK
 }
 ANAT_SETTER(mhip_anatomy_set_i8)
 __device__ __forceinline__ bool mhip_small_c_dev(int in_c, int kw, int out_c) { return in_c <= 4 && kw <= 8 && out_c <= 64; }
@@ -1121,6 +882,109 @@
     return launch_pair_t<128, 32>(a, b, total_pix, k64, lg, magic, wres);
 }
 
+static unsigned long g_group_launches = 0;
+extern "C" unsigned long mhip_conv_i8_group_launches(void) { return g_group_launches; }
+template <int BPX, int BN, bool HAS_LUT>
+static int launch_group_t(conv_group_t &g, int n, const double *work, size_t lds) {
+    static bool attr = false;
+    if (!attr && hipFuncSetAttribute((const void *)conv_i8_persist_group<BPX, BN, HAS_LUT>, hipFuncAttributeMaxDynamicSharedMemorySize,
+                                     80 * 1024) != hipSuccess)
+        return mhip_check(hipErrorUnknown, "conv_i8_persist_group LDS attribute");
+    attr = true;
+    int occ = 0, dev = 0;
+    static int cus = 0;
+    if (!cus) {
+        hipDeviceProp_t prop;
+        if (hipGetDevice(&dev) != hipSuccess || hipGetDeviceProperties(&prop, dev) != hipSuccess)
+            return mhip_check(hipErrorUnknown, "conv_i8_persist_group device query");
+        cus = prop.multiProcessorCount > 0 ? prop.multiProcessorCount : 1;
+    }
+    if (hipOccupancyMaxActiveBlocksPerMultiprocessor(&occ, conv_i8_persist_group<BPX, BN, HAS_LUT>, NTHREADS, lds) != hipSuccess)
+        return mhip_check(hipErrorUnknown, "conv_i8_persist_group occupancy query");
+    const double slots = tune().persist_slots > 0 ? (double)tune().persist_slots : (double)((occ > 0 ? occ : 1) * cus);
+    double total = 0;
+    for (int i = 0; i < n; i++) total += work[i];
+    unsigned end = 0;
+    for (int i = 0; i < 3; i++) {
+        conv_group_member_t &mb = g.m[i];
+        if (i < n) {
+            const double share = slots * (mb.wres ? 1.0 : 4.0) * (work[i] / total);
+            unsigned ng = (unsigned)(share / mb.noc);
+            if (ng < 1) ng = 1;
+            if (ng > mb.npt) ng = mb.npt;
+            mb.ngrp = ng;
+            end += (mb.noc * ng + 7u) & ~7u;
+        }
+        mb.end = end;
+    }
+    hipLaunchKernelGGL((conv_i8_persist_group<BPX, BN, HAS_LUT>), dim3(end), dim3(NTHREADS), lds, mhip_stream_native(), g,
+                       (const int8_t *)mhip_zero_page());
+    g_group_launches++;
+    return mhip_check(hipGetLastError(), "conv_i8_persist_group launch");
+}
+extern "C" int mhip_conv_i8_group(const mhip_conv_i8_t *ps, int n) {
+    if (!ps || n < 2 || n > 3 || !tune().persist || tune().variant || !mhip_zero_page()) return -2;
+    conv_group_t g;
+    memset(&g, 0, sizeof(g));
+    double work[3];
+    int bn = 0, bpx = 0, has_lut = 0;
+    size_t lds = 0;
+    for (int i = 0; i < n; i++) {
+        const mhip_conv_i8_t *p = &ps[i];
+        if (!p->in || !p->out || !p->w || p->frames <= 0 || p->kh != 1 || p->kw != 1 || p->stride_h != 1 || p->stride_w != 1 || p->pad_top ||
+            p->pad_left || p->in_h != p->out_h || p->in_w != p->out_w || p->in_h <= 0 || p->in_w <= 0 || p->out_c <= 0 || p->nseg > 1 ||
+            p->add || p->pre_w || p->in_planar || p->variant || (p->in_c % 16) != 0 || mhip_conv_i8_small_c(p->in_c, p->kw, p->out_c) ||
+            !persist_eligible(p) || ((p->out_c | p->out_pix_stride | p->out_ch_off) & 15) != 0 || p->out_pix_stride < 0 || p->out_ch_off < 0 ||
+            (p->out_pix_stride && p->out_pix_stride < p->out_ch_off + p->out_c))
+            return -2;
+        int row_pad, oc_pad;
+        mhip_conv_i8_pack_geom(p->in_c, p->kw, p->out_c, &row_pad, &oc_pad, nullptr);
+        if (row_pad != p->row_pad || oc_pad != p->oc_pad) return -2;
+        const long total_pix = (long)p->frames * p->out_h * p->out_w;
+        if (total_pix <= 0 || total_pix > 0x7fffffffL) return -2;
+        const int k64 = (p->kh * p->row_pad + BK - 1) / BK * BK, nks = k64 / BK;
+        const int b = p->oc_pad % 128 == 0 ? 128 : (p->oc_pad % 64 == 0 ? 64 : 32);
+        const variant_t dv = default_variant(p, nks);
+        const bool walker = dv.persist > 0 && dv.stages == 2 && !dv.patch && !dv.rows && !dv.r128 && !dv.w8 && !dv.ks2;
+        const int px = walker && dv.bpx == 256 ? 256 : 128;
+        const int wres = walker && dv.wres;
+        if (i == 0) { bn = b; bpx = px; has_lut = p->lut != nullptr; }
+        if (b != bn || px != bpx || (p->lut != nullptr) != (has_lut != 0)) return -2;
+        const size_t need = wres ? LUTB + 2 * (size_t)px * BK + (size_t)nks * b * BK : LUTB + 2 * (size_t)(px + b) * BK;
+        if (need > 80 * 1024) return -2;
+        if (need > lds) lds = need;
+        conv_group_member_t &mb = g.m[i];
+        mb.p = *p;
+        mb.total_pix = (unsigned)total_pix;
+        mb.k64 = k64;
+        mb.noc = (unsigned)(p->oc_pad / b);
+        mb.npt = (unsigned)((total_pix + px - 1) / px);
+        mb.lg_inc = 0;
+        while ((1 << mb.lg_inc) < p->in_c) mb.lg_inc++;
+        mb.kw_magic = 65536u;
+        mb.dhw = make_fastdiv((unsigned)(p->out_h * p->out_w));
+        mb.dow = make_fastdiv((unsigned)p->out_w);
+        mb.out_bytes = (unsigned)persist_out_bytes(p);
+        mb.in_bytes = (unsigned)in_extent_bytes(p);
+        mb.bufmode = buf_mode(p, k64);
+        mb.wres = wres;
+        work[i] = (double)mb.npt * nks * mb.noc;
+    }
+    for (int i = 1; i < n; i++)
+        for (int j = i; j > 0 && work[j] > work[j - 1]; j--) {
+            const conv_group_member_t t = g.m[j]; g.m[j] = g.m[j - 1]; g.m[j - 1] = t;
+            const double w = work[j]; work[j] = work[j - 1]; work[j - 1] = w;
+        }
+    if (bpx == 256) {
+        if (bn == 128) return has_lut ? launch_group_t<256, 128, true>(g, n, work, lds) : launch_group_t<256, 128, false>(g, n, work, lds);
+        if (bn == 64) return has_lut ? launch_group_t<256, 64, true>(g, n, work, lds) : launch_group_t<256, 64, false>(g, n, work, lds);
+        return has_lut ? launch_group_t<256, 32, true>(g, n, work, lds) : launch_group_t<256, 32, false>(g, n, work, lds);
+    }
+    if (bn == 128) return has_lut ? launch_group_t<128, 128, true>(g, n, work, lds) : launch_group_t<128, 128, false>(g, n, work, lds);
+    if (bn == 64) return has_lut ? launch_group_t<128, 64, true>(g, n, work, lds) : launch_group_t<128, 64, false>(g, n, work, lds);
+    return has_lut ? launch_group_t<128, 32, true>(g, n, work, lds) : launch_group_t<128, 32, false>(g, n, work, lds);
+}
+
 extern "C" int mhip_conv_i8_seg_ok(const mhip_conv_i8_t *p) {
     return p && (p->in_c % 16) == 0 && !mhip_conv_i8_small_c(p->in_c, p->kw, p->out_c) && seg_valid(p) && persist_eligible(p);
 }
diff --git a/thingino-accel_amd/csrc/hip/conv_i8_persist_body.hpp b/thingino-accel_amd/csrc/hip/conv_i8_persist_body.hpp
--- /dev/null
+++ b/thingino-accel_amd/csrc/hip/conv_i8_persist_body.hpp
@@ -0,0 +1,273 @@
+    ANAT_BEGIN();
+    const int STAGE = wres ? BPX * BK : (BPX + BN) * BK;
+    constexpr int NWN = BN == 128 ? 2 : 1;
+    constexpr int NWM = 4 / NWN;
+    constexpr int WPX = BPX / NWM / 16;
+    constexpr int WOC = BN / NWN / 16;
+    constexpr int XI = BPX / 64;
+    constexpr int LW = BN >= 128 ? 2 : 1;
+    constexpr int L = XI + LW;
+    constexpr int NST = WPX;
+    extern __shared__ __attribute__((aligned(16))) int8_t dynlds[];
+    uint8_t *slut = (uint8_t *)dynlds;
+    int8_t *lds = dynlds + LUTB;
+    lds_base_must_be_zero(dynlds);
+
+    const int tid = threadIdx.x, lane = tid & 63;
+    const int wv = __builtin_amdgcn_readfirstlane(tid >> 6);
+    const unsigned id = xcd_remap(PERSIST_BLOCK, noc * ngrp);
+    const unsigned grp = id / noc;
+    unsigned ot = id - grp * noc;
+    mhip_conv_i8_t p = pin;
+    unsigned out_bytes = out_bytes_first;
+    if (PAIR && ot >= noc0) {
+        ot -= noc0;
+        p.lut2 = alt.lut2;
+        p.out = alt.out; p.out_stride = alt.out_stride; p.w = alt.w; p.bias = alt.bias; p.lut = alt.lut;
+        p.out_c = alt.out_c; p.relu = alt.relu; p.out_pix_stride = alt.out_pix_stride; p.out_ch_off = alt.out_ch_off;
+        p.cs = alt.cs;
+        out_bytes = alt.out_bytes;
+    }
+    const int oc0 = (int)ot * BN;
+    const unsigned t0 = (unsigned)(((unsigned long long)grp * npt) / ngrp);
+    const unsigned t1 = (unsigned)(((unsigned long long)(grp + 1) * npt) / ngrp);
+    if (t0 >= t1) return;
+    const unsigned hw = (unsigned)(p.out_h * p.out_w);
+    const int wm = wv % NWM, wn = wv / NWM;
+    const int pxw = wm * (WPX * 16), ocw = wn * (WOC * 16);
+
+    auto packed_row16 = [](int c) { return ((c >> 2) & 1) * 16 + (c >> 3) * 4 + (c & 3); };
+    v4i bias[WOC];
+#pragma unroll
+    for (int s = 0; s < WOC; s++)
+        bias[s] = p.bias ? *(const v4i *)(p.bias + (BN == 16 ? packed_row16((lane >> 4) * 4) : oc0 + ocw + s * 16 + (lane >> 4) * 4)) : (v4i){0, 0, 0, 0};
+    if (HAS_LUT) {
+        if (p.lut2) { if (tid < 128) ((uint32_t *)slut)[tid] = ((const uint32_t *)p.lut2)[tid]; }
+        else if (tid < 64) ((uint32_t *)slut)[tid] = ((const uint32_t *)p.lut)[tid];
+        __syncthreads();
+    }
+    const __amdgpu_buffer_rsrc_t orsrc = __builtin_amdgcn_make_buffer_rsrc(p.out, 0, (int)out_bytes, 0x00020000);
+
+    const int schunk = (lane & 3) ^ (((lane >> 4) & 1) << 1);
+    const int8_t *xwin[XI];
+    unsigned tapmask[XI];
+    unsigned rowf[SEG ? XI : 1], rowrem[SEG ? XI : 1];
+    unsigned rowrem_up[SEG ? XI : 1];
+    int xvoff[XI];
+    auto setup_rows = [&](unsigned tile) {
+#pragma unroll
+        for (int j = 0; j < XI; j++) {
+            const unsigned pix = tile * BPX + wv * (BPX / 4) + j * 16 + (lane >> 2);
+            const bool valid = pix < total_pix;
+            const unsigned f = valid ? fdiv(pix, dhw) : 0u;
+            const unsigned rem = valid ? pix - f * hw : 0u;
+            if (SEG) {
+                rowf[j] = f;
+                rowrem[j] = rem;
+                const unsigned oy = fdiv(rem, dow), ox = rem - oy * (unsigned)p.out_w;
+                rowrem_up[j] = (oy >> 1) * ((unsigned)p.out_w >> 1) + (ox >> 1);
+                tapmask[j] = valid ? 1u : 0u;
+                continue;
+            }
+            const int oy = (int)fdiv(rem, dow), ox = (int)(rem - (unsigned)oy * (unsigned)p.out_w);
+            const int iy0 = oy * p.stride_h - p.pad_top, ix0 = ox * p.stride_w - p.pad_left;
+            xwin[j] = p.in + (size_t)f * p.in_stride + ((long)iy0 * p.in_w + ix0) * p.in_c;
+            xvoff[j] = (int)(f * (unsigned)p.in_stride) + (iy0 * p.in_w + ix0) * p.in_c + schunk * 16;
+            const int kx_lo = ix0 < 0 ? -ix0 : 0, kx_hi = p.in_w - ix0 < p.kw ? p.in_w - ix0 : p.kw;
+            const unsigned colbits = kx_hi > kx_lo ? ((kx_hi >= 32 ? ~0u : (1u << kx_hi) - 1u) & ~((1u << kx_lo) - 1u)) : 0u;
+            unsigned m = 0;
+            for (int r = 0; r < p.kh; r++) {
+                const int iy = iy0 + r;
+                if (iy >= 0 && iy < p.in_h) m |= colbits << (r * p.kw);
+            }
+            tapmask[j] = valid ? m : 0u;
+        }
+    };
+    const int8_t *wsrc[LW];
+    int wq[LW], wvoff[LW];
+#pragma unroll
+    for (int j = 0; j < LW; j++) {
+        wq[j] = BN >= 64 ? wv * LW + j : (BN == 16 ? 0 : (wv & 1));
+        const int wrow = BN == 16 ? packed_row16(lane >> 2) : oc0 + wq[j] * 16 + (lane >> 2);
+        wsrc[j] = p.w + (size_t)wrow * k64 + schunk * 16;
+        wvoff[j] = wrow * k64 + schunk * 16;
+    }
+    const __amdgpu_buffer_rsrc_t xrs = __builtin_amdgcn_make_buffer_rsrc((void *)p.in, 0, (int)in_bytes, 0x00020000);
+    const __amdgpu_buffer_rsrc_t wrs = __builtin_amdgcn_make_buffer_rsrc((void *)p.w, 0, p.oc_pad * k64, 0x00020000);
+    const int taps = p.kh * p.kw;
+    const int nks = k64 / BK;
+
+    auto issue = [&](int ks, int stage) {
+        int8_t *sb = lds + stage * STAGE;
+        const unsigned pos = (unsigned)(ks * BK + schunk * 16);
+        if (SEG) {
+            auto owner = [&](int c) { return (c >= p.seg_c0[1]) + (c >= p.seg_c0[2]) + (c >= p.seg_c0[3]); };
+            const int sa = owner(ks * BK), sb2 = owner(ks * BK + 32);
+            const bool hi = schunk >= 2;
+            const int8_t *base = hi ? p.seg_in[sb2] : p.seg_in[sa];
+            const unsigned fstride = (unsigned)(hi ? p.seg_stride[sb2] : p.seg_stride[sa]);
+            const unsigned segc = (unsigned)(hi ? p.seg_c[sb2] : p.seg_c[sa]);
+            const unsigned coff = pos - (unsigned)(hi ? p.seg_c0[sb2] : p.seg_c0[sa]);
+            const bool up = ((p.seg_up >> (hi ? sb2 : sa)) & 1) != 0;
+            const bool kvalid = (int)pos < p.in_c;
+#pragma unroll
+            for (int j = 0; j < XI; j++) {
+                const bool ok = kvalid & (tapmask[j] != 0u);
+                const int8_t *src = base + (size_t)rowf[j] * fstride + (size_t)(up ? rowrem_up[j] : rowrem[j]) * segc + coff;
+                glds16(ok ? src : zeros, sb + (wv * (BPX / 4) + j * 16) * BK);
+            }
+        } else if (bufmode) {
+            const int utap = (ks * BK) >> lg_inc, urc = (ks * BK) & ((1 << lg_inc) - 1);
+            const int uky = (int)(((unsigned)utap * kw_magic) >> 16), ukx = utap - uky * p.kw;
+            const int ukoff = (uky * p.in_w + ukx) * p.in_c + urc;
+            const bool uvalid = utap < taps;
+#pragma unroll
+            for (int j = 0; j < XI; j++) {
+                const bool ok = uvalid & (((tapmask[j] >> utap) & 1u) != 0u);
+                blds16(xrs, ok ? xvoff[j] + ukoff : -1, 0, sb + (wv * (BPX / 4) + j * 16) * BK);
+            }
+            if (!wres)
+#pragma unroll
+                for (int j = 0; j < LW; j++) blds16(wrs, wvoff[j], ks * BK, sb + BPX * BK + wq[j] * 16 * BK);
+            return;
+        } else {
+            const unsigned tap = pos >> lg_inc;
+            const int rc = (int)(pos & ((1u << lg_inc) - 1u));
+            const int ky = (int)((tap * kw_magic) >> 16);
+            const int kx = (int)tap - ky * p.kw;
+            const bool kvalid = (int)tap < taps;
+            const long koff = ((long)ky * p.in_w + kx) * p.in_c + rc;
+#pragma unroll
+            for (int j = 0; j < XI; j++) {
+                const bool ok = kvalid & ((tapmask[j] >> tap) & 1u);
+                glds16(ok ? xwin[j] + koff : zeros, sb + (wv * (BPX / 4) + j * 16) * BK);
+            }
+        }
+        if (!wres)
+#pragma unroll
+            for (int j = 0; j < LW; j++) glds16(wsrc[j] + ks * BK, sb + BPX * BK + wq[j] * 16 * BK);
+    };
+
+    int8_t *const wres_base = lds + STAGES * STAGE;
+    if (wres)
+        for (int ks = 0; ks < nks; ks++)
+#pragma unroll
+            for (int j = 0; j < LW; j++) glds16(wsrc[j] + ks * BK, wres_base + (ks * BN + wq[j] * 16) * BK);
+    unsigned itile = t0;
+    int iks = 0;
+    int younger[STAGES - 1];
+    setup_rows(t0);
+    int nstage = 0;
+#pragma unroll
+    for (int s = 0; s < STAGES - 1; s++) {
+        int n = 0;
+        if (itile < t1) {
+            issue(iks, nstage);
+            n = wres ? XI : L;
+            if (++iks == nks) {
+                iks = 0;
+                if (++itile < t1) setup_rows(itile);
+            }
+        }
+#pragma unroll
+        for (int i = 0; i < s; i++) younger[i] += n;
+        younger[s] = 0;
+        nstage++;
+    }
+    nstage = STAGES - 1;
+
+    const int frow = lane & 15, fchunk = lane >> 4;
+    const int chan = ocw + (lane >> 4) * (4 * WOC);
+    const int pstride = p.out_pix_stride ? p.out_pix_stride : p.out_c;
+    const int lo = p.relu ? 0 : -128;
+    const uint8_t *lut128 = slut + 128;
+    const bool ragged = (p.out_c % (WOC * 4)) != 0;
+    int stage = 0;
+    ANAT_NOW(1);
+    for (unsigned tile = t0; tile < t1; tile++) {
+        v4i acc[WOC][WPX];
+        for (int ks = 0; ks < nks; ks++) {
+            wait_vmcnt_at_most<(STAGES - 2) * L, NST>(younger[0]);
+            __builtin_amdgcn_s_barrier();
+            asm volatile("" ::: "memory");
+            const int8_t *xs = lds + stage * STAGE, *ws = wres ? wres_base + ks * (BN * BK) : xs + BPX * BK;
+            v4i xb[WPX], wa[WOC];
+#pragma unroll
+            for (int t = 0; t < WPX; t++) xb[t] = *(const v4i *)(xs + lds_off(pxw + t * 16 + frow, fchunk));
+#pragma unroll
+            for (int s = 0; s < WOC; s++) wa[s] = *(const v4i *)(ws + lds_off(ocw + s * 16 + frow, fchunk));
+            int n = 0;
+            if (itile < t1) {
+                issue(iks, nstage);
+                n = wres ? XI : L;
+                if (++iks == nks) {
+                    iks = 0;
+                    if (++itile < t1) setup_rows(itile);
+                }
+            }
+#pragma unroll
+            for (int i = 0; i + 1 < STAGES - 1; i++) younger[i] = younger[i + 1] + n;
+            younger[STAGES - 2] = 0;
+            if (ks == 0) {
+#pragma unroll
+                for (int s = 0; s < WOC; s++)
+#pragma unroll
+                    for (int t = 0; t < WPX; t++) acc[s][t] = __builtin_amdgcn_mfma_i32_16x16x64_i8(wa[s], xb[t], bias[s], 0, 0, 0);
+            } else {
+#pragma unroll
+                for (int s = 0; s < WOC; s++)
+#pragma unroll
+                    for (int t = 0; t < WPX; t++) acc[s][t] = __builtin_amdgcn_mfma_i32_16x16x64_i8(wa[s], xb[t], acc[s][t], 0, 0, 0);
+            }
+            stage = stage + 1 == STAGES ? 0 : stage + 1;
+            nstage = nstage + 1 == STAGES ? 0 : nstage + 1;
+        }
+#ifdef ANATOMY
+        if (tile + 1 == t1) ANAT_NOW(2);
+#endif
+#pragma unroll
+        for (int t = 0; t < WPX; t++) {
+            const unsigned pix = tile * BPX + pxw + t * 16 + (lane & 15);
+            const unsigned f = fdiv(pix, dhw), rem = pix - f * hw;
+            const unsigned off = f * (unsigned)p.out_stride + rem * (unsigned)pstride + (unsigned)(p.out_ch_off + oc0 + chan);
+            const int nvalid = p.out_c - (oc0 + chan);
+            const bool ok = pix < total_pix && nvalid >= WOC * 4;
+            uint32_t pk[WOC];
+            int a[WOC * 4];
+#pragma unroll
+            for (int s = 0; s < WOC; s++)
+#pragma unroll
+                for (int r = 0; r < 4; r++) a[s * 4 + r] = acc[s][t][r];
+            if (HAS_LUT && p.lut2) requant_pack<WOC * 4, HAS_LUT, true, true, false, true>(a, p.cs, lo, lut128, pk);
+            else requant_pack<WOC * 4, HAS_LUT, true, true>(a, p.cs, lo, lut128, pk);
+            const int voff = ok ? (int)off : -1;
+            if (WOC == 4)
+                __builtin_amdgcn_raw_buffer_store_b128((v4i){(int)pk[0], (int)pk[1], (int)pk[2], (int)pk[3]}, orsrc, voff, 0, 0);
+            else if (WOC == 2)
+                __builtin_amdgcn_raw_buffer_store_b64((v2i){(int)pk[0], (int)pk[WOC > 1 ? 1 : 0]}, orsrc, voff, 0, 0);
+            else
+                __builtin_amdgcn_raw_buffer_store_b32((int)pk[0], orsrc, voff, 0, 0);
+            if (ragged) {
+                const bool part = pix < total_pix && nvalid > 0 && nvalid < WOC * 4;
+                const int nv = part ? nvalid : 0;
+                const int o4 = nv & 8, o2 = nv & 12, o1 = nv & 14;
+                const uint32_t w4 = o4 ? pk[(WOC * 4 > 8) ? 2 : 0] : pk[0];
+                const int i2 = o2 >> 2, i1 = o1 >> 2;
+                uint32_t w2 = pk[0], w1 = pk[0];
+#pragma unroll
+                for (int q = 1; q < WOC; q++) {
+                    w2 = i2 == q ? pk[q] : w2;
+                    w1 = i1 == q ? pk[q] : w1;
+                }
+                w1 >>= (o1 & 2) * 8;
+                if (WOC == 4)
+                    __builtin_amdgcn_raw_buffer_store_b64((v2i){(int)pk[0], (int)pk[1]}, orsrc, (nv & 8) ? (int)off : -1, 0, 0);
+                __builtin_amdgcn_raw_buffer_store_b32((int)w4, orsrc, (nv & 4) ? (int)off + o4 : -1, 0, 0);
+                __builtin_amdgcn_raw_buffer_store_b16((short)w2, orsrc, (nv & 2) ? (int)off + o2 : -1, 0, 0);
+                __builtin_amdgcn_raw_buffer_store_b8((char)w1, orsrc, (nv & 1) ? (int)off + o1 : -1, 0, 0);
+            }
+        }
+#pragma unroll
+        for (int i = 0; i < STAGES - 1; i++) younger[i] += ragged ? NST * (WOC == 4 ? 5 : 4) : NST;
+    }
+    ANAT_END(p);
diff --git a/thingino-accel_amd/csrc/host/mars_internal.h b/thingino-accel_amd/csrc/host/mars_internal.h
--- a/thingino-accel_amd/csrc/host/mars_internal.h
+++ b/thingino-accel_amd/csrc/host/mars_internal.h
@@ -67,6 +67,7 @@
     int nseg, seg_t[4], seg_c[4], seg_up;
     int chain_n, chain_out[3];
     int pair_next;
+    int group_next;
     int row_pad, oc_pad, c_pad;
     int ch_off, scale_h, scale_w, bn_n;
     int out_pix_stride, out_ch_off;
@@ -96,7 +97,7 @@
 typedef struct {
     int fusion;
     unsigned no_fuse_lut : 1, no_nhwc_internal : 1, no_vconcat_q : 1, no_pair_f32 : 1, no_rec : 1, no_zero_tail : 1, no_vconcat_f32 : 1,
-        no_rowpad : 1;
+        no_rowpad : 1, no_colaunch : 1;
     size_t rec_limit;
     size_t vconcat_limit;
     size_t bottleneck_limit;
@@ -200,6 +201,7 @@
 MARS_INTERNAL void fuse_lut(mars_model_ext_t *m);
 MARS_INTERNAL void nhwc_internal(mars_model_ext_t *m);
 MARS_INTERNAL void fold_add(mars_model_ext_t *m, int f32);
+MARS_INTERNAL void colaunch_convs(mars_model_ext_t *m);
 MARS_INTERNAL void virtual_concat(mars_model_ext_t *m);
 MARS_INTERNAL void elide_concat(mars_model_ext_t *m);
 MARS_INTERNAL void trim_concat(mars_model_ext_t *m);
diff --git a/thingino-accel_amd/csrc/host/mars_model.c b/thingino-accel_amd/csrc/host/mars_model.c
--- a/thingino-accel_amd/csrc/host/mars_model.c
+++ b/thingino-accel_amd/csrc/host/mars_model.c
@@ -26,6 +26,7 @@
     sw->no_zero_tail = getenv("MARS_HIP_NO_ZERO_TAIL") != NULL;
     sw->no_vconcat_f32 = getenv("MARS_HIP_NO_VCONCAT_F32") != NULL;
     sw->no_rowpad = getenv("MARS_HIP_NO_ROWPAD") != NULL;
+    sw->no_colaunch = getenv("MARS_HIP_NO_COLAUNCH") != NULL;
     sw->rec_limit = (e = getenv("MARS_HIP_REC_LIMIT")) ? (size_t)strtoull(e, NULL, 0) : (size_t)0xfffffff0u;
     sw->vconcat_limit = (e = getenv("MARS_HIP_VCONCAT_LIMIT")) ? (size_t)strtoull(e, NULL, 0) : (size_t)0x7fffffffu;
     sw->bottleneck_limit = (e = getenv("MARS_HIP_BOTTLENECK_LIMIT")) ? (size_t)strtoull(e, NULL, 0) : 0;
@@ -157,6 +158,7 @@
         if (m->sw.fusion >= 2 && !m->no_bottleneck) fuse_bottleneck(m);
         pad_output_rows(m);
         virtual_concat_q(m);
+        colaunch_convs(m);
     } else {
         nhwc_internal(m);
     }
@@ -379,7 +381,7 @@
         (ssize_t)o->w_blob_off[1]);
     ADD(" pre %d", o->pre);
     if (o->pre) ADD(" %zd %zd %zd %a", (ssize_t)o->pre_w_off, (ssize_t)o->pre_b_off, (ssize_t)o->pre_lut2_off, (double)o->pre_cs);
-    ADD(" macs %a bytes %a prof_kind %d", o->macs, o->bytes, o->prof_kind);
+    ADD(" macs %a bytes %a prof_kind %d group_next %d", o->macs, o->bytes, o->prof_kind, o->group_next);
 #undef ADD
     return k;
 }
@@ -401,7 +403,7 @@
 #define FLAG(cond, ...) if (cond) k += snprintf(line + k, sizeof line - (size_t)k, __VA_ARGS__)
         FLAG(o->kind == OP_CONV_I8 || o->kind == OP_CONV_F32 || o->kind == OP_CONV_F32_VHEAD, " k%dx%d s%d c%d->%d", o->kh, o->kw, o->sw, o->in_c, o->out_c);
         FLAG(o->nchw, " relayout"); FLAG(o->out_nchw, " planar_store"); FLAG(o->lut_off != NO_OFF, " lut"); FLAG(o->add_t, " add=%d", o->add_t - 1);
-        FLAG(o->nseg, " seg=%d", o->nseg); FLAG(o->pair_next, " pair_next"); FLAG(o->pre, " pre"); FLAG(o->silu_f32, " silu");
+        FLAG(o->nseg, " seg=%d", o->nseg); FLAG(o->pair_next, " pair_next"); FLAG(o->group_next, " group_next"); FLAG(o->pre, " pre"); FLAG(o->silu_f32, " silu");
         FLAG(o->k_limit, " k_limit=%d", o->k_limit); FLAG(o->in_rec, " in_rec=%d", o->in_rec); FLAG(o->out_rec, " out_rec");
         FLAG(o->vc_shift, " view=-%d", o->vc_shift); FLAG(o->vc_n, " vcat=%dx%d", o->vc_n, o->vc_run);
         FLAG(o->rows_only, " rows_only=%d", o->rows_only); FLAG(o->out_byte_off, " out_off=%zu", o->out_byte_off); FLAG(o->chain_n, " chain=%d", o->chain_n);
@@ -428,9 +430,9 @@
         const plan_switches_t *w = &m->sw;
         snprintf(line, sizeof line, "+plan n_ops %d arena_size %zu scratch_per_frame %zu blob_mirror_bytes %zu rec_max_frames %zu rec_skipped %d f32_mode %d | fusion %d"
                  " no_fuse_lut %d no_nhwc_internal %d no_vconcat_q %d no_pair_f32 %d no_rec %d no_zero_tail %d no_vconcat_f32 %d no_rowpad %d rec_limit %zu"
-                 " vconcat_limit %zu bottleneck_limit %zu\n", m->n_ops, m->arena_size, m->scratch_per_frame, m->blob_mirror_bytes, m->rec_max_frames, m->rec_skipped,
+                 " vconcat_limit %zu bottleneck_limit %zu no_colaunch %d\n", m->n_ops, m->arena_size, m->scratch_per_frame, m->blob_mirror_bytes, m->rec_max_frames, m->rec_skipped,
                  m->plan_f32_mode, w->fusion, w->no_fuse_lut, w->no_nhwc_internal, w->no_vconcat_q, w->no_pair_f32, w->no_rec, w->no_zero_tail, w->no_vconcat_f32,
-                 w->no_rowpad, w->rec_limit, w->vconcat_limit, w->bottleneck_limit);
+                 w->no_rowpad, w->rec_limit, w->vconcat_limit, w->bottleneck_limit, w->no_colaunch);
         EMIT();
     }
 #undef EMIT
diff --git a/thingino-accel_amd/csrc/host/mars_plan.c b/thingino-accel_amd/csrc/host/mars_plan.c
--- a/thingino-accel_amd/csrc/host/mars_plan.c
+++ b/thingino-accel_amd/csrc/host/mars_plan.c
@@ -1199,6 +1199,42 @@
             if (op_reads(b, b->t_out) || op_reads(b, a->t_out)) continue;
             if (pair_up(m, i, j)) break;
         }
+    }
+}
+
+static int colaunchable(const mars_model_ext_t *m, int i) {
+    const mars_op_t *o = &m->ops[i];
+    const int oc = o->store_c ? o->store_c : o->out_c;
+    return o->kind == OP_CONV_I8 && !o->nchw && !o->out_nchw && !o->add_t && !o->nseg && o->safe && !o->pair_next && !o->group_next && !o->pre && !o->variant &&
+           !(i > 0 && (m->ops[i - 1].pair_next || m->ops[i - 1].group_next)) && o->n_in == 1 && o->t_in[0] >= 0 && o->t_out >= 0 && o->t_in[0] != o->t_out &&
+           o->kh == 1 && o->kw == 1 && o->sh == 1 && o->sw == 1 && !o->pt && !o->pl && o->in_h == o->out_h && o->in_w == o->out_w && o->in_c >= 16 &&
+           (o->in_c & (o->in_c - 1)) == 0 && ((oc | o->out_pix_stride | o->out_ch_off) & 15) == 0 && !o->in_byte_off && !o->out_byte_off;
+}
+static int colaunch_tile(const mars_op_t *o) { return o->oc_pad % 128 == 0 ? 128 : (o->oc_pad % 64 == 0 ? 64 : 32); }
+void colaunch_convs(mars_model_ext_t *m) {
+    for (int i = 0; i < m->n_ops; i++) m->ops[i].group_next = 0;
+    if (m->sw.fusion < 1 || m->sw.no_colaunch) return;
+    for (int i = 0; i + 1 < m->n_ops; i++) {
+        if (!colaunchable(m, i)) continue;
+        int last = i;
+        for (int j = i + 1; j < m->n_ops && j <= i + 48 && last - i < 2; j++) {
+            if (j <= last) continue;
+            const mars_op_t *a = &m->ops[i], *b = &m->ops[j];
+            if (!colaunchable(m, j)) continue;
+            if (colaunch_tile(a) != colaunch_tile(b) || (a->lut_off != NO_OFF) != (b->lut_off != NO_OFF)) continue;
+            if ((m->mt[a->t_out].io_out != 0) != (m->mt[b->t_out].io_out != 0)) continue;
+            int ok = 1;
+            for (int q = i; q <= last && ok; q++) {
+                const mars_op_t *c = &m->ops[q];
+                if (b->t_out == c->t_out || op_reads(b, c->t_out) || op_reads(c, b->t_out)) ok = 0;
+            }
+            if (!ok) continue;
+            if (!pair_up(m, last, j)) continue;
+            m->ops[last].pair_next = 0;
+            m->ops[last].group_next = 1;
+            last++;
+        }
+        i = last;
     }
 }
 
@@ -1518,6 +1554,10 @@
         else if (o->add_t && !op_reads(o, o->add_t - 1)) why = "add_t is not among t_in";
         else if (o->chain_n && o->t_out != o->chain_out[o->chain_n - 1]) why = "t_out is not the chain's last stage";
         else if (o->pair_next && (i + 1 >= m->n_ops || m->ops[i + 1].kind != o->kind)) why = "pair_next without a mate of its kind";
+        else if (o->group_next && (o->kind != OP_CONV_I8 || o->pair_next || i + 1 >= m->n_ops || m->ops[i + 1].kind != OP_CONV_I8 || m->ops[i + 1].pair_next ||
+                                   (i > 0 && m->ops[i - 1].pair_next)))
+            why = "group_next without a plain int8 convolution behind it";
+        else if (o->group_next && i >= 2 && m->ops[i - 1].group_next && m->ops[i - 2].group_next) why = "a co-launch group of more than 3";
         for (int k = 0; !why && k < o->nseg; k++)
             if (!op_reads(o, o->seg_t[k])) why = "a seg_t is not among t_in";
         for (int k = 0; !why && k < o->vc_n; k++)
diff --git a/thingino-accel_amd/csrc/host/mars_run.c b/thingino-accel_amd/csrc/host/mars_run.c
--- a/thingino-accel_amd/csrc/host/mars_run.c
+++ b/thingino-accel_amd/csrc/host/mars_run.c
@@ -303,8 +303,12 @@
             return (mars_error_t)op->err;
         }
         mars_op_t *mate = op->pair_next && i + 1 < m->n_ops ? &m->ops[i + 1] : NULL;
-        if (wait_tail && ((op->t_out >= 0 && (m->mt[op->t_out].io_out || m->mt[op->t_out].tail_read)) ||
-                          (mate && mate->t_out >= 0 && (m->mt[mate->t_out].io_out || m->mt[mate->t_out].tail_read)))) {
+        int ngroup = 1;
+        while (!mate && ngroup < 3 && i + ngroup < m->n_ops && m->ops[i + ngroup - 1].group_next) ngroup++;
+        int held = mate && mate->t_out >= 0 && (m->mt[mate->t_out].io_out || m->mt[mate->t_out].tail_read);
+        for (int q = 0; q < ngroup; q++)
+            if (op[q].t_out >= 0 && (m->mt[op[q].t_out].io_out || m->mt[op[q].t_out].tail_read)) held = 1;
+        if (wait_tail && held) {
             mhip_stream_wait(sid, m->ev_tail_done);
             wait_tail = 0;
         }
@@ -338,6 +342,15 @@
                 if (!rc) rc = launch_op(m, mate);
             }
             i++;
+        } else if (ngroup > 1) {
+            mhip_conv_i8_t ps[3];
+            for (int q = 0; q < ngroup; q++) conv_i8_params(m, &op[q], &ps[q]);
+            rc = mhip_conv_i8_group(ps, ngroup);
+            if (rc == -2) {
+                rc = 0;
+                for (int q = 0; q < ngroup && !rc; q++) rc = launch_op(m, &op[q]);
+            }
+            i += ngroup - 1;
         } else {
             rc = launch_op(m, op);
         }
@@ -345,6 +358,8 @@
             const mars_op_t *w2[2] = {op, mate};
             for (int q = 0; q < 2; q++)
                 if (w2[q] && op_writes(w2[q], m->scratch_t)) m->scratch_t = -1;
+            for (int q = 1; q < ngroup; q++)
+                if (op_writes(&op[q], m->scratch_t)) m->scratch_t = -1;
         }
         if (m->profiling) {
             const int nx = i + 1;
@@ -683,6 +698,7 @@
         mars_op_t *op = &m->ops[i];
         if (op->kind != OP_CONV_I8 || op->nchw) continue;
         if (op->pair_next || (i > 0 && m->ops[i - 1].pair_next)) continue;
+        if (op->group_next || (i > 0 && m->ops[i - 1].group_next)) continue;
         mhip_conv_i8_t p;
         conv_i8_params(m, op, &p);
         int codes[32];
diff --git a/thingino-accel_amd/csrc/mhip.h b/thingino-accel_amd/csrc/mhip.h
--- a/thingino-accel_amd/csrc/mhip.h
+++ b/thingino-accel_amd/csrc/mhip.h
@@ -88,6 +88,8 @@
 int mhip_conv_i8_variants(const mhip_conv_i8_t *p, int *codes, int max);
 int mhip_conv_i8_seg_ok(const mhip_conv_i8_t *p);
 int mhip_conv_i8_pair(const mhip_conv_i8_t *a, const mhip_conv_i8_t *b);
+int mhip_conv_i8_group(const mhip_conv_i8_t *ps, int n);
+unsigned long mhip_conv_i8_group_launches(void);
 int mhip_conv_i8_small_c(int in_c, int kw, int out_c);
 void mhip_conv_i8_pack_geom(int in_c, int kw, int out_c, int *row_pad, int *oc_pad, int *c_eff);
 int mhip_conv_i8(const mhip_conv_i8_t *p);
```

Result: no change. 55920, median of 6 (+0.6%).
